# jorgeMFS/HYMET

Measured on AMD Instinct MI355X. Metric: contigs/s + Mbp/s classified, CAMI-medium, 1/2/4/8 MI355X; % HBM roofline, higher is better.
Workload: dtype u64

## Files before the change

### hymet_amd/_lib.py

```python
from __future__ import annotations

import ctypes
import os

HERE = os.path.dirname(os.path.abspath(__file__))
LIB_PATH = os.path.join(HERE, "libhymet_gpu.so")

_c = ctypes
_i64, _u64, _i32, _u32, _vp = _c.c_int64, _c.c_uint64, _c.c_int, _c.c_uint32, _c.c_void_p

_SIGS = {
    "hymet_version": (_i32, []),
    "hymet_init": (_i32, [_i32, _c.POINTER(_vp)]),
    "hymet_destroy": (_i32, [_vp]),
    "hymet_last_error": (_c.c_char_p, []),
    "hymet_set_stream": (_i32, [_vp, _vp]),
    "hymet_sync": (_i32, [_vp]),
    "hymet_prof_enable": (_i32, [_vp, _i32]),
    "hymet_prof_reset": (_i32, [_vp]),
    "hymet_prof_query": (_i32, [_vp, _c.c_char_p, _c.POINTER(_c.c_double), _c.POINTER(_i64), _c.POINTER(_c.c_double)]),
    "hymet_prof_names": (_i32, [_vp, _c.c_char_p, _i64]),
    "hymet_scratch_trim": (_i32, [_vp, _c.POINTER(_i64)]),
    "hymet_scratch_cached": (_i32, [_vp, _c.POINTER(_i64)]),
    "hymet_scratch_stats": (_i32, [_vp, _vp]),
    "hymet_scratch_reserve": (_i32, [_vp, _i64]),
    "hymet_set_oom_hook": (_i32, [_vp, _vp]),
    "hymet_copy_to_host": (_i32, [_vp, _vp, _vp, _i64, _i32]),
    "hymet_copy_to_device": (_i32, [_vp, _vp, _vp, _i64, _i32]),
    "hymet_pack": (_i32, [_vp, _vp, _i64, _i32, _vp, _vp]),
    "hymet_fasta_index": (_i32, [_vp, _i64, _i32, _i64, _c.POINTER(_i64), _vp, _vp, _vp, _vp, _vp]),
    "hymet_fasta_names": (_i32, [_vp, _vp, _vp, _i64, _vp, _vp]),
    "hymet_fasta_compact": (_i32, [_vp, _vp, _i64, _i64, _vp, _vp, _vp, _i64, _vp, _i64, _vp]),
    "hymet_name_hash": (_i32, [_vp, _vp, _vp, _vp, _i64, _vp]),
    "hymet_sort_pairs_u64": (_i32, [_vp, _vp, _vp, _i64, _i32, _i32]),
    "hymet_scan_u32": (_i32, [_vp, _vp, _vp, _i64, _i32, _vp]),
    "hymet_msh_open": (_i32, [_c.c_char_p, _c.POINTER(_vp)]),
    "hymet_msh_info_get": (_i32, [_vp, _vp]),
    "hymet_msh_copy": (_i32, [_vp, _i32, _vp, _vp, _vp, _vp, _vp, _vp]),
    "hymet_msh_upload": (_i32, [_vp, _vp, _i32, _vp, _vp, _i32]),
    "hymet_msh_upload_range": (_i32, [_vp, _vp, _i32, _vp, _vp, _i32, _i64, _i64]),
    "hymet_msh_text_offsets": (_i32, [_vp, _vp, _vp]),
    "hymet_msh_close": (None, [_vp]),
    "hymet_screen_table_slots": (_i64, [_i64]),
    "hymet_screen_table_build": (_i32, [_vp, _vp, _i64, _vp, _i64, _vp, _vp, _i32]),
    "hymet_screen_count": (_i32, [_vp, _vp, _vp, _i64, _i64, _i64, _i32, _u32, _i32, _c.POINTER(_vp), _c.POINTER(_i64),
                                  _c.POINTER(_vp), _c.POINTER(_i64), _c.POINTER(_vp), _u64, _vp, _i64, _vp, _vp]),
    "hymet_screen_stats": (_i32, [_vp, _vp, _i64, _vp, _vp, _vp, _vp]),
    "hymet_screen_winner": (_i32, [_vp, _vp, _i64, _vp, _vp, _i64, _vp, _i64, _vp, _vp, _vp]),
    "hymet_sketch_max_size": (_i64, []),
    "hymet_sketch_batch": (_i32, [_vp, _vp, _vp, _i64, _i32, _u32, _i32, _i64, _vp, _vp, _vp, _i32, _vp, _vp]),
    "hymet_mash_dist": (_i32, [_vp, _vp, _i64, _vp, _i64, _vp, _i64, _vp, _i64, _i64, _i64, _i32, _vp]),
    "hymet_mash_dist_tile": (_i32, [_i32]),
    "hymet_mash_dist_tune": (_i32, [_i32, _i32]),
    "hymet_mash_dist_select": (_i32, [_vp, _vp, _i64, _i64, _vp, _i32, _vp, _vp, _vp, _i64, _c.POINTER(_i64)]),
    "hymet_mash_dist_tri": (_i32, [_vp, _vp, _i64, _vp, _i64, _i64, _i64, _i32, _vp]),
    "hymet_mash_link": (_i32, [_vp, _vp, _i64, _i64, _i64, _vp, _i32, _vp, _vp]),
    "hymet_mash_labels": (_i32, [_vp, _vp, _i64, _vp]),
    "hymet_mm_sketch": (_i32, [_vp, _vp, _vp, _vp, _vp, _i32, _i32, _i32, _i32, _vp, _vp, _i64, _c.POINTER(_i64)]),
    "hymet_mm_index_build": (_i32, [_vp, _vp, _vp, _vp, _vp, _i32, _i32, _i32, _c.POINTER(_vp)]),
    "hymet_mm_index_destroy": (_i32, [_vp]),
    "hymet_mm_index_info": (_i32, [_vp, _c.POINTER(_i32), _c.POINTER(_i32), _c.POINTER(_i32), _c.POINTER(_i64)]),
    "hymet_mm_index_max_occ": (_i32, [_vp, _vp, _c.c_float, _c.POINTER(_i32)]),
    "hymet_mm_index_save": (_i32, [_vp, _vp, _c.c_char_p, _i32, _c.POINTER(_i64)]),
    "hymet_mm_index_load": (_i32, [_vp, _c.c_char_p, _i64, _c.POINTER(_vp), _c.POINTER(_i64)]),
    "hymet_mm_index_export": (_i32, [_vp, _vp, _vp, _vp]),
    "hymet_mm_map": (_i32, [_vp, _vp, _vp, _vp, _vp, _vp, _vp, _vp, _i32, _c.POINTER(_vp)]),
    "hymet_mm_result_size": (_i32, [_vp, _c.POINTER(_i64)]),
    "hymet_mm_result_copy": (_i32, [_vp, _vp, _vp, _vp]),
    "hymet_mm_result_destroy": (_i32, [_vp]),
    "hymet_paf_acc_create": (_i32, [_vp, _c.POINTER(_vp)]),
    "hymet_paf_acc_reset": (_i32, [_vp]),
    "hymet_paf_acc_destroy": (_i32, [_vp]),
    "hymet_paf_acc_info": (_i32, [_vp, _c.POINTER(_i64), _c.POINTER(_vp), _c.POINTER(_vp), _c.POINTER(_vp),
                                  _c.POINTER(_vp), _c.POINTER(_vp)]),
    "hymet_paf_acc_append": (_i32, [_vp, _vp, _vp, _i64, _i64]),
    "hymet_paf_acc_copy": (_i32, [_vp, _vp, _vp, _vp, _vp]),
    "hymet_paf_acc_field": (_i32, [_vp, _vp, _i32, _vp]),
    "hymet_mm_map_acc": (_i32, [_vp, _vp, _vp, _vp, _vp, _vp, _vp, _vp, _i32, _i32, _i32, _i32, _vp]),
    "hymet_emit_paf": (_i32, [_vp, _vp, _vp, _vp, _vp, _vp, _vp, _vp, _vp, _i64, _c.POINTER(_i64), _vp]),
    "hymet_acc_ref_counts": (_i32, [_vp, _vp, _vp]),
    "hymet_acc_classify": (_i32, [_vp, _vp, _i32, _i32] + [_vp] * 15 + [_c.POINTER(_i32)]),
    "hymet_emit_tsv": (_i32, [_vp, _i32, _i32] + [_vp] * 14 + [_i64, _c.POINTER(_i64)]),
    "hymet_mm_chain_dp": (_i32, [_vp, _vp, _vp, _i64, _i32, _i32, _i32, _i32, _i32, _c.c_float, _c.c_float, _vp, _vp]),
    "hymet_mm_mark_compact": (_i32, [_vp, _vp, _vp, _vp, _i64, _vp, _vp, _i32, _vp, _vp, _vp, _c.POINTER(_i64)]),
    "hymet_mm_stamp_scratch": (_i32, [_vp, _c.POINTER(_i64), _c.POINTER(_i64)]),
    "hymet_mm_anchor_sort": (_i32, [_vp, _vp, _vp, _i64, _vp, _i32, _i32, _i32, _u64, _i64, _vp, _vp, _vp, _vp, _vp]),
    "hymet_lca_ref_counts": (_i32, [_vp, _vp, _i64, _vp]),
    "hymet_lca": (_i32, [_vp, _i32, _i32] + [_vp] * 17),
}

_lib = None
_oom_hook = None


def _release_torch_cache(_user):
    try:
        import torch
        torch.cuda.empty_cache()
    except Exception:
        pass


class HymetError(RuntimeError):
    pass


def load():
    global _lib
    if _lib is not None:
        return _lib
    path = os.environ.get("HYMET_LIB", LIB_PATH)
    if not os.path.exists(path):
        raise HymetError(f"{path} not found: build the HIP extension (python -m hymet_amd.build); "
                         "hymet_amd has no CPU fallback")
    lib = ctypes.CDLL(path)
    for name, (res, args) in _SIGS.items():
        fn = getattr(lib, name)
        fn.restype = res
        fn.argtypes = args
    global _oom_hook
    _oom_hook = _c.CFUNCTYPE(None, _vp)(_release_torch_cache)
    lib.hymet_set_oom_hook(_c.cast(_oom_hook, _vp), None)
    _lib = lib
    return lib


def exported_symbols():
    return list(_SIGS)


def check(rc: int, what: str):
    if rc != 0:
        msg = load().hymet_last_error()
        raise HymetError(f"{what} failed ({rc}): {msg.decode() if msg else ''}")


class Gpu:

    def __init__(self, device: int = 0, stream=None):
        import torch

        if not torch.cuda.is_available():
            raise HymetError("no GPU visible: hymet_amd runs on MI355X (gfx950) only")
        self.torch = torch
        self.device = device
        torch.cuda.set_device(device)
        self.dev = torch.device("cuda", device)
        self.lib = load()
        h = _vp()
        check(self.lib.hymet_init(device, _c.byref(h)), "hymet_init")
        self.ctx = h
        self.stream = stream
        self.children = []
        self.bind_stream(stream)

    def fork(self) -> "Gpu":
        child = Gpu(self.device, stream=self.torch.cuda.Stream(device=self.device))
        self.children.append(child)
        return child

    def bind_stream(self, stream=None):
        s = stream if stream is not None else self.torch.cuda.current_stream(self.device)
        check(self.lib.hymet_set_stream(self.ctx, _vp(s.cuda_stream)), "hymet_set_stream")
        self.bound_stream = s

    def call(self, name, *args):
        check(getattr(self.lib, name)(self.ctx, *args), name)

    def sync(self):
        check(self.lib.hymet_sync(self.ctx), "hymet_sync")
        for ch in self.children:
            ch.sync()

    def prof(self, on: bool = True):
        check(self.lib.hymet_prof_enable(self.ctx, int(on)), "hymet_prof_enable")
        for ch in self.children:
            ch.prof(on)

    def prof_reset(self):
        check(self.lib.hymet_prof_reset(self.ctx), "hymet_prof_reset")
        for ch in self.children:
            ch.prof_reset()

    def prof_table(self):
        buf = _c.create_string_buffer(1 << 16)
        check(self.lib.hymet_prof_names(self.ctx, buf, 1 << 16), "hymet_prof_names")
        out = {}
        for name in buf.value.decode().split():
            ms, n, b = _c.c_double(), _i64(), _c.c_double()
            check(self.lib.hymet_prof_query(self.ctx, name.encode(), _c.byref(ms), _c.byref(n), _c.byref(b)), "hymet_prof_query")
            out[name] = (ms.value, n.value, b.value)
        for ch in self.children:
            for name, (ms, n, b) in ch.prof_table().items():
                m0, n0, b0 = out.get(name, (0.0, 0, 0.0))
                out[name] = (m0 + ms, n0 + n, b0 + b)
        return out

    def trim(self) -> int:
        out = _i64()
        check(self.lib.hymet_scratch_trim(self.ctx, _c.byref(out)), "hymet_scratch_trim")
        return out.value

    def reserve(self, nbytes: int):
        check(self.lib.hymet_scratch_reserve(self.ctx, int(nbytes)), "hymet_scratch_reserve")

    def _alloc(self, fn, n, dtype):
        try:
            return fn(int(n), dtype=dtype, device=self.dev)
        except self.torch.OutOfMemoryError:
            if self.trim() == 0:
                raise
            return fn(int(n), dtype=dtype, device=self.dev)

    def empty(self, n, dtype):
        return self._alloc(self.torch.empty, n, dtype)

    def zeros(self, n, dtype):
        return self._alloc(self.torch.zeros, n, dtype)

    def close(self):
        if self.ctx:
            self.lib.hymet_destroy(self.ctx)
            self.ctx = None

    def __del__(self):
        try:
            self.close()
        except Exception:
            pass


def ptr(t) -> _vp:
    return _vp(t.data_ptr())
```

### hymet_amd/csrc/common.hpp

```cpp
#pragma once
#include <hip/hip_runtime.h>
#include <stdint.h>
#include <algorithm>
#include <cstdlib>
#include <map>
#include <string>
#include <utility>
#include <vector>
#include "../../include/hymet_gpu.h"

struct hymet_ctx {
    int device = 0;
    hipStream_t stream = nullptr;
    bool own_stream = false;
    int n_cu = 256;
    bool prof = false;
    std::map<std::string, std::vector<std::pair<hipEvent_t, hipEvent_t>>> ev;
    std::map<std::string, double> bytes;
    std::map<std::string, std::pair<int, double>> dev_bytes;
    int64_t *prof_dev = nullptr;
    void *stage[2] = {nullptr, nullptr};
    hipEvent_t stage_ev[2] = {nullptr, nullptr};
    int64_t *mbox_h = nullptr;
    int64_t *mbox_d = nullptr;
    int32_t *dctr = nullptr;
    int32_t *stamp = nullptr;
    int64_t stamp_cap = 0;
    size_t stamp_cls = 0;
};

namespace hymet {
struct ProfScope {
    hymet_ctx *c;
    const char *name;
    hipEvent_t a = nullptr, b = nullptr;
    ProfScope(hymet_ctx *ctx, const char *n, double alg_bytes = 0.0) : c(ctx), name(n) {
        if (c && c->prof && hipEventCreate(&a) == hipSuccess && hipEventCreate(&b) == hipSuccess) {
            (void)hipEventRecord(a, c->stream);
            c->bytes[name] += alg_bytes;
        }
    }
    ProfScope(hymet_ctx *ctx, const char *n, int slot, double per_unit) : ProfScope(ctx, n, 0.0) {
        if (c && c->prof) c->dev_bytes[name] = {slot, per_unit};
    }
    ~ProfScope() {
        if (c && c->prof && a && b) {
            (void)hipEventRecord(b, c->stream);
            c->ev[name].push_back({a, b});
        }
    }
};
constexpr int kProfSlots = 8;
inline int64_t *prof_dev_slot(hymet_ctx *c, int k) { return c && c->prof && c->prof_dev ? c->prof_dev + k : nullptr; }
}

namespace hymet {
constexpr int kMbox = 64;
inline int64_t *mb_dev(hymet_ctx *c, int i) { return c->mbox_d + i; }
inline int64_t mb_read(const hymet_ctx *c, int i) { return __atomic_load_n(c->mbox_h + i, __ATOMIC_ACQUIRE); }
}

namespace hymet {
inline const char *env_str(const char *name) {
    const char *e = getenv(name);
    return e && *e ? e : nullptr;
}
inline bool env_flag(const char *name, bool dflt = false) {
    const char *e = env_str(name);
    return e ? e[0] != '0' : dflt;
}
inline int64_t env_int(const char *name, int64_t dflt, int64_t lo, int64_t hi) {
    const char *e = env_str(name);
    return e ? std::max(lo, std::min(hi, (int64_t)atoll(e))) : dflt;
}
}

namespace hymet {
void set_error(const std::string &msg);
int fail(int code, const std::string &msg);
int hip_fail(hipError_t e, const char *what);
inline int64_t cdiv(int64_t a, int64_t b) { return (a + b - 1) / b; }
hipError_t scratch_alloc(size_t bytes, hipStream_t stream, void **p, size_t *cls);
void set_oom_hook(void (*hook)(void *), void *user);
void scratch_free(void *p, hipStream_t stream, size_t cls);
hipError_t stamp_scratch(hymet_ctx *ctx, int64_t n, int32_t **out);
void stamp_release(hymet_ctx *ctx);
}

#define HY_CHECK_LAUNCH(what)                                   \
    do {                                                        \
        hipError_t e_ = hipGetLastError();                      \
        if (e_ != hipSuccess) return hymet::hip_fail(e_, what); \
    } while (0)

#define HY_HIP(call)                                            \
    do {                                                        \
        hipError_t e_ = (call);                                 \
        if (e_ != hipSuccess) return hymet::hip_fail(e_, #call); \
    } while (0)

#define HY_ARG(cond, msg)                                                   \
    do {                                                                    \
        if (!(cond)) return hymet::fail(HYMET_E_ARG, std::string(msg));     \
    } while (0)
```

### hymet_amd/csrc/mm_map.hip

```cpp
#include "mm_stages.hpp"

#include <algorithm>
#include <type_traits>
#include <utility>

#include <chrono>
#include <cstdio>
#include <cstdlib>
#include <cstring>

struct hymet_mm_result {
    int n_q = 0;
    std::vector<int64_t> reg_off;
    std::vector<int32_t> rep_len;
    std::vector<hymet_mm_reg> regs;
};

namespace hymet {
namespace mm {

int launch_regions(hymet_ctx *ctx, const uint64_t *ax, const uint32_t *ay, int span, const int32_t *ids, const int64_t *cfirst,
                   const uint64_t *cu, const int64_t *cboff,
                   const int64_t *qc, const int64_t *qb, const uint64_t *mini_pos, const int64_t *mp_off, const int64_t *qlen,
                   const uint32_t *name_hash, const int32_t *rep_len, const int64_t *ref_len, int n_q, const hymet_mm_opt *o,
                   int k, void *z, hymet_mm_reg *regs, int32_t *w, uint64_t *cov, int32_t *tmp, int32_t *n_regs,
                   int64_t NB, int64_t NC, int64_t NM, const uint32_t *cq,
                   const MiniWord *mtab, const int64_t *qbase, const uint32_t *skip_q, uint64_t *sumk, bool sumk_done);

namespace {

__global__ void fill_qid_kernel(const int64_t *off, int n_q, int64_t n, uint32_t *qid, uint32_t *ones, int32_t *zq) {
    const int64_t i = (int64_t)blockIdx.x * blockDim.x + threadIdx.x;
    if (i < n) {
        qid[i] = (uint32_t)upper_idx(off, n_q, i);
        if (ones) ones[i] = 1u;
    }
    if (zq && i < n_q) zq[i] = 0;
}

__global__ void flagged_len_kernel(const uint32_t *flag, const int64_t *qb, int n_q, uint32_t *cnt, int64_t *any) {
    const int q = blockIdx.x * blockDim.x + threadIdx.x;
    if (q > n_q) return;
    if (q == n_q) {
        cnt[q] = 0;
        return;
    }
    const bool f = flag[q] != 0;
    cnt[q] = f ? (uint32_t)(qb[q + 1] - qb[q]) : 0u;
    if (f) *any = 1;
}


__global__ void mzflt_runs_kernel(const uint32_t *sq, const uint64_t *sx, const uint32_t *sidx, const int64_t *qm_off,
                                  int64_t n, int q_occ_max, float q_occ_frac, uint32_t *keep) {
    const int64_t p = (int64_t)blockIdx.x * blockDim.x + threadIdx.x;
    if (p >= n) return;
    if (p > 0 && sq[p] == sq[p - 1] && sx[p] == sx[p - 1]) return;
    int64_t e = p + 1;
    while (e < n && sq[e] == sq[p] && sx[e] == sx[p]) e++;
    const uint32_t q = sq[p];
    const int64_t nq = qm_off[q + 1] - qm_off[q];
    if (nq <= q_occ_max) return;
    const int32_t cnt = (int32_t)(e - p);
    if (cnt > q_occ_max && (float)cnt > (float)nq * q_occ_frac)
        for (int64_t j = p; j < e; j++) keep[sidx[j]] = 0;
}

constexpr int kMzBuckets = 4096;
__global__ __launch_bounds__(256) void mzflt_screen_kernel(const uint64_t *mx, const int64_t *qm_off, int n_q, int q_occ_max,
                                                           uint32_t *keep, uint32_t *cnt, int64_t *any) {
    __shared__ uint32_t h[kMzBuckets];
    __shared__ int hit;
    const int q = blockIdx.x;
    if (q == n_q) {
        if (threadIdx.x == 0) cnt[q] = 0;
        return;
    }
    const int64_t s = qm_off[q], nq = qm_off[q + 1] - s;
    for (int64_t e = threadIdx.x; e < nq; e += 256) keep[s + e] = 1u;
    if (nq <= q_occ_max) {
        if (threadIdx.x == 0) cnt[q] = 0;
        return;
    }
    for (int b = threadIdx.x; b < kMzBuckets; b += 256) h[b] = 0;
    if (threadIdx.x == 0) hit = 0;
    __syncthreads();
    bool over = false;
    for (int64_t e = threadIdx.x; e < nq; e += 256)
        over |= atomicAdd(&h[(uint32_t)(mx[s + e] >> 8) & (kMzBuckets - 1)], 1u) >= (uint32_t)q_occ_max;
    if (over) hit = 1;
    __syncthreads();
    if (threadIdx.x == 0) {
        cnt[q] = hit ? (uint32_t)nq : 0u;
        if (hit) *any = 1;
    }
}

__global__ __launch_bounds__(256) void mzflt_list_kernel(const int64_t *qm_off, const uint32_t *cnt, const int64_t *coff,
                                                         uint32_t *gidx, uint32_t *sq) {
    const int q = blockIdx.x;
    const uint32_t nq = cnt[q];
    if (nq == 0) return;
    const int64_t s = qm_off[q], d = coff[q];
    for (uint32_t e = threadIdx.x; e < nq; e += 256) {
        gidx[d + e] = (uint32_t)(s + e);
        sq[d + e] = (uint32_t)q;
    }
}

__global__ void mzflt_gather_kernel(const uint32_t *perm, const uint32_t *gidx, const uint64_t *mx, uint32_t *gout,
                                    uint64_t *xout, int64_t n) {
    const int64_t i = (int64_t)blockIdx.x * blockDim.x + threadIdx.x;
    if (i >= n) return;
    const uint32_t g = gidx[perm[i]];
    gout[i] = g;
    xout[i] = mx[g];
}

__global__ void compact_mz_kernel(const uint64_t *x, const uint64_t *y, const uint32_t *keep, int64_t *pos, int64_t n,
                                  uint64_t *ox, uint64_t *oy) {
    const int64_t i = (int64_t)blockIdx.x * blockDim.x + threadIdx.x;
    if (i == n - 1) pos[n] = pos[i] + keep[i];
    if (i < n && keep[i]) {
        ox[pos[i]] = x[i];
        oy[pos[i]] = y[i];
    }
}

__global__ void sample_off_kernel(const int64_t *pos, const int64_t *qm_off, int n_q, int64_t total, int64_t *out) {
    const int q = blockIdx.x * blockDim.x + threadIdx.x;
    if (q > n_q) return;
    out[q] = q == n_q ? total : pos[qm_off[q]];
}

__global__ void seed_count_kernel(const uint64_t *mx, int64_t n, const uint32_t *koff, int64_t n_buckets,
                                  uint32_t *seed_n) {
    const int64_t i = (int64_t)blockIdx.x * blockDim.x + threadIdx.x;
    if (i >= n) return;
    const uint64_t h = mx[i] >> 8;
    uint32_t c = 0;
    if ((int64_t)h < n_buckets) c = koff[h + 1] - koff[h];
    seed_n[i] = c;
}

constexpr uint32_t kFlt = 0x80000000u;

__global__ void seed_class_kernel(const uint32_t *seed_n, int64_t M, int max_occ, uint64_t *cls) {
    const int64_t i = (int64_t)blockIdx.x * blockDim.x + threadIdx.x;
    if (i > M) return;
    if (i == M) {
        cls[M] = 0;
        return;
    }
    const uint32_t n = seed_n[i];
    const bool hi = (int)n > max_occ, lo = n > 0 && !hi;
    cls[i] = (uint64_t)(hi ? 1u : 0u) << 32 | (lo ? 1u : 0u);
}

__global__ void seed_list_kernel(const uint32_t *seed_n, const uint64_t *rank, int64_t M, int max_occ, int32_t *low_idx,
                                 int32_t *high_idx) {
    const int64_t i = (int64_t)blockIdx.x * blockDim.x + threadIdx.x;
    if (i >= M) return;
    const uint32_t n = seed_n[i];
    if (!n) return;
    if ((int)n > max_occ) high_idx[rank[i] >> 32] = (int32_t)i;
    else low_idx[(uint32_t)rank[i]] = (int32_t)i;
}

struct StreakParams {
    const uint64_t *my;
    const uint32_t *qid;
    const int64_t *qm_off, *qlen;
    const uint64_t *rank;
    const int32_t *low_idx, *high_idx;
    int64_t n_low;
    int n_q;
    int max_occ, max_max_occ, dist;
    uint32_t *seed_n;
    uint32_t *flt_high;
};

__global__ void streak_kernel(StreakParams P) {
    const int64_t t = (int64_t)blockIdx.x * blockDim.x + threadIdx.x;
    if (t >= P.n_low + P.n_q) return;
    int q;
    int64_t e_idx = -1, p_idx = -1;
    uint64_t re, rp;
    if (t < P.n_low) {
        e_idx = P.low_idx[t];
        q = (int)P.qid[e_idx];
        re = P.rank[e_idx];
        if (t > 0 && P.qid[P.low_idx[t - 1]] == (uint32_t)q) p_idx = P.low_idx[t - 1];
    } else {
        q = (int)(t - P.n_low);
        re = P.rank[P.qm_off[q + 1]];
        const uint64_t r0 = P.rank[P.qm_off[q]];
        if ((uint32_t)re > (uint32_t)r0) p_idx = P.low_idx[(uint32_t)re - 1];
    }
    rp = p_idx >= 0 ? P.rank[p_idx] : P.rank[P.qm_off[q]];
    const int64_t h0 = (int64_t)(rp >> 32), h1 = (int64_t)(re >> 32);
    const int cnt = (int)(h1 - h0);
    if (cnt <= 0) return;
    const bool case_a = P.dist > 0 && P.max_max_occ > P.max_occ;
    bool keep_all = false, keep_none = false;
    uint64_t thr = 0;
    if (case_a) {
        const uint64_t rq0 = P.rank[P.qm_off[q]], rq1 = P.rank[P.qm_off[q + 1]];
        const int64_t n_seed = (int64_t)((uint32_t)rq1 - (uint32_t)rq0) + (int64_t)((rq1 >> 32) - (rq0 >> 32));
        if (n_seed <= 1) return;
        const int32_t ps = p_idx >= 0 ? (int32_t)((uint32_t)P.my[p_idx] >> 1) : 0;
        const int32_t pe = e_idx >= 0 ? (int32_t)((uint32_t)P.my[e_idx] >> 1) : (int32_t)P.qlen[q];
        int32_t mh = (int32_t)((double)(pe - ps) / P.dist + .499);
        if (mh > 128) mh = 128;
        keep_all = mh >= cnt, keep_none = mh <= 0;
        if (!keep_all && !keep_none) {
            uint64_t lo = 0, hi = ~0ull;
            while (lo < hi) {
                const uint64_t mid = lo + (hi - lo) / 2;
                int c = 0;
                for (int64_t r = h0; r < h1; r++) {
                    const int32_t a = P.high_idx[r];
                    c += ((uint64_t)P.seed_n[a] << 32 | (uint32_t)a) <= mid;
                }
                if (c >= mh) hi = mid;
                else lo = mid + 1;
            }
            thr = lo;
        }
    }
    for (int64_t r = h0; r < h1; r++) {
        const int32_t a = P.high_idx[r];
        const uint32_t n = P.seed_n[a];
        bool flt = true;
        if (case_a) {
            const bool chosen = keep_all || (!keep_none && ((uint64_t)n << 32 | (uint32_t)a) <= thr);
            flt = !chosen || (int)n > P.max_max_occ;
        }
        P.flt_high[r] = flt ? 1u : 0u;
    }
}

__global__ void flt_mark_kernel(const uint32_t *flt_high, int64_t n_high, int32_t *v) {
    const int64_t r = (int64_t)blockIdx.x * blockDim.x + threadIdx.x;
    if (r < n_high) v[r] = flt_high[r] ? (int32_t)r : -1;
}

__global__ void rep_len_kernel(const uint32_t *flt_high, const int32_t *prev_max, const int32_t *high_idx, int64_t n_high,
                               const uint64_t *mx, const uint64_t *my, const uint32_t *qid, int32_t *rep_len,
                               uint32_t *seed_n) {
    const int64_t r = (int64_t)blockIdx.x * blockDim.x + threadIdx.x;
    if (r >= n_high || !flt_high[r]) return;
    const int32_t a = high_idx[r];
    const uint32_t q = qid[a];
    const int32_t en = (int32_t)((uint32_t)my[a] >> 1) + 1, st = en - (int32_t)(mx[a] & 0xff);
    int32_t en_prev = 0;
    const int32_t pr = r > 0 ? prev_max[r - 1] : -1;
    if (pr >= 0) {
        const int32_t b = high_idx[pr];
        if (qid[b] == q) en_prev = (int32_t)((uint32_t)my[b] >> 1) + 1;
    }
    atomicAdd(rep_len + q, en - max(st, en_prev));
    seed_n[a] = 0;
}

__global__ void nz_flag_kernel(const uint32_t *v, int64_t n, uint32_t *flag) {
    const int64_t i = (int64_t)blockIdx.x * blockDim.x + threadIdx.x;
    if (i < n) flag[i] = v[i] ? 1u : 0u;
}

struct AnchorParams {
    const uint64_t *mx, *my;
    const uint32_t *seed_n;
    const int64_t *a_pos;
    const uint32_t *qid;
    const int64_t *qlen;
    const uint32_t *koff;
    const uint64_t *ipos;
    int64_t n;
    int rb;
    uint64_t *ax, *k1, *k2;
    uint32_t *ay;
    uint32_t *val;
    const int64_t *mp_pos;
    uint64_t *mini_pos;
};

__global__ void write_anchors_kernel(AnchorParams P) {
    const int64_t i = (int64_t)blockIdx.x * blockDim.x + threadIdx.x;
    if (i >= P.n) return;
    const uint32_t n = P.seed_n[i];
    if (!n) return;
    const uint64_t mx = P.mx[i], my = P.my[i];
    const uint32_t q_pos = (uint32_t)my, q_span = (uint32_t)(mx & 0xff);
    P.mini_pos[P.mp_pos[i]] = (uint64_t)q_span << 32 | (q_pos >> 1);
    const uint32_t q = P.qid[i];
    const int32_t qlen = (int32_t)P.qlen[q];
    const uint32_t *kp = P.koff + (mx >> 8);
    const uint64_t *r = P.ipos + kp[0];
    int64_t a = P.a_pos[i];
    for (uint32_t k = 0; k < n; k++, a++) {
        const uint64_t rk = r[k];
        const uint32_t rpos = (uint32_t)rk >> 1;
        const uint32_t rid = (uint32_t)(rk >> 32);
        uint64_t x, y;
        uint32_t rev;
        if ((rk & 1) == (q_pos & 1)) {
            rev = 0;
            x = (rk & 0xffffffff00000000ULL) | rpos;
            y = (uint64_t)q_span << 32 | (q_pos >> 1);
        } else {
            rev = 1;
            x = 1ULL << 63 | (rk & 0xffffffff00000000ULL) | rpos;
            y = (uint64_t)q_span << 32 | (uint32_t)(qlen - (int32_t)((q_pos >> 1) + 1 - q_span) - 1);
        }
        P.ax[a] = x;
        P.ay[a] = (uint32_t)y;
        P.k1[a] = (uint64_t)q << (1 + P.rb) | (uint64_t)rev << P.rb | rid;
        P.k2[a] = (uint64_t)rpos << 32 | (uint32_t)y;
        P.val[a] = (uint32_t)a;
    }
}

struct AnchorKeyParams {
    const uint64_t *mx, *my;
    const uint32_t *seed_n;
    const int64_t *a_pos;
    const uint32_t *qid;
    const int64_t *qlen;
    const uint32_t *koff;
    const uint64_t *ipos;
    int64_t n;
    int rb, pb;
    int ybits;
    uint64_t *key;
    uint32_t *val;
    const int64_t *mp_pos;
    uint64_t *mini_pos;
};

__global__ __launch_bounds__(256) void write_anchor_keys_kernel(AnchorKeyParams P) {
    __shared__ int64_t s_a[257];
    __shared__ uint64_t s_r[256];
    __shared__ uint32_t s_yf[256], s_yr[256], s_strand[256];
    __shared__ uint64_t s_q[256];
    const int tid = threadIdx.x;
    const int64_t m0 = (int64_t)blockIdx.x * 256;
    const int cnt = (int)min((int64_t)256, P.n - m0);
    if (tid < cnt) {
        const int64_t i = m0 + tid;
        const uint32_t n = P.seed_n[i];
        const uint64_t mx = P.mx[i], my = P.my[i];
        const uint32_t q_pos = (uint32_t)my, q_span = (uint32_t)(mx & 0xff);
        const uint32_t q = P.qid[i];
        if (n) P.mini_pos[P.mp_pos[i]] = (uint64_t)q_span << 32 | (q_pos >> 1);
        s_a[tid] = P.a_pos[i];
        s_r[tid] = P.koff[mx >> 8];
        s_yf[tid] = q_pos >> 1;
        s_yr[tid] = (uint32_t)((int32_t)P.qlen[q] - (int32_t)((q_pos >> 1) + 1 - q_span) - 1);
        s_strand[tid] = q_pos & 1;
        s_q[tid] = (uint64_t)q << (1 + P.rb + P.pb);
    }
    if (tid == 0) s_a[cnt] = P.a_pos[m0 + cnt];
    __syncthreads();
    const int64_t a0 = s_a[0], a1 = s_a[cnt];
    const int sh_rev = P.rb + P.pb;
    for (int64_t a = a0 + tid; a < a1; a += 256) {
        int lo = 0, hi = cnt - 1;
        while (lo < hi) {
            const int mid = (lo + hi + 1) >> 1;
            if (s_a[mid] <= a) lo = mid;
            else hi = mid - 1;
        }
        const uint64_t rk = P.ipos[s_r[lo] + (a - s_a[lo])];
        const uint32_t rpos = (uint32_t)rk >> 1;
        const uint64_t rid = rk >> 32;
        const uint32_t rev = ((uint32_t)rk & 1) != s_strand[lo];
        const uint64_t k = (uint64_t)rev << sh_rev | rid << P.pb | rpos;
        const uint32_t y = rev ? s_yr[lo] : s_yf[lo];
        if (P.ybits) {
            P.key[a] = k << P.ybits | y;
        } else {
            P.key[a] = s_q[lo] | k;
            P.val[a] = y;
        }
    }
}

__global__ void anchor_unpack_kernel(const uint64_t *key, const uint32_t *val, int64_t n, int rb, int pb, uint64_t *ax,
                                     uint32_t *ay) {
    const int64_t i = (int64_t)blockIdx.x * blockDim.x + threadIdx.x;
    if (i >= n) return;
    const uint64_t k = key[i];
    const uint64_t rev = k >> (rb + pb) & 1, rid = k >> pb & ((1ull << rb) - 1), rpos = k & ((1ull << pb) - 1);
    ax[i] = rev << 63 | rid << 32 | rpos;
    const bool prev_eq = i > 0 && key[i - 1] == k;
    const bool next_eq = i + 1 < n && key[i + 1] == k;
    if (!prev_eq && !next_eq) {
        ay[i] = val[i];
    } else if (!prev_eq) {
        int64_t e = i + 1;
        while (e + 1 < n && key[e + 1] == k) e++;
        for (int64_t a = i; a <= e; a++) {
            const uint32_t v = val[a];
            int64_t b = a;
            while (b > i && ay[b - 1] > v) {
                ay[b] = ay[b - 1];
                b--;
            }
            ay[b] = v;
        }
    }
}

__global__ __launch_bounds__(256) void mini_bits_kernel(const uint64_t *my, const uint32_t *seed_n, const uint32_t *qid,
                                                        const int64_t *qbase, int64_t M, MiniWord *tab) {
    const int64_t i = (int64_t)blockIdx.x * blockDim.x + threadIdx.x;
    const int lane = threadIdx.x & 63;
    const bool on = i < M && seed_n[i];
    const int64_t b = on ? qbase[qid[i]] + ((uint32_t)my[i] >> 1) : -64 * (int64_t)(lane + 1);
    const int64_t w = b >> 6;
    uint64_t bits = on ? 1ull << (b & 63) : 0;
#pragma unroll
    for (int d = 1; d < 64; d <<= 1) {
        const int64_t wo = __shfl_down(w, d, 64);
        const uint64_t bo = __shfl_down(bits, d, 64);
        if (lane + d < 64 && wo == w) bits |= bo;
    }
    const int64_t wp = __shfl_up(w, 1, 64);
    if (on && (lane == 0 || wp != w)) atomicOr((unsigned long long *)&tab[w].bits, bits);
}
__global__ void mini_base_kernel(const uint64_t *my, const uint32_t *seed_n, const uint32_t *qid, const int64_t *qm_off,
                                 const int64_t *mp_pos, const int64_t *qbase, int64_t M, MiniWord *tab) {
    const int64_t i = (int64_t)blockIdx.x * blockDim.x + threadIdx.x;
    if (i >= M || !seed_n[i]) return;
    const uint32_t q = qid[i];
    const int64_t b = qbase[q] + ((uint32_t)my[i] >> 1);
    const uint64_t bits = tab[b >> 6].bits;
    tab[b >> 6].base = (uint32_t)(mp_pos[i] - mp_pos[qm_off[q]]) - (uint32_t)__popcll(bits & ((1ull << (b & 63)) - 1));
}

__global__ void rechain_gather_kernel(const uint64_t *bx, const uint32_t *by, const int64_t *qb, const uint32_t *qflag,
                                      const int64_t *new_off, int n_q, int rb, uint64_t *x, uint32_t *y, uint64_t *k1,
                                      uint64_t *k2, uint32_t *val) {
    const int q = blockIdx.x;
    if (q >= n_q || !qflag[q]) return;
    const int64_t b0 = qb[q], b1 = qb[q + 1], o = new_off[q];
    for (int64_t i = b0 + threadIdx.x; i < b1; i += blockDim.x) {
        const int64_t a = o + (i - b0);
        const uint64_t ax = bx[i];
        const uint32_t ay = by[i];
        x[a] = ax;
        y[a] = ay;
        k1[a] = (uint64_t)q << (1 + rb) | (ax >> 63) << rb | (ax << 1 >> 33);
        k2[a] = (uint64_t)(uint32_t)ax << 32 | ay;
        val[a] = (uint32_t)a;
    }
}

__global__ __launch_bounds__(256) void rechain_keys_kernel(const uint64_t *bx, const uint32_t *by, const int64_t *qb,
                                                           const int64_t *new_off, int n_q, int64_t n, int rb, int pb,
                                                           int ybits, uint64_t *key, uint32_t *val) {
    __shared__ int s_q0;
    const int64_t a0 = (int64_t)blockIdx.x * blockDim.x;
    if (threadIdx.x == 0) s_q0 = upper_idx(new_off, n_q, a0);
    __syncthreads();
    const int64_t a = a0 + threadIdx.x;
    if (a >= n) return;
    int q = s_q0;
    while (q + 1 < n_q && new_off[q + 1] <= a) q++;
    const int64_t i = qb[q] + (a - new_off[q]);
    const uint64_t ax = bx[i];
    const uint64_t k = (ax >> 63) << (rb + pb) | (ax << 1 >> 33) << pb | (uint32_t)ax;
    if (ybits) {
        key[a] = k << ybits | by[i];
    } else {
        key[a] = (uint64_t)q << (1 + rb + pb) | k;
        val[a] = by[i];
    }
}

__global__ void reg_count_kernel(const uint32_t *flag, const int32_t *n1, const int32_t *n2, int n_q, uint32_t *cnt) {
    const int q = blockIdx.x * blockDim.x + threadIdx.x;
    if (q < n_q) cnt[q] = (uint32_t)((flag && flag[q]) ? n2[q] : n1[q]);
}

struct RegOut {
    hymet_mm_reg *regs;
    int32_t *q, *part, *rl, *t;
    int32_t q_base, part_id, t_base;
};
__global__ void reg_gather_kernel(const uint32_t *flag, const int32_t *n1, const int32_t *n2, const int64_t *qc1,
                                  const int64_t *qc2, const hymet_mm_reg *r1, const hymet_mm_reg *r2, const int64_t *off,
                                  const int32_t *rep_len, int n_q, RegOut o) {
    const int q = blockIdx.x * blockDim.x + threadIdx.x;
    if (q >= n_q) return;
    const bool use2 = flag && flag[q];
    const hymet_mm_reg *src = use2 ? r2 + qc2[q] : r1 + qc1[q];
    const int nr = use2 ? n2[q] : n1[q];
    const int64_t d = off[q];
    for (int i = 0; i < nr; i++) {
        const hymet_mm_reg r = src[i];
        o.regs[d + i] = r;
        if (o.q) {
            o.q[d + i] = o.q_base + q;
            o.part[d + i] = o.part_id;
            o.rl[d + i] = rep_len[q];
            o.t[d + i] = o.t_base + r.rid;
        }
    }
}
}
}
}

using namespace hymet;
using namespace hymet::mm;

struct CallTrace {
    bool on = env_flag("HYMET_TRACE");
    std::chrono::steady_clock::time_point t = std::chrono::steady_clock::now();
    ~CallTrace() {
        if (on)
            fprintf(stderr, "[hymet_mm_map] %-22s %9.2f ms\n", "TOTAL (with frees)",
                    std::chrono::duration<double, std::milli>(std::chrono::steady_clock::now() - t).count());
    }
};
struct PhaseTrace {
    hymet_ctx *ctx;
    bool on;
    std::chrono::steady_clock::time_point t;
    explicit PhaseTrace(hymet_ctx *c) : ctx(c), on(env_flag("HYMET_TRACE")), t(std::chrono::steady_clock::now()) {}
    void mark(const char *what) {
        if (!on) return;
        (void)hipStreamSynchronize(ctx->stream);
        const auto n = std::chrono::steady_clock::now();
        fprintf(stderr, "[hymet_mm_map] %-22s %9.2f ms\n", what, std::chrono::duration<double, std::milli>(n - t).count());
        t = n;
    }
};

static int sort_anchor_set(hymet_ctx *ctx, DevBuf &x, DevBuf &y, DevBuf &k1, DevBuf &k2, DevBuf &val, int64_t n,
                           int key1_bits, int yhi, AnchorSet &out) {
    DevBuf k2b, valb, k1g, k1b;
    HY_HIP(k2b.alloc(8 * (size_t)n, ctx->stream));
    HY_HIP(valb.alloc(4 * (size_t)n, ctx->stream));
    uint64_t *kk = k2.as<uint64_t>(), *kka = k2b.as<uint64_t>();
    uint32_t *vv = val.as<uint32_t>(), *vva = valb.as<uint32_t>();
    int rc = sort_pairs(ctx, kk, kka, vv, vva, n, 0, 64, "radix_sort_anchor_pos");
    if (rc) return rc;
    HY_HIP(k1g.alloc(8 * (size_t)n, ctx->stream));
    HY_HIP(k1b.alloc(8 * (size_t)n, ctx->stream));
    LAUNCH1(gather_kernel<uint64_t>, n, k1.as<uint64_t>(), vv, k1g.as<uint64_t>(), n);
    uint64_t *k1p = k1g.as<uint64_t>(), *k1a = k1b.as<uint64_t>();
    rc = sort_pairs(ctx, k1p, k1a, vv, vva, n, 0, key1_bits, "radix_sort_anchor_group");
    if (rc) return rc;
    HY_HIP(out.ax.alloc(8 * (size_t)n, ctx->stream));
    HY_HIP(out.ay.alloc(4 * (size_t)n, ctx->stream));
    LAUNCH1(gather_kernel<uint64_t>, n, x.as<uint64_t>(), vv, out.ax.as<uint64_t>(), n);
    LAUNCH1(gather_kernel<uint32_t>, n, y.as<uint32_t>(), vv, out.ay.as<uint32_t>(), n);
    out.n = n;
    out.span = yhi & 0xff;
    return HYMET_OK;
}

static int sort_anchor_words(hymet_ctx *ctx, DevBuf &word, int64_t n, int rb, int pb, int yhi, const int64_t *d_qoff, int n_q,
                             int64_t max_qlen, AnchorSet &out) {
    DevBuf wb;
    HY_HIP(wb.alloc(8 * (size_t)n, ctx->stream));
    HY_HIP(out.ax.alloc(8 * (size_t)n, ctx->stream));
    HY_HIP(out.ay.alloc(4 * (size_t)n, ctx->stream));
    HY_HIP(out.hb.alloc(head_bits_bytes(n), ctx->stream));
    HY_HIP(out.ax32.alloc(4 * (size_t)n, ctx->stream));
    out.n = n;
    out.span = yhi & 0xff;
    const bool log_stats = env_flag("HYMET_ASORT_STATS");
    DevBuf sstat;
    if (log_stats) {
        HY_HIP(sstat.alloc(32, ctx->stream));
        HY_HIP(hipMemsetAsync(sstat.p, 0, 32, ctx->stream));
    }
    const int rc = grouped_anchor_sort(ctx, word.as<uint64_t>(), n, d_qoff, n_q, rb, pb, max_qlen,
                                       wb.as<uint64_t>(), out.ax.as<uint64_t>(), out.ay.as<uint32_t>(),
                                       out.hb.as<uint32_t>(), out.ax32.as<uint32_t>(),
                                       log_stats ? sstat.as<unsigned long long>() : nullptr);
    if (rc == 1) return hymet::fail(HYMET_E_INTERNAL, "sort_anchor_words: anchor words emitted for a layout without one");
    if (rc) return rc;
    if (log_stats) {
        unsigned long long h[4] = {};
        HY_HIP(hipMemcpyAsync(h, sstat.p, 32, hipMemcpyDeviceToHost, ctx->stream));
        HY_HIP(hipStreamSynchronize(ctx->stream));
        fprintf(stderr, "[asort] anchors %lld fast_segs %llu fast_anchors %llu full_segs %llu full_anchors %llu\n",
                (long long)n, h[0], h[1], h[2], h[3]);
    }
    out.has_hb = out.has_x32 = true;
    return HYMET_OK;
}

static int sort_anchor_keys(hymet_ctx *ctx, DevBuf &key, DevBuf &val, int64_t n, int end_bit, int rb, int pb, int yhi,
                            AnchorSet &out) {
    DevBuf kb, vb;
    HY_HIP(kb.alloc(8 * (size_t)n, ctx->stream));
    HY_HIP(vb.alloc(4 * (size_t)n, ctx->stream));
    HY_HIP(out.ax.alloc(8 * (size_t)n, ctx->stream));
    HY_HIP(out.ay.alloc(4 * (size_t)n, ctx->stream));
    out.n = n;
    out.span = yhi & 0xff;
    uint64_t *kk = key.as<uint64_t>(), *kka = kb.as<uint64_t>();
    uint32_t *vv = val.as<uint32_t>(), *vva = vb.as<uint32_t>();
    int rc = sort_pairs<uint64_t, uint32_t>(ctx, kk, kka, vv, vva, n, 0, end_bit, "radix_sort_anchors");
    if (rc) return rc;
    {
        ProfScope _ps(ctx, "mm_anchor_unpack", 24.0 * (double)n);
        LAUNCH1(anchor_unpack_kernel, n, kk, vv, n, rb, pb, out.ax.as<uint64_t>(), out.ay.as<uint32_t>());
    }
    return HYMET_OK;
}

static int dump_anchors(hymet_ctx *ctx, const char *var, const AnchorSet &S, int n_q, bool &dumped) {
    const char *path = env_str(var);
    if (!path || dumped || S.n == 0) return HYMET_OK;
    dumped = true;
    hipStream_t st = ctx->stream;
    const int64_t nd = std::min<int64_t>(S.n, env_int("HYMET_DUMP_MAX", 1 << 24, 0, INT64_MAX));
    std::vector<uint64_t> hx(nd);
    std::vector<uint32_t> hy(nd);
    std::vector<int64_t> qo(n_q + 1);
    HY_HIP(hipMemcpyAsync(hx.data(), S.ax.p, 8 * (size_t)nd, hipMemcpyDeviceToHost, st));
    HY_HIP(hipMemcpyAsync(hy.data(), S.ay.p, 4 * (size_t)nd, hipMemcpyDeviceToHost, st));
    HY_HIP(hipMemcpyAsync(qo.data(), S.d_off.p, 8 * (size_t)(n_q + 1), hipMemcpyDeviceToHost, st));
    HY_HIP(hipStreamSynchronize(st));
    if (FILE *fp = fopen(path, "wb")) {
        uint64_t gid = 0;
        int q = 0;
        std::vector<uint64_t> buf;
        buf.reserve(1 << 21);
        for (int64_t a = 0; a < nd; a++) {
            bool qs = false;
            while (q < n_q && qo[q + 1] <= a) q++, qs = true;
            if (a && (qs || (hx[a] >> 32) != (hx[a - 1] >> 32))) gid++;
            buf.push_back(gid << 32 | (uint32_t)hx[a]);
            buf.push_back((uint64_t)S.span << 32 | hy[a]);
            if (buf.size() >= (1u << 21)) fwrite(buf.data(), 8, buf.size(), fp), buf.clear();
        }
        fwrite(buf.data(), 8, buf.size(), fp);
        fclose(fp);
    }
    return HYMET_OK;
}

struct MapSink {
    hymet_mm_result *res = nullptr;
    hymet_paf_acc *acc = nullptr;
    int32_t q_base = 0, part_id = 0, t_base = 0;
};

static int acc_reserve(hymet_ctx *ctx, hymet_paf_acc *a, int64_t need) {
    if (need <= a->cap) return HYMET_OK;
    const int64_t cap = std::max<int64_t>(need, std::max<int64_t>(a->cap * 3 / 2, 1 << 16));
    hipStream_t st = ctx->stream;
    DevBuf nregs, nq, npart, nrl, nt;
    HY_HIP(nregs.alloc(sizeof(hymet_mm_reg) * (size_t)cap, st));
    HY_HIP(nq.alloc(4 * (size_t)cap, st));
    HY_HIP(npart.alloc(4 * (size_t)cap, st));
    HY_HIP(nrl.alloc(4 * (size_t)cap, st));
    HY_HIP(nt.alloc(4 * (size_t)cap, st));
    if (a->n) {
        HY_HIP(hipMemcpyAsync(nregs.p, a->regs.p, sizeof(hymet_mm_reg) * (size_t)a->n, hipMemcpyDeviceToDevice, st));
        HY_HIP(hipMemcpyAsync(nq.p, a->q.p, 4 * (size_t)a->n, hipMemcpyDeviceToDevice, st));
        HY_HIP(hipMemcpyAsync(npart.p, a->part.p, 4 * (size_t)a->n, hipMemcpyDeviceToDevice, st));
        HY_HIP(hipMemcpyAsync(nrl.p, a->rl.p, 4 * (size_t)a->n, hipMemcpyDeviceToDevice, st));
        HY_HIP(hipMemcpyAsync(nt.p, a->t.p, 4 * (size_t)a->n, hipMemcpyDeviceToDevice, st));
    }
    a->regs.swap(nregs);
    a->q.swap(nq);
    a->part.swap(npart);
    a->rl.swap(nrl);
    a->t.swap(nt);
    a->cap = cap;
    return HYMET_OK;
}

struct MapBatch {
    hymet_ctx *ctx;
    const hymet_mm_index *idx;
    const hymet_mm_opt *opt;
    const int64_t *h_lens;
    int32_t n_q;
    DevBuf mx, my, qm_off;
    int64_t M = 0;
    DevBuf d_qlen, d_hash_buf;
    const uint32_t *d_hash = nullptr;
    DevBuf seed_n, rep_len, qid;
    DevBuf mini_pos, mp_off;
    int64_t NM = 0;
    DevBuf d_qbase, pos_tab;
    std::vector<int64_t> qbase;
    int64_t max_qlen = 1;
    int rb = 0, pb = 0, key1_bits = 0;
    bool key_path = false;
    int ybits = 0;
};

static int sketch_queries(MapBatch &B, const uint32_t *d_2b, const uint32_t *d_mask, const int64_t *h_starts,
                          const uint32_t *h_name_hash, const uint32_t *d_name_hash) {
    hipStream_t st = B.ctx->stream;
    const int n_q = B.n_q;
    int rc = sketch_sequences(B.ctx, d_2b, d_mask, h_starts, B.h_lens, n_q, B.idx->w, B.idx->k, 0, B.mx, B.my, &B.M, &B.qm_off);
    if (rc) return rc;
    HY_HIP(B.d_qlen.alloc(8 * (size_t)n_q, st));
    HY_HIP(hipMemcpyAsync(B.d_qlen.p, B.h_lens, 8 * (size_t)n_q, hipMemcpyHostToDevice, st));
    B.d_hash = d_name_hash;
    if (!B.d_hash) {
        HY_HIP(B.d_hash_buf.alloc(4 * (size_t)n_q, st));
        HY_HIP(hipMemcpyAsync(B.d_hash_buf.p, h_name_hash, 4 * (size_t)n_q, hipMemcpyHostToDevice, st));
        B.d_hash = B.d_hash_buf.as<uint32_t>();
    }
    return HYMET_OK;
}

static int filter_minimizers(MapBatch &B) {
    hymet_ctx *ctx = B.ctx;
    hipStream_t st = ctx->stream;
    const hymet_mm_opt *opt = B.opt;
    const int n_q = B.n_q;
    const int64_t M = B.M;
    DevBuf &mx = B.mx, &my = B.my, &qm_off = B.qm_off;
    DevBuf keep, fcnt, fcoff;
    int64_t MF = 0;
    int rc;
    if (opt->q_occ_frac > 0.0f && M > 0 && opt->mid_occ > 0) {
        HY_HIP(keep.alloc(4 * (size_t)M, st));
        HY_HIP(fcnt.alloc(4 * (size_t)(n_q + 1), st));
        ctx->mbox_h[kMbFlag] = 0;
        hipLaunchKernelGGL(mzflt_screen_kernel, dim3((unsigned)n_q + 1), dim3(256), 0, st, mx.as<uint64_t>(), qm_off.as<int64_t>(),
                           n_q, opt->mid_occ, keep.as<uint32_t>(), fcnt.as<uint32_t>(), mb_dev(ctx, kMbFlag));
        HY_CHECK_LAUNCH("mzflt_screen_kernel");
        HY_HIP(hipStreamSynchronize(st));
        if (mb_read(ctx, kMbFlag) != 0) {
            HY_HIP(fcoff.alloc(8 * (size_t)(n_q + 1), st));
            rc = exclusive_scan_u32_i64(ctx, fcnt.as<uint32_t>(), fcoff.as<int64_t>(), n_q + 1, &MF);
            if (rc) return rc;
        }
    }
    if (MF == 0) return HYMET_OK;
    DevBuf gidx, sx, sx2, sidx, sidx2, sq0, sq, sq2, kpos, nx, ny, gx, gg;
    HY_HIP(gidx.alloc(4 * (size_t)MF, st));
    HY_HIP(sq0.alloc(4 * (size_t)MF, st));
    hipLaunchKernelGGL(mzflt_list_kernel, dim3((unsigned)n_q), dim3(256), 0, st, qm_off.as<int64_t>(), fcnt.as<uint32_t>(),
                       fcoff.as<int64_t>(), gidx.as<uint32_t>(), sq0.as<uint32_t>());
    HY_CHECK_LAUNCH("mzflt_list_kernel");
    HY_HIP(sx.alloc(8 * (size_t)MF, st));
    HY_HIP(sx2.alloc(8 * (size_t)MF, st));
    HY_HIP(sidx.alloc(4 * (size_t)MF, st));
    HY_HIP(sidx2.alloc(4 * (size_t)MF, st));
    LAUNCH1(gather_kernel<uint64_t>, MF, mx.as<uint64_t>(), gidx.as<uint32_t>(), sx.as<uint64_t>(), MF);
    LAUNCH1(iota_u32_kernel, MF, sidx.as<uint32_t>(), MF);
    uint64_t *kx = sx.as<uint64_t>(), *kxa = sx2.as<uint64_t>();
    uint32_t *vi = sidx.as<uint32_t>(), *via = sidx2.as<uint32_t>();
    rc = sort_pairs(ctx, kx, kxa, vi, via, MF, 0, 2 * B.idx->k + 8, "radix_sort_mz");
    if (rc) return rc;
    HY_HIP(sq.alloc(4 * (size_t)MF, st));
    HY_HIP(sq2.alloc(4 * (size_t)MF, st));
    LAUNCH1(gather_kernel<uint32_t>, MF, sq0.as<uint32_t>(), vi, sq.as<uint32_t>(), MF);
    uint32_t *kq = sq.as<uint32_t>(), *kqa = sq2.as<uint32_t>();
    rc = sort_pairs(ctx, kq, kqa, vi, via, MF, 0, bits_for(n_q), "radix_sort_mz");
    if (rc) return rc;
    HY_HIP(gx.alloc(8 * (size_t)MF, st));
    HY_HIP(gg.alloc(4 * (size_t)MF, st));
    LAUNCH1(mzflt_gather_kernel, MF, vi, gidx.as<uint32_t>(), mx.as<uint64_t>(), gg.as<uint32_t>(), gx.as<uint64_t>(), MF);
    LAUNCH1(mzflt_runs_kernel, MF, kq, gx.as<uint64_t>(), gg.as<uint32_t>(), qm_off.as<int64_t>(), MF, opt->mid_occ,
            opt->q_occ_frac, keep.as<uint32_t>());
    int64_t M2 = 0;
    rc = scan_flags(ctx, keep.as<uint32_t>(), M, kpos, &M2);
    if (rc) return rc;
    HY_HIP(nx.alloc(8 * (size_t)(M2 + 1), st));
    HY_HIP(ny.alloc(8 * (size_t)(M2 + 1), st));
    LAUNCH1(compact_mz_kernel, M, mx.as<uint64_t>(), my.as<uint64_t>(), keep.as<uint32_t>(), kpos.as<int64_t>(), M,
            nx.as<uint64_t>(), ny.as<uint64_t>());
    DevBuf nqm;
    HY_HIP(nqm.alloc(8 * (size_t)(n_q + 1), st));
    hipLaunchKernelGGL(sample_off_kernel, dim3((unsigned)cdiv(n_q + 1, 256)), dim3(256), 0, st, kpos.as<int64_t>(),
                       qm_off.as<int64_t>(), n_q, M2, nqm.as<int64_t>());
    HY_CHECK_LAUNCH("sample_off_kernel");
    mx.swap(nx);
    my.swap(ny);
    qm_off.swap(nqm);
    B.M = M2;
    return HYMET_OK;
}

static int select_seeds(MapBatch &B) {
    hymet_ctx *ctx = B.ctx;
    hipStream_t st = ctx->stream;
    const hymet_mm_opt *opt = B.opt;
    const int n_q = B.n_q;
    const int64_t M = B.M;
    DevBuf &mx = B.mx, &my = B.my, &qm_off = B.qm_off, &seed_n = B.seed_n, &rep_len = B.rep_len, &qid = B.qid;
    HY_HIP(seed_n.alloc(4 * (size_t)(M + 1), st));
    HY_HIP(rep_len.alloc(4 * (size_t)n_q, st));
    HY_HIP(qid.alloc(4 * (size_t)(M + 1), st));
    LAUNCH1(fill_qid_kernel, std::max<int64_t>(M, n_q), qm_off.as<int64_t>(), n_q, M, qid.as<uint32_t>(), nullptr,
            rep_len.as<int32_t>());
    {
        ProfScope _ps(ctx, "mm_seed_count", (double)M * (8.0 + 8.0 + 4.0));
        LAUNCH1(seed_count_kernel, M, mx.as<uint64_t>(), M, B.idx->d_koff, B.idx->n_buckets, seed_n.as<uint32_t>());
    }
    if (M == 0) return HYMET_OK;
    ProfScope _ps(ctx, "mm_seed_select", (double)M * (4.0 + 8.0 + 8.0 + 8.0));
    DevBuf cls, rank, spart;
    HY_HIP(cls.alloc(8 * (size_t)(M + 1), st));
    HY_HIP(rank.alloc(8 * (size_t)(M + 1), st));
    LAUNCH1(seed_class_kernel, M + 1, seed_n.as<uint32_t>(), M, opt->mid_occ, cls.as<uint64_t>());
    int rc = scan_u64(ctx, cls.as<uint64_t>(), rank.as<uint64_t>(), M + 1, spart, mb_dev(ctx, kMbScan));
    if (rc) return rc;
    HY_HIP(hipStreamSynchronize(st));
    const uint64_t tot = (uint64_t)mb_read(ctx, kMbScan);
    const int64_t n_low = (uint32_t)tot, n_high = (int64_t)(tot >> 32);
    if (n_high == 0) return HYMET_OK;
    DevBuf low_idx, high_idx, flt_high, vmax, pmax;
    HY_HIP(low_idx.alloc(4 * (size_t)(n_low + 1), st));
    HY_HIP(high_idx.alloc(4 * (size_t)n_high, st));
    HY_HIP(flt_high.alloc(4 * (size_t)n_high, st));
    LAUNCH1(seed_list_kernel, M, seed_n.as<uint32_t>(), rank.as<uint64_t>(), M, opt->mid_occ, low_idx.as<int32_t>(),
            high_idx.as<int32_t>());
    StreakParams S{my.as<uint64_t>(), qid.as<uint32_t>(), qm_off.as<int64_t>(), B.d_qlen.as<int64_t>(),
                   rank.as<uint64_t>(), low_idx.as<int32_t>(), high_idx.as<int32_t>(), n_low, n_q, opt->mid_occ,
                   opt->max_max_occ, opt->occ_dist, seed_n.as<uint32_t>(), flt_high.as<uint32_t>()};
    HY_HIP(hipMemsetAsync(flt_high.p, 0, 4 * (size_t)n_high, st));
    LAUNCH1(streak_kernel, n_low + n_q, S);
    HY_HIP(vmax.alloc(4 * (size_t)n_high, st));
    HY_HIP(pmax.alloc(4 * (size_t)n_high, st));
    LAUNCH1(flt_mark_kernel, n_high, flt_high.as<uint32_t>(), n_high, vmax.as<int32_t>());
    {
        DevBuf mpart;
        rc = inclusive_max_scan_i32(ctx, vmax.as<int32_t>(), pmax.as<int32_t>(), n_high, mpart);
        if (rc) return rc;
    }
    LAUNCH1(rep_len_kernel, n_high, flt_high.as<uint32_t>(), pmax.as<int32_t>(), high_idx.as<int32_t>(), n_high,
            mx.as<uint64_t>(), my.as<uint64_t>(), qid.as<uint32_t>(), rep_len.as<int32_t>(), seed_n.as<uint32_t>());
    return HYMET_OK;
}

static int build_mini_table(MapBatch &B, const DevBuf &mp_pos) {
    hymet_ctx *ctx = B.ctx;
    hipStream_t st = ctx->stream;
    const int n_q = B.n_q;
    B.qbase.assign(n_q + 1, 0);
    for (int q = 0; q < n_q; q++) {
        B.qbase[q + 1] = B.qbase[q] + ((B.h_lens[q] + 63) & ~(int64_t)63);
        B.max_qlen = std::max<int64_t>(B.max_qlen, B.h_lens[q]);
    }
    HY_HIP(B.d_qbase.alloc(8 * (size_t)(n_q + 1), st));
    HY_HIP(hipMemcpyAsync(B.d_qbase.p, B.qbase.data(), 8 * (size_t)(n_q + 1), hipMemcpyHostToDevice, st));
    const size_t n_words = (size_t)(B.qbase[n_q] >> 6) + 1;
    HY_HIP(B.pos_tab.alloc(sizeof(MiniWord) * n_words, st));
    HY_HIP(hipMemsetAsync(B.pos_tab.p, 0, sizeof(MiniWord) * n_words, st));
    LAUNCH1(mini_bits_kernel, B.M, B.my.as<uint64_t>(), B.seed_n.as<uint32_t>(), B.qid.as<uint32_t>(), B.d_qbase.as<int64_t>(),
            B.M, B.pos_tab.as<MiniWord>());
    LAUNCH1(mini_base_kernel, B.M, B.my.as<uint64_t>(), B.seed_n.as<uint32_t>(), B.qid.as<uint32_t>(), B.qm_off.as<int64_t>(),
            mp_pos.as<int64_t>(), B.d_qbase.as<int64_t>(), B.M, B.pos_tab.as<MiniWord>());
    return HYMET_OK;
}

static int first_pass_anchors(MapBatch &B, AnchorSet &S1) {
    hymet_ctx *ctx = B.ctx;
    hipStream_t st = ctx->stream;
    const hymet_mm_index *idx = B.idx;
    const int n_q = B.n_q;
    const int64_t M = B.M;
    DevBuf &mx = B.mx, &my = B.my, &qm_off = B.qm_off, &seed_n = B.seed_n, &qid = B.qid, &d_qlen = B.d_qlen;
    DevBuf a_pos, mflag, mp_pos;
    int64_t A = 0;
    int rc = scan_flags(ctx, seed_n.as<uint32_t>(), M, a_pos, &A);
    if (rc) return rc;
    HY_ARG(A <= anchor_cap(), "hymet_mm_map: the batch has more anchors than 32-bit chain links hold (map fewer bases per batch)");
    HY_HIP(mflag.alloc(4 * (size_t)(M + 1), st));
    LAUNCH1(nz_flag_kernel, M, seed_n.as<uint32_t>(), M, mflag.as<uint32_t>());
    rc = scan_flags(ctx, mflag.as<uint32_t>(), M, mp_pos, &B.NM);
    if (rc) return rc;
    HY_HIP(hipMemcpyAsync(a_pos.as<int64_t>() + M, &A, 8, hipMemcpyHostToDevice, st));
    HY_HIP(hipMemcpyAsync(mp_pos.as<int64_t>() + M, &B.NM, 8, hipMemcpyHostToDevice, st));
    HY_HIP(B.mini_pos.alloc(8 * (size_t)(B.NM + 1), st));
    HY_HIP(B.mp_off.alloc(8 * (size_t)(n_q + 1), st));
    hipLaunchKernelGGL(sample_off_kernel, dim3((unsigned)cdiv(n_q + 1, 256)), dim3(256), 0, st, mp_pos.as<int64_t>(),
                       qm_off.as<int64_t>(), n_q, B.NM, B.mp_off.as<int64_t>());
    HY_CHECK_LAUNCH("sample_off_kernel");
    rc = build_mini_table(B, mp_pos);
    if (rc) return rc;
    HY_HIP(S1.d_off.alloc(8 * (size_t)(n_q + 1), st));
    hipLaunchKernelGGL(sample_off_kernel, dim3((unsigned)cdiv(n_q + 1, 256)), dim3(256), 0, st, a_pos.as<int64_t>(),
                       qm_off.as<int64_t>(), n_q, A, S1.d_off.as<int64_t>());
    HY_CHECK_LAUNCH("sample_off_kernel");
    B.rb = bits_for(idx->n_seq);
    B.key1_bits = bits_for(n_q) + 1 + B.rb;
    HY_ARG(B.key1_bits <= 64, "hymet_mm_map: too many queries x targets for the sort key");
    int64_t max_len = 1;
    for (int64_t l : idx->h_len) max_len = std::max(max_len, l);
    B.pb = bits_for(max_len - 1);
    B.key_path = B.key1_bits + B.pb <= 64 && !env_flag("HYMET_ANCHOR_LEGACY");
    B.ybits = B.key_path && env_flag("HYMET_ANCHOR_GSORT", true) ? anchor_word_ybits(B.rb, B.pb, B.max_qlen) : 0;
    if (B.key_path) {
        const bool words = B.ybits > 0 && A > 0;
        DevBuf key, val;
        HY_HIP(key.alloc(8 * (size_t)(A + 1), st));
        if (!words) HY_HIP(val.alloc(4 * (size_t)(A + 1), st));
        AnchorKeyParams P{mx.as<uint64_t>(), my.as<uint64_t>(), seed_n.as<uint32_t>(), a_pos.as<int64_t>(),
                          qid.as<uint32_t>(), d_qlen.as<int64_t>(), idx->d_koff, idx->d_pos, M, B.rb, B.pb,
                          words ? B.ybits : 0, key.as<uint64_t>(), val.as<uint32_t>(), mp_pos.as<int64_t>(),
                          B.mini_pos.as<uint64_t>()};
        {
            ProfScope _ps(ctx, "mm_anchors", (double)A * (8.0 + 12.0));
            if (M > 0) {
                hipLaunchKernelGGL(write_anchor_keys_kernel, dim3((unsigned)cdiv(M, 256)), dim3(256), 0, st, P);
                HY_CHECK_LAUNCH("write_anchor_keys_kernel");
            }
        }
        if (words) return sort_anchor_words(ctx, key, A, B.rb, B.pb, idx->k, S1.d_off.as<int64_t>(), n_q, B.max_qlen, S1);
        return sort_anchor_keys(ctx, key, val, A, B.key1_bits + B.pb, B.rb, B.pb, idx->k, S1);
    }
    DevBuf x, y, k1, k2, val;
    HY_HIP(x.alloc(8 * (size_t)(A + 1), st));
    HY_HIP(y.alloc(4 * (size_t)(A + 1), st));
    HY_HIP(k1.alloc(8 * (size_t)(A + 1), st));
    HY_HIP(k2.alloc(8 * (size_t)(A + 1), st));
    HY_HIP(val.alloc(4 * (size_t)(A + 1), st));
    AnchorParams P{mx.as<uint64_t>(), my.as<uint64_t>(), seed_n.as<uint32_t>(), a_pos.as<int64_t>(), qid.as<uint32_t>(),
                   d_qlen.as<int64_t>(), idx->d_koff, idx->d_pos, M, B.rb, x.as<uint64_t>(), k1.as<uint64_t>(),
                   k2.as<uint64_t>(), y.as<uint32_t>(), val.as<uint32_t>(), mp_pos.as<int64_t>(), B.mini_pos.as<uint64_t>()};
    ProfScope _ps(ctx, "mm_anchors", (double)A * (8.0 + 36.0));
    LAUNCH1(write_anchors_kernel, M, P);
    return sort_anchor_set(ctx, x, y, k1, k2, val, A, B.key1_bits, idx->k, S1);
}

static int long_join_anchors(MapBatch &B, const AnchorSet &S1, const ChainSet &C1, const LeanJoin &lj, const DevBuf &flag,
                             AnchorSet &S2, bool &any) {
    hymet_ctx *ctx = B.ctx;
    hipStream_t st = ctx->stream;
    const int n_q = B.n_q;
    const DevBuf &qbuf = lj.mark_only ? lj.qb2 : C1.d_qb;
    DevBuf fcnt;
    HY_HIP(fcnt.alloc(4 * (size_t)(n_q + 1), st));
    ctx->mbox_h[kMbFlag] = 0;
    LAUNCH1(flagged_len_kernel, n_q + 1, flag.as<uint32_t>(), qbuf.as<int64_t>(), n_q, fcnt.as<uint32_t>(), mb_dev(ctx, kMbFlag));
    int64_t A2 = 0;
    int rc = scan_flags(ctx, fcnt.as<uint32_t>(), n_q + 1, S2.d_off, &A2);
    if (rc) return rc;
    any = mb_read(ctx, kMbFlag) != 0;
    if (!any) return HYMET_OK;
    HY_ARG(A2 <= anchor_cap(), "hymet_mm_map: the long join has more anchors than 32-bit chain links hold");
    if (lj.mark_only) {
        rc = marked_anchor_set(ctx, S1, lj, flag.as<uint32_t>(), n_q, A2, S2);
    } else if (B.key_path) {
        const bool words = B.ybits > 0 && A2 > 0;
        DevBuf key, val;
        HY_HIP(key.alloc(8 * (size_t)(A2 + 1), st));
        if (!words) HY_HIP(val.alloc(4 * (size_t)(A2 + 1), st));
        LAUNCH1(rechain_keys_kernel, A2, C1.bx.as<uint64_t>(), C1.by.as<uint32_t>(), C1.d_qb.as<int64_t>(),
                S2.d_off.as<int64_t>(), n_q, A2, B.rb, B.pb, words ? B.ybits : 0, key.as<uint64_t>(), val.as<uint32_t>());
        rc = words ? sort_anchor_words(ctx, key, A2, B.rb, B.pb, B.idx->k, S2.d_off.as<int64_t>(), n_q, B.max_qlen, S2)
                   : sort_anchor_keys(ctx, key, val, A2, B.key1_bits + B.pb, B.rb, B.pb, B.idx->k, S2);
    } else {
        DevBuf x, y, k1, k2, val;
        HY_HIP(x.alloc(8 * (size_t)(A2 + 1), st));
        HY_HIP(y.alloc(4 * (size_t)(A2 + 1), st));
        HY_HIP(k1.alloc(8 * (size_t)(A2 + 1), st));
        HY_HIP(k2.alloc(8 * (size_t)(A2 + 1), st));
        HY_HIP(val.alloc(4 * (size_t)(A2 + 1), st));
        hipLaunchKernelGGL(rechain_gather_kernel, dim3((unsigned)n_q), dim3(256), 0, st, C1.bx.as<uint64_t>(),
                           C1.by.as<uint32_t>(), C1.d_qb.as<int64_t>(), flag.as<uint32_t>(), S2.d_off.as<int64_t>(), n_q,
                           B.rb, x.as<uint64_t>(), y.as<uint32_t>(), k1.as<uint64_t>(), k2.as<uint64_t>(), val.as<uint32_t>());
        HY_CHECK_LAUNCH("rechain_gather_kernel");
        rc = sort_anchor_set(ctx, x, y, k1, k2, val, A2, B.key1_bits, S1.span, S2);
    }
    if (rc) return rc;
    static bool dumped = false;
    return dump_anchors(ctx, "HYMET_DUMP_ANCHORS2", S2, n_q, dumped);
}

static int run_regions(MapBatch &B, ChainSet &C, DevBuf &rg, DevBuf &nr, const uint32_t *skip_q, DevBuf &sumk, bool &sumk_done) {
    hipStream_t st = B.ctx->stream;
    const int64_t NC = C.n_chain;
    DevBuf z, wv, cov, tmp;
    HY_HIP(z.alloc(16 * (size_t)(NC + 1), st));
    HY_HIP(rg.alloc(sizeof(hymet_mm_reg) * (size_t)(NC + 1), st));
    HY_HIP(wv.alloc(4 * (size_t)(NC + 1), st));
    HY_HIP(cov.alloc(8 * (size_t)(NC + 1), st));
    HY_HIP(tmp.alloc(4 * (size_t)(NC + 1), st));
    HY_HIP(nr.alloc(4 * (size_t)B.n_q, st));
    return launch_regions(B.ctx, C.ax, C.ay, C.span, C.ids.as<int32_t>(), C.cfirst.as<int64_t>(), C.cu.as<uint64_t>(),
                          C.cboff.as<int64_t>(), C.d_qc.as<int64_t>(), C.d_qb.as<int64_t>(), B.mini_pos.as<uint64_t>(),
                          B.mp_off.as<int64_t>(), B.d_qlen.as<int64_t>(), B.d_hash, B.rep_len.as<int32_t>(), B.idx->d_len,
                          B.n_q, B.opt, B.idx->k, z.p, rg.as<hymet_mm_reg>(), wv.as<int32_t>(), cov.as<uint64_t>(),
                          tmp.as<int32_t>(), nr.as<int32_t>(), C.n_anchor, NC, B.NM, C.cq.as<uint32_t>(),
                          B.pos_tab.as<MiniWord>(), B.d_qbase.as<int64_t>(), skip_q, sumk.as<uint64_t>(),
                          std::exchange(sumk_done, true));
}

struct RegSet {
    const int32_t *n;
    const int64_t *qc;
    const hymet_mm_reg *r;
};

static int emit_records(MapBatch &B, const uint32_t *fl, const RegSet &s1, const RegSet &s2, MapSink &sink) {
    hymet_ctx *ctx = B.ctx;
    hipStream_t st = ctx->stream;
    const int n_q = B.n_q;
    hymet_mm_result *res = sink.res;
    DevBuf cnt, off;
    HY_HIP(cnt.alloc(4 * (size_t)(n_q + 1), st));
    LAUNCH1(reg_count_kernel, n_q, fl, s1.n, s2.n, n_q, cnt.as<uint32_t>());
    int64_t N = 0;
    int rc = scan_flags(ctx, cnt.as<uint32_t>(), n_q, off, &N);
    if (rc) return rc;
    HY_HIP(hipMemcpyAsync(off.as<int64_t>() + n_q, &N, 8, hipMemcpyHostToDevice, st));
    RegOut o{};
    DevBuf tmp_regs;
    if (sink.acc) {
        hymet_paf_acc *a = sink.acc;
        rc = acc_reserve(ctx, a, a->n + N);
        if (rc) return rc;
        o = RegOut{a->regs.as<hymet_mm_reg>() + a->n, a->q.as<int32_t>() + a->n, a->part.as<int32_t>() + a->n,
                   a->rl.as<int32_t>() + a->n, a->t.as<int32_t>() + a->n, sink.q_base, sink.part_id, sink.t_base};
    } else {
        HY_HIP(tmp_regs.alloc(sizeof(hymet_mm_reg) * (size_t)(N + 1), st));
        o.regs = tmp_regs.as<hymet_mm_reg>();
    }
    {
        ProfScope _ps(ctx, "mm_paf_records", (double)N * (2.0 * sizeof(hymet_mm_reg) + 16.0));
        LAUNCH1(reg_gather_kernel, n_q, fl, s1.n, s2.n, s1.qc, s2.qc, s1.r, s2.r, off.as<int64_t>(), B.rep_len.as<int32_t>(),
                n_q, o);
    }
    if (sink.acc) {
        sink.acc->n += N;
    } else {
        res->regs.resize(N);
        if (N) HY_HIP(hipMemcpyAsync(res->regs.data(), tmp_regs.p, sizeof(hymet_mm_reg) * (size_t)N, hipMemcpyDeviceToHost, st));
        HY_HIP(hipMemcpyAsync(res->reg_off.data(), off.p, 8 * (size_t)(n_q + 1), hipMemcpyDeviceToHost, st));
        HY_HIP(hipMemcpyAsync(res->rep_len.data(), B.rep_len.p, 4 * (size_t)n_q, hipMemcpyDeviceToHost, st));
    }
    HY_HIP(hipStreamSynchronize(st));
    return HYMET_OK;
}

static int mm_map_impl(hymet_ctx *ctx, const hymet_mm_index *idx, const hymet_mm_opt *opt, const uint32_t *d_2b,
                       const uint32_t *d_mask, const int64_t *h_starts, const int64_t *h_lens, const uint32_t *h_name_hash,
                       const uint32_t *d_name_hash, int32_t n_q, MapSink &sink) {
    CallTrace call_trace;
    HY_ARG(ctx && idx && opt && d_2b && d_mask, "hymet_mm_map: null argument");
    HY_ARG(n_q >= 0, "hymet_mm_map: n_q < 0");
    HY_ARG(h_name_hash || d_name_hash, "hymet_mm_map: no query name hashes");
    HY_ARG(opt->mid_occ > 0, "hymet_mm_map: opt->mid_occ must be resolved (hymet_mm_index_max_occ + clamps)");
    HY_HIP(hipSetDevice(ctx->device));
    if (sink.res) {
        sink.res->n_q = n_q;
        sink.res->reg_off.assign(n_q + 1, 0);
        sink.res->rep_len.assign(n_q, 0);
    }
    if (n_q == 0) return HYMET_OK;
    const float pen_gap = (float)(opt->chain_gap_scale * 0.01 * idx->k);
    const float pen_skip = (float)(opt->chain_skip_scale * 0.01 * idx->k);
    PhaseTrace tr(ctx);
    MapBatch B{ctx, idx, opt, h_lens, n_q};
    int rc = sketch_queries(B, d_2b, d_mask, h_starts, h_name_hash, d_name_hash);
    if (rc) return rc;
    tr.mark("sketch");
    rc = filter_minimizers(B);
    if (rc) return rc;
    tr.mark("mz_flt");
    rc = select_seeds(B);
    if (rc) return rc;
    tr.mark("seeds");
    AnchorSet S1;
    rc = first_pass_anchors(B, S1);
    if (rc) return rc;
    tr.mark("anchors+sort");
    static bool dumped1 = false;
    rc = dump_anchors(ctx, "HYMET_DUMP_ANCHORS", S1, n_q, dumped1);
    if (rc) return rc;
    ChainSet C1;
    const bool long_join = opt->bw_long > opt->bw;
    const bool resort = env_flag("HYMET_RECHAIN_SORT");
    LeanJoin lj{B.d_qlen.as<int64_t>(), opt->rmq_rescue_size, opt->rmq_rescue_ratio, B.key_path && !resort};
    rc = chain_set(ctx, opt, pen_gap, pen_skip, opt->bw, S1, n_q, C1, long_join ? &lj : nullptr, long_join && !lj.mark_only);
    if (rc) return rc;
    tr.mark("chain_set 1");
    ChainSet C2;
    AnchorSet S2;
    DevBuf flag;
    bool joined = false;
    if (long_join && C1.n_chain > 0) {
        flag.swap(lj.flag);
        rc = long_join_anchors(B, S1, C1, lj, flag, S2, joined);
        if (rc) return rc;
        if (joined) {
            rc = chain_set(ctx, opt, pen_gap, pen_skip, opt->bw_long, S2, n_q, C2);
            if (rc) return rc;
        }
    }
    tr.mark("long join");
    DevBuf sumk, rg1, nr1, rg2, nr2;
    HY_HIP(sumk.alloc(8 * (size_t)(n_q + 1), ctx->stream));
    bool sumk_done = false;
    const uint32_t *fl = joined ? flag.as<uint32_t>() : nullptr;
    rc = run_regions(B, C1, rg1, nr1, fl, sumk, sumk_done);
    if (rc) return rc;
    if (joined) {
        rc = run_regions(B, C2, rg2, nr2, nullptr, sumk, sumk_done);
        if (rc) return rc;
    }
    const RegSet r1{nr1.as<int32_t>(), C1.d_qc.as<int64_t>(), rg1.as<hymet_mm_reg>()};
    const RegSet r2{nr2.as<int32_t>(), C2.d_qc.as<int64_t>(), rg2.as<hymet_mm_reg>()};
    rc = emit_records(B, fl, r1, joined ? r2 : r1, sink);
    if (rc) return rc;
    tr.mark("regions");
    return HYMET_OK;
}

extern "C" {

int hymet_mm_map(hymet_ctx *ctx, const hymet_mm_index *idx, const hymet_mm_opt *opt, const uint32_t *d_2b,
                 const uint32_t *d_mask, const int64_t *h_starts, const int64_t *h_lens, const uint32_t *h_name_hash,
                 int32_t n_q, hymet_mm_result **out) {
    HY_ARG(out != nullptr, "hymet_mm_map: null argument");
    MapSink sink;
    sink.res = new hymet_mm_result();
    *out = sink.res;
    return mm_map_impl(ctx, idx, opt, d_2b, d_mask, h_starts, h_lens, h_name_hash, nullptr, n_q, sink);
}

int hymet_paf_acc_create(hymet_ctx *ctx, hymet_paf_acc **out) {
    HY_ARG(ctx && out, "hymet_paf_acc_create: null argument");
    hymet_paf_acc *a = new hymet_paf_acc();
    a->device = ctx->device;
    *out = a;
    return HYMET_OK;
}

int hymet_paf_acc_reset(hymet_paf_acc *acc) {
    HY_ARG(acc, "hymet_paf_acc_reset: null argument");
    acc->n = 0;
    return HYMET_OK;
}

int hymet_paf_acc_destroy(hymet_paf_acc *acc) {
    if (acc) {
        (void)hipSetDevice(acc->device);
        delete acc;
    }
    return HYMET_OK;
}

int hymet_paf_acc_info(const hymet_paf_acc *acc, int64_t *n_lines, void **d_regs, void **d_q, void **d_part, void **d_rl,
                       void **d_t) {
    HY_ARG(acc && n_lines, "hymet_paf_acc_info: null argument");
    *n_lines = acc->n;
    if (d_regs) *d_regs = acc->regs.p;
    if (d_q) *d_q = acc->q.p;
    if (d_part) *d_part = acc->part.p;
    if (d_rl) *d_rl = acc->rl.p;
    if (d_t) *d_t = acc->t.p;
    return HYMET_OK;
}

int hymet_paf_acc_append(hymet_ctx *ctx, hymet_paf_acc *dst, const hymet_paf_acc *src, int64_t begin, int64_t end) {
    HY_ARG(ctx && dst && src && dst != src, "hymet_paf_acc_append: null or aliased argument");
    HY_ARG(begin >= 0 && end >= begin && end <= src->n, "hymet_paf_acc_append: line range outside the source");
    const int64_t m = end - begin;
    if (m == 0) return HYMET_OK;
    HY_HIP(hipSetDevice(ctx->device));
    int rc = acc_reserve(ctx, dst, dst->n + m);
    if (rc) return rc;
    hipStream_t st = ctx->stream;
    const int64_t d = dst->n;
    HY_HIP(hipMemcpyAsync(dst->regs.as<hymet_mm_reg>() + d, src->regs.as<hymet_mm_reg>() + begin, sizeof(hymet_mm_reg) * (size_t)m,
                          hipMemcpyDeviceToDevice, st));
    HY_HIP(hipMemcpyAsync(dst->q.as<int32_t>() + d, src->q.as<int32_t>() + begin, 4 * (size_t)m, hipMemcpyDeviceToDevice, st));
    HY_HIP(hipMemcpyAsync(dst->part.as<int32_t>() + d, src->part.as<int32_t>() + begin, 4 * (size_t)m, hipMemcpyDeviceToDevice,
                          st));
    HY_HIP(hipMemcpyAsync(dst->rl.as<int32_t>() + d, src->rl.as<int32_t>() + begin, 4 * (size_t)m, hipMemcpyDeviceToDevice, st));
    HY_HIP(hipMemcpyAsync(dst->t.as<int32_t>() + d, src->t.as<int32_t>() + begin, 4 * (size_t)m, hipMemcpyDeviceToDevice, st));
    dst->n += m;
    return HYMET_OK;
}

int hymet_paf_acc_copy(hymet_ctx *ctx, const hymet_paf_acc *acc, int32_t *h_q, int32_t *h_part, int32_t *h_t) {
    HY_ARG(ctx && acc, "hymet_paf_acc_copy: null argument");
    if (acc->n <= 0) return HYMET_OK;
    HY_HIP(hipSetDevice(ctx->device));
    hipStream_t st = ctx->stream;
    if (h_q) HY_HIP(hipMemcpyAsync(h_q, acc->q.p, 4 * (size_t)acc->n, hipMemcpyDeviceToHost, st));
    if (h_part) HY_HIP(hipMemcpyAsync(h_part, acc->part.p, 4 * (size_t)acc->n, hipMemcpyDeviceToHost, st));
    if (h_t) HY_HIP(hipMemcpyAsync(h_t, acc->t.p, 4 * (size_t)acc->n, hipMemcpyDeviceToHost, st));
    HY_HIP(hipStreamSynchronize(st));
    return HYMET_OK;
}

int hymet_paf_acc_field(hymet_ctx *ctx, const hymet_paf_acc *acc, int field, int32_t *h_out) {
    HY_ARG(ctx && acc && h_out && field >= 0 && field < (int)(sizeof(hymet_mm_reg) / 4), "hymet_paf_acc_field: bad argument");
    if (acc->n <= 0) return HYMET_OK;
    HY_HIP(hipSetDevice(ctx->device));
    const char *src = static_cast<const char *>(acc->regs.p) + 4 * (size_t)field;
    HY_HIP(hipMemcpy2DAsync(h_out, 4, src, sizeof(hymet_mm_reg), 4, (size_t)acc->n, hipMemcpyDeviceToHost, ctx->stream));
    HY_HIP(hipStreamSynchronize(ctx->stream));
    return HYMET_OK;
}

int hymet_mm_map_acc(hymet_ctx *ctx, const hymet_mm_index *idx, const hymet_mm_opt *opt, const uint32_t *d_2b,
                     const uint32_t *d_mask, const int64_t *h_starts, const int64_t *h_lens, const uint32_t *d_name_hash,
                     int32_t n_q, int32_t q_base, int32_t part_id, int32_t t_base, hymet_paf_acc *acc) {
    HY_ARG(acc && d_name_hash, "hymet_mm_map_acc: null argument");
    MapSink sink;
    sink.acc = acc;
    sink.q_base = q_base;
    sink.part_id = part_id;
    sink.t_base = t_base;
    return mm_map_impl(ctx, idx, opt, d_2b, d_mask, h_starts, h_lens, nullptr, d_name_hash, n_q, sink);
}

int hymet_mm_result_size(const hymet_mm_result *res, int64_t *n_regs) {
    HY_ARG(res && n_regs, "hymet_mm_result_size: null argument");
    *n_regs = (int64_t)res->regs.size();
    return HYMET_OK;
}

int hymet_mm_result_copy(const hymet_mm_result *res, int64_t *h_off, int32_t *h_rep_len, hymet_mm_reg *h_regs) {
    HY_ARG(res, "hymet_mm_result_copy: null result");
    if (h_off) memcpy(h_off, res->reg_off.data(), 8 * (size_t)(res->n_q + 1));
    if (h_rep_len && res->n_q) memcpy(h_rep_len, res->rep_len.data(), 4 * (size_t)res->n_q);
    if (h_regs && !res->regs.empty()) memcpy(h_regs, res->regs.data(), sizeof(hymet_mm_reg) * res->regs.size());
    return HYMET_OK;
}

int hymet_mm_result_destroy(hymet_mm_result *res) {
    delete res;
    return HYMET_OK;
}

}
```

### hymet_amd/csrc/mm_sketch.hip

```cpp
#include "mm_common.hpp"

#include "sort.hpp"

#include <cstdio>
#include <cstdlib>
#include <cstring>

namespace hymet {
namespace mm {
namespace {

template <int W, bool WRITE>
__global__ __launch_bounds__(256) void mm_sketch_kernel(SketchParams P) {
    const int64_t g = (int64_t)blockIdx.x * blockDim.x + threadIdx.x;
    if (g >= P.n_chunks) return;
    int lo = 0, hi = P.n_seq - 1;
    while (lo < hi) {
        const int mid = (lo + hi + 1) >> 1;
        if (P.chunk_off[mid] <= g) lo = mid;
        else hi = mid - 1;
    }
    const int s = lo;
    const int64_t L = P.seq_len[s];
    const int64_t cst = (g - P.chunk_off[s]) * kChunk;
    const int64_t cen = min(cst + kChunk, L);
    const int64_t wst = max((int64_t)0, cst - P.warm);
    const int64_t base = P.seq_start[s];
    const int k = P.k;
    const uint64_t shift1 = 2 * (k - 1), mask = (1ULL << 2 * k) - 1;
    const uint64_t ridhi = P.rid_mode ? ((uint64_t)s << 32) : 0;
    uint64_t km0 = 0, km1 = 0;
    int l = 0, kmer_span = 0;
    uint64_t bx[W], by[W];
#pragma unroll
    for (int j = 0; j < W; j++) bx[j] = by[j] = kMax64;
    uint64_t minx = kMax64, miny = kMax64;
    int64_t step = 0, min_step = -W;
    uint32_t cnt = 0;
    const int64_t out0 = WRITE ? (P.slot_cap ? g * P.slot_cap : P.out_off[g]) : 0;
    const uint32_t lim = P.slot_cap ? (uint32_t)P.slot_cap : 0xffffffffu;
    uint32_t cw = 0, mw = 0;
    auto push = [&](uint64_t x, uint64_t y) {
        if (WRITE && cnt < lim) {
            P.out_x[out0 + cnt] = x;
            P.out_y[out0 + cnt] = y;
        }
        cnt++;
    };
    for (int64_t i = wst; i < cen; ++i) {
        const int64_t pi = base + i;
        if (i == wst || (pi & 15) == 0) cw = P.w2b[pi >> 4];
        if (i == wst || (pi & 31) == 0) mw = P.wm[pi >> 5];
        const bool emit = i >= cst;
        const uint32_t c = (cw >> (2 * (pi & 15))) & 3u;
        const bool bad = (mw >> (pi & 31)) & 1u;
        uint64_t ix = kMax64, iy = kMax64;
        if (!bad) {
            kmer_span = l + 1 < k ? l + 1 : k;
            km0 = (km0 << 2 | c) & mask;
            km1 = (km1 >> 2) | (uint64_t)(3u ^ c) << shift1;
            if (km0 == km1) continue;
            const int z = km0 < km1 ? 0 : 1;
            ++l;
            if (l >= k && kmer_span < 256) {
                ix = hash64m(z ? km1 : km0, mask) << 8 | (uint64_t)kmer_span;
                iy = ridhi | (uint64_t)(uint32_t)i << 1 | (uint64_t)z;
            }
        } else {
            l = 0;
            kmer_span = 0;
        }
#pragma unroll
        for (int j = 0; j < W - 1; j++) {
            bx[j] = bx[j + 1];
            by[j] = by[j + 1];
        }
        bx[W - 1] = ix;
        by[W - 1] = iy;
        if (l == W + k - 1 && minx != kMax64 && emit) {
#pragma unroll
            for (int j = 0; j < W - 1; j++)
                if (minx == bx[j] && by[j] != miny) push(bx[j], by[j]);
        }
        if (ix <= minx) {
            if (l >= W + k && minx != kMax64 && emit) push(minx, miny);
            minx = ix;
            miny = iy;
            min_step = step;
        } else if (min_step == step - W) {
            if (l >= W + k - 1 && minx != kMax64 && emit) push(minx, miny);
            minx = kMax64;
#pragma unroll
            for (int j = 0; j < W; j++)
                if (minx >= bx[j]) {
                    minx = bx[j];
                    miny = by[j];
                    min_step = step - (W - 1 - j);
                }
            if (l >= W + k - 1 && minx != kMax64 && emit) {
#pragma unroll
                for (int j = 0; j < W; j++)
                    if (minx == bx[j] && miny != by[j]) push(bx[j], by[j]);
            }
        }
        ++step;
    }
    if (cen == L && minx != kMax64) push(minx, miny);
    if (!WRITE || P.slot_cap) P.counts[g] = cnt;
    if (WRITE && P.slot_cap && cnt > lim) atomicOr(P.overflow, 1u);
}

__global__ __launch_bounds__(64) void sketch_compact_kernel(const uint64_t *sx, const uint64_t *sy, const uint32_t *cnt,
                                                            const int64_t *off, int slot_cap, uint64_t *ox, uint64_t *oy) {
    const int64_t g = blockIdx.x;
    const int64_t s0 = g * slot_cap, o = off[g];
    for (uint32_t j = threadIdx.x; j < cnt[g]; j += 64) {
        ox[o + j] = sx[s0 + j];
        oy[o + j] = sy[s0 + j];
    }
}

__global__ void bucket_hist_kernel(const uint64_t *__restrict__ x, int64_t n, uint32_t *__restrict__ cnt,
                                   uint32_t *__restrict__ hash_out) {
    const int64_t i = (int64_t)blockIdx.x * blockDim.x + threadIdx.x;
    if (i >= n) return;
    const uint32_t h = (uint32_t)(x[i] >> 8);
    hash_out[i] = h;
    atomicAdd(&cnt[h], 1u);
}

__global__ __launch_bounds__(256) void occ_hist_kernel(const uint32_t *__restrict__ koff, int64_t n_buckets, uint32_t *hist,
                                                       int cap) {
    __shared__ uint32_t sh[256];
    sh[threadIdx.x] = 0;
    __syncthreads();
    uint32_t ones = 0;
    for (int64_t h = (int64_t)blockIdx.x * blockDim.x + threadIdx.x; h < n_buckets;
         h += (int64_t)gridDim.x * blockDim.x) {
        const uint32_t c = koff[h + 1] - koff[h];
        if (c == 1) ones++;
        else if (c > 1 && c < 256) atomicAdd(&sh[c], 1u);
        else if (c >= 256) atomicAdd(&hist[c < (uint32_t)cap ? c : (uint32_t)cap], 1u);
    }
    for (int o = 32; o > 0; o >>= 1) ones += __shfl_xor(ones, o, 64);
    if ((threadIdx.x & 63) == 0) atomicAdd(&sh[1], ones);
    __syncthreads();
    if (sh[threadIdx.x]) atomicAdd(&hist[threadIdx.x], sh[threadIdx.x]);
}

}

int launch_sketch(hymet_ctx *ctx, int w, bool write, const SketchParams &P) {
    if (P.n_chunks <= 0) return HYMET_OK;
    ProfScope _ps(ctx, write ? "mm_sketch_write" : "mm_sketch_count", (double)P.n_chunks * (kChunk * 0.375 + 4.0));
    const dim3 grid((unsigned)cdiv(P.n_chunks, 256)), block(256);
    switch (w) {
#define HY_W(WW)                                                                                   \
    case WW:                                                                                       \
        if (write) hipLaunchKernelGGL((mm_sketch_kernel<WW, true>), grid, block, 0, ctx->stream, P); \
        else hipLaunchKernelGGL((mm_sketch_kernel<WW, false>), grid, block, 0, ctx->stream, P);    \
        break;
        HY_W(2) HY_W(3) HY_W(4) HY_W(5) HY_W(6) HY_W(7) HY_W(8) HY_W(9) HY_W(10) HY_W(11) HY_W(12)
        HY_W(13) HY_W(14) HY_W(15) HY_W(16) HY_W(17) HY_W(18) HY_W(19) HY_W(20) HY_W(24) HY_W(25) HY_W(28) HY_W(32)
#undef HY_W
    default:
        return fail(HYMET_E_ARG, "minimizer window w must be one of 2..20, 24, 25, 28, 32");
    }
    HY_CHECK_LAUNCH("mm_sketch_kernel");
    return HYMET_OK;
}

int sketch_sequences(hymet_ctx *ctx, const uint32_t *d_2b, const uint32_t *d_mask, const int64_t *h_starts,
                     const int64_t *h_lens, int n_seq, int w, int k, int rid_mode, DevBuf &d_x, DevBuf &d_y,
                     int64_t *n_out, DevBuf *d_seq_off) {
    *n_out = 0;
    if (k < 1 || k > 28) return fail(HYMET_E_ARG, "k must be in 1..28 (minimap2)");
    std::vector<int64_t> coff(n_seq + 1, 0);
    for (int i = 0; i < n_seq; i++) coff[i + 1] = coff[i] + (h_lens[i] + kChunk - 1) / kChunk;
    const int64_t n_chunks = coff[n_seq];
    DevBuf d_starts, d_lens, d_coff, d_cnt, d_off;
    HY_HIP(d_starts.alloc(8 * (size_t)n_seq, ctx->stream));
    HY_HIP(d_lens.alloc(8 * (size_t)n_seq, ctx->stream));
    HY_HIP(d_coff.alloc(8 * (size_t)(n_seq + 1), ctx->stream));
    HY_HIP(hipMemcpyAsync(d_starts.p, h_starts, 8 * (size_t)n_seq, hipMemcpyHostToDevice, ctx->stream));
    HY_HIP(hipMemcpyAsync(d_lens.p, h_lens, 8 * (size_t)n_seq, hipMemcpyHostToDevice, ctx->stream));
    HY_HIP(hipMemcpyAsync(d_coff.p, coff.data(), 8 * (size_t)(n_seq + 1), hipMemcpyHostToDevice, ctx->stream));
    HY_HIP(d_cnt.alloc(4 * (size_t)(n_chunks + 1), ctx->stream));
    HY_HIP(d_off.alloc(8 * (size_t)(n_chunks + 1), ctx->stream));
    SketchParams P{};
    P.w2b = d_2b;
    P.wm = d_mask;
    P.seq_start = d_starts.as<int64_t>();
    P.seq_len = d_lens.as<int64_t>();
    P.chunk_off = d_coff.as<int64_t>();
    P.n_chunks = n_chunks;
    P.n_seq = n_seq;
    P.k = k;
    P.warm = w + k + 16;
    P.rid_mode = rid_mode;
    P.counts = d_cnt.as<uint32_t>();
    int64_t total = 0;
    int rc = HYMET_OK;
    constexpr int kSlotCap = kChunk + 64;
    bool done = false;
    if (n_chunks > 0 && (double)n_chunks * kSlotCap * 16.0 <= 2.0e9 && !env_flag("HYMET_SKETCH_TWO_PASS")) {
        DevBuf sx, sy;
        HY_HIP(sx.alloc(8 * (size_t)n_chunks * kSlotCap, ctx->stream));
        HY_HIP(sy.alloc(8 * (size_t)n_chunks * kSlotCap, ctx->stream));
        HY_HIP(hipMemsetAsync(d_cnt.as<uint32_t>() + n_chunks, 0, 4, ctx->stream));
        SketchParams Q = P;
        Q.slot_cap = kSlotCap;
        Q.overflow = d_cnt.as<uint32_t>() + n_chunks;
        Q.out_x = sx.as<uint64_t>();
        Q.out_y = sy.as<uint64_t>();
        rc = launch_sketch(ctx, w, true, Q);
        if (rc) return rc;
        uint32_t ovf = 0;
        HY_HIP(hipMemcpyAsync(&ovf, Q.overflow, 4, hipMemcpyDeviceToHost, ctx->stream));
        rc = exclusive_scan_u32_i64(ctx, d_cnt.as<uint32_t>(), d_off.as<int64_t>(), n_chunks, &total);
        if (rc) return rc;
        if (!ovf) {
            HY_HIP(d_x.alloc(8 * (size_t)total, ctx->stream));
            HY_HIP(d_y.alloc(8 * (size_t)total, ctx->stream));
            hipLaunchKernelGGL(sketch_compact_kernel, dim3((unsigned)n_chunks), dim3(64), 0, ctx->stream, sx.as<uint64_t>(),
                               sy.as<uint64_t>(), d_cnt.as<uint32_t>(), d_off.as<int64_t>(), kSlotCap, d_x.as<uint64_t>(),
                               d_y.as<uint64_t>());
            HY_CHECK_LAUNCH("sketch_compact_kernel");
            done = true;
        }
    }
    if (!done) {
        rc = launch_sketch(ctx, w, false, P);
        if (rc) return rc;
        rc = exclusive_scan_u32_i64(ctx, d_cnt.as<uint32_t>(), d_off.as<int64_t>(), n_chunks, &total);
        if (rc) return rc;
        HY_HIP(d_x.alloc(8 * (size_t)total, ctx->stream));
        HY_HIP(d_y.alloc(8 * (size_t)total, ctx->stream));
        P.out_off = d_off.as<int64_t>();
        P.out_x = d_x.as<uint64_t>();
        P.out_y = d_y.as<uint64_t>();
        rc = launch_sketch(ctx, w, true, P);
        if (rc) return rc;
    }
    if (d_seq_off) {
        std::vector<int64_t> so(n_seq + 1);
        std::vector<int64_t> choff(n_chunks + 1);
        if (n_chunks) HY_HIP(hipMemcpyAsync(choff.data(), d_off.p, 8 * (size_t)n_chunks, hipMemcpyDeviceToHost, ctx->stream));
        HY_HIP(hipStreamSynchronize(ctx->stream));
        choff[n_chunks] = total;
        for (int i = 0; i <= n_seq; i++) so[i] = choff[coff[i]];
        HY_HIP(d_seq_off->alloc(8 * (size_t)(n_seq + 1), ctx->stream));
        HY_HIP(hipMemcpyAsync(d_seq_off->p, so.data(), 8 * (size_t)(n_seq + 1), hipMemcpyHostToDevice, ctx->stream));
        HY_HIP(hipStreamSynchronize(ctx->stream));
    }
    *n_out = total;
    return HYMET_OK;
}

}
}

using namespace hymet;
using namespace hymet::mm;

extern "C" {

int hymet_mm_sketch(hymet_ctx *ctx, const uint32_t *d_2b, const uint32_t *d_mask, const int64_t *h_starts,
                    const int64_t *h_lens, int32_t n_seq, int w, int k, int rid_mode, uint64_t *h_x, uint64_t *h_y,
                    int64_t cap, int64_t *n_out) {
    HY_ARG(ctx && d_2b && d_mask && n_out, "hymet_mm_sketch: null argument");
    HY_HIP(hipSetDevice(ctx->device));
    DevBuf dx, dy;
    int64_t n = 0;
    int rc = sketch_sequences(ctx, d_2b, d_mask, h_starts, h_lens, n_seq, w, k, rid_mode, dx, dy, &n, nullptr);
    if (rc) return rc;
    *n_out = n;
    if (n > cap) return fail(HYMET_E_CAPACITY, "hymet_mm_sketch: output capacity too small");
    if (n) {
        HY_HIP(hipMemcpyAsync(h_x, dx.p, 8 * (size_t)n, hipMemcpyDeviceToHost, ctx->stream));
        HY_HIP(hipMemcpyAsync(h_y, dy.p, 8 * (size_t)n, hipMemcpyDeviceToHost, ctx->stream));
    }
    HY_HIP(hipStreamSynchronize(ctx->stream));
    return HYMET_OK;
}

int hymet_mm_index_build(hymet_ctx *ctx, const uint32_t *d_2b, const uint32_t *d_mask, const int64_t *h_starts,
                         const int64_t *h_lens, int32_t n_seq, int w, int k, hymet_mm_index **out) {
    HY_ARG(ctx && d_2b && d_mask && out, "hymet_mm_index_build: null argument");
    HY_ARG(k >= 1 && k <= 15, "hymet_mm_index_build: direct-address index supports k <= 15 (minimap2 default 15)");
    HY_ARG(n_seq >= 0, "hymet_mm_index_build: n_seq < 0");
    HY_HIP(hipSetDevice(ctx->device));
    hipStream_t st = ctx->stream;
    DevBuf dx, dy;
    int64_t n = 0;
    int rc = sketch_sequences(ctx, d_2b, d_mask, h_starts, h_lens, n_seq, w, k, 1, dx, dy, &n, nullptr);
    if (rc) return rc;
    HY_ARG(n < (1ll << 32), "hymet_mm_index_build: more than 2^32 minimizers in one index part");
    const int64_t nb = 1ll << (2 * k);
    hymet_mm_index *idx = new hymet_mm_index();
    idx->w = w, idx->k = k, idx->n_seq = n_seq, idx->n_pos = n, idx->n_buckets = nb, idx->device = ctx->device;
    idx->h_len.assign(h_lens, h_lens + n_seq);
    auto cleanup = [&](int code) {
        hymet_mm_index_destroy(idx);
        return code;
    };
    if (hipMalloc(&idx->d_koff, 4 * (size_t)(nb + 1)) != hipSuccess || hipMalloc(&idx->d_pos, 8 * (size_t)(n + 1)) != hipSuccess ||
        hipMalloc(&idx->d_hash, 4 * (size_t)(n + 1)) != hipSuccess || hipMalloc(&idx->d_len, 8 * (size_t)(n_seq + 1)) != hipSuccess)
        return cleanup(fail(HYMET_E_HIP, "hymet_mm_index_build: out of device memory"));
    if (n_seq) {
        if (hipMemcpyAsync(idx->d_len, h_lens, 8 * (size_t)n_seq, hipMemcpyHostToDevice, st) != hipSuccess)
            return cleanup(fail(HYMET_E_HIP, "copy lengths"));
    }
    DevBuf cnt, hsh, hsh2, pos2;
    if (cnt.alloc(4 * (size_t)(nb + 1), st) || hsh.alloc(4 * (size_t)(n + 1), st) || hsh2.alloc(4 * (size_t)(n + 1), st) ||
        pos2.alloc(8 * (size_t)(n + 1), st))
        return cleanup(fail(HYMET_E_HIP, "hymet_mm_index_build: out of device memory (scratch)"));
    if (hipMemsetAsync(cnt.p, 0, 4 * (size_t)(nb + 1), st)) return cleanup(fail(HYMET_E_HIP, "memset"));
    if (n) {
        hipLaunchKernelGGL(bucket_hist_kernel, dim3((unsigned)cdiv(n, 256)), dim3(256), 0, st, dx.as<uint64_t>(), n,
                           cnt.as<uint32_t>(), hsh.as<uint32_t>());
        if (hipGetLastError() != hipSuccess) return cleanup(fail(HYMET_E_HIP, "bucket_hist_kernel"));
    }
    {
        DevBuf part;
        if (scan_u32(ctx, cnt.as<uint32_t>(), idx->d_koff, nb + 1, part)) return cleanup(fail(HYMET_E_HIP, "scan"));
    }
    if (n) {
        uint64_t *ky = dy.as<uint64_t>(), *kya = pos2.as<uint64_t>();
        uint32_t *vh = hsh.as<uint32_t>(), *vha = hsh2.as<uint32_t>();
        const int ybits = 32 + bits_for(n_seq);
        if (radix_sort_pairs(ctx, ky, kya, vh, vha, n, 0, std::min(64, ybits))) return cleanup(fail(HYMET_E_HIP, "sort"));
        uint32_t *kh = vh, *kha = vha;
        uint64_t *vy = ky, *vya = kya;
        if (radix_sort_pairs(ctx, kh, kha, vy, vya, n, 0, 2 * k)) return cleanup(fail(HYMET_E_HIP, "sort"));
        if (hipMemcpyAsync(idx->d_hash, kh, 4 * (size_t)n, hipMemcpyDeviceToDevice, st) ||
            hipMemcpyAsync(idx->d_pos, vy, 8 * (size_t)n, hipMemcpyDeviceToDevice, st))
            return cleanup(fail(HYMET_E_HIP, "copy"));
    }
    if (hipStreamSynchronize(st) != hipSuccess) return cleanup(fail(HYMET_E_HIP, "hymet_mm_index_build: sync"));
    *out = idx;
    return HYMET_OK;
}

int hymet_mm_index_destroy(hymet_mm_index *idx) {
    if (!idx) return HYMET_OK;
    (void)hipSetDevice(idx->device);
    if (idx->d_koff) (void)hipFree(idx->d_koff);
    if (idx->d_pos) (void)hipFree(idx->d_pos);
    if (idx->d_hash) (void)hipFree(idx->d_hash);
    if (idx->d_len) (void)hipFree(idx->d_len);
    delete idx;
    return HYMET_OK;
}

int hymet_mm_index_info(const hymet_mm_index *idx, int32_t *w, int32_t *k, int32_t *n_seq, int64_t *n_pos) {
    HY_ARG(idx, "hymet_mm_index_info: null index");
    if (w) *w = idx->w;
    if (k) *k = idx->k;
    if (n_seq) *n_seq = idx->n_seq;
    if (n_pos) *n_pos = idx->n_pos;
    return HYMET_OK;
}

int hymet_mm_index_max_occ(hymet_ctx *ctx, const hymet_mm_index *idx, float frac, int32_t *out) {
    HY_ARG(ctx && idx && out, "hymet_mm_index_max_occ: null argument");
    if (frac <= 0.f) {
        *out = INT32_MAX;
        return HYMET_OK;
    }
    HY_HIP(hipSetDevice(ctx->device));
    const int cap = 1 << 20;
    DevBuf hist;
    HY_HIP(hist.alloc(4 * (size_t)(cap + 1), ctx->stream));
    HY_HIP(hipMemsetAsync(hist.p, 0, 4 * (size_t)(cap + 1), ctx->stream));
    hipLaunchKernelGGL(occ_hist_kernel, dim3(ctx->n_cu * 8), dim3(256), 0, ctx->stream, idx->d_koff, idx->n_buckets,
                       hist.as<uint32_t>(), cap);
    HY_CHECK_LAUNCH("occ_hist_kernel");
    std::vector<uint32_t> h(cap + 1);
    HY_HIP(hipMemcpyAsync(h.data(), hist.p, 4 * (size_t)(cap + 1), hipMemcpyDeviceToHost, ctx->stream));
    HY_HIP(hipStreamSynchronize(ctx->stream));
    uint64_t n_keys = 0;
    for (int c = 1; c <= cap; c++) n_keys += h[c];
    if (n_keys == 0) {
        *out = INT32_MAX;
        return HYMET_OK;
    }
    const uint64_t kk = (uint64_t)(uint32_t)((1. - frac) * (double)n_keys);
    uint64_t acc = 0;
    int val = cap;
    for (int c = 1; c <= cap; c++) {
        acc += h[c];
        if (acc > kk) {
            val = c;
            break;
        }
    }
    HY_ARG(val < cap, "hymet_mm_index_max_occ: occurrence above histogram range");
    *out = val + 1;
    return HYMET_OK;
}

static const char kIxMagic[8] = {'H', 'Y', 'M', 'E', 'T', 'I', 'X', '1'};

int hymet_mm_index_save(hymet_ctx *ctx, const hymet_mm_index *idx, const char *path, int append, int64_t *end_offset) {
    HY_ARG(ctx && idx && path, "hymet_mm_index_save: null argument");
    HY_HIP(hipSetDevice(ctx->device));
    FILE *fp = fopen(path, append ? "ab" : "wb");
    if (!fp) return fail(HYMET_E_ARG, std::string("hymet_mm_index_save: cannot open ") + path);
    const int32_t hdr[4] = {idx->w, idx->k, idx->n_seq, 0};
    const int64_t n = idx->n_pos;
    bool ok = fwrite(kIxMagic, 1, 8, fp) == 8 && fwrite(hdr, 4, 4, fp) == 4 && fwrite(&n, 8, 1, fp) == 1 &&
              (idx->n_seq == 0 || fwrite(idx->h_len.data(), 8, (size_t)idx->n_seq, fp) == (size_t)idx->n_seq);
    const int64_t chunk = 1 << 24;
    std::vector<uint64_t> buf;
    for (int pass = 0; ok && pass < 2; pass++) {
        const size_t es = pass == 0 ? 4 : 8;
        buf.resize((size_t)std::min<int64_t>(n, chunk) + 1);
        for (int64_t a = 0; ok && a < n; a += chunk) {
            const int64_t m = std::min<int64_t>(chunk, n - a);
            const void *src = pass == 0 ? (const void *)(idx->d_hash + a) : (const void *)(idx->d_pos + a);
            if (hipMemcpy(buf.data(), src, es * (size_t)m, hipMemcpyDeviceToHost) != hipSuccess) {
                fclose(fp);
                return fail(HYMET_E_HIP, "hymet_mm_index_save: copy");
            }
            ok = fwrite(buf.data(), es, (size_t)m, fp) == (size_t)m;
        }
    }
    if (end_offset) *end_offset = (int64_t)ftell(fp);
    if (fclose(fp) != 0 || !ok) return fail(HYMET_E_ARG, std::string("hymet_mm_index_save: write failed: ") + path);
    return HYMET_OK;
}

__global__ void koff_gap_kernel(const uint32_t *__restrict__ hash, int64_t n, uint32_t *__restrict__ koff) {
    const int64_t i = (int64_t)blockIdx.x * blockDim.x + threadIdx.x;
    if (i >= n) return;
    const int64_t prev = i ? (int64_t)hash[i - 1] : -1;
    for (int64_t b = prev + 1; b <= (int64_t)hash[i]; b++) koff[b] = (uint32_t)i;
}

__global__ void koff_tail_kernel(int64_t from, int64_t to, uint32_t v, uint32_t *__restrict__ koff) {
    for (int64_t b = from + (int64_t)blockIdx.x * blockDim.x + threadIdx.x; b <= to; b += (int64_t)gridDim.x * blockDim.x)
        koff[b] = v;
}

int hymet_mm_index_load(hymet_ctx *ctx, const char *path, int64_t offset, hymet_mm_index **out, int64_t *end_offset) {
    HY_ARG(ctx && path && out, "hymet_mm_index_load: null argument");
    HY_HIP(hipSetDevice(ctx->device));
    hipStream_t st = ctx->stream;
    FILE *fp = fopen(path, "rb");
    if (!fp) return fail(HYMET_E_ARG, std::string("hymet_mm_index_load: cannot open ") + path);
    char mg[8];
    int32_t hdr[4];
    int64_t n = 0;
    if (fseeko(fp, offset, SEEK_SET) != 0 || fread(mg, 1, 8, fp) != 8 || memcmp(mg, kIxMagic, 8) != 0 ||
        fread(hdr, 4, 4, fp) != 4 || fread(&n, 8, 1, fp) != 1 || hdr[1] < 1 || hdr[1] > 15 || hdr[2] < 0 || n < 0 ||
        n >= (1ll << 32)) {
        fclose(fp);
        return fail(HYMET_E_ARG, std::string("hymet_mm_index_load: not a hymet index part: ") + path);
    }
    hymet_mm_index *idx = new hymet_mm_index();
    idx->w = hdr[0], idx->k = hdr[1], idx->n_seq = hdr[2], idx->n_pos = n, idx->n_buckets = 1ll << (2 * hdr[1]);
    idx->device = ctx->device;
    idx->h_len.resize(idx->n_seq);
    auto bad = [&](int code, const char *what) {
        fclose(fp);
        hymet_mm_index_destroy(idx);
        return fail(code, std::string("hymet_mm_index_load: ") + what);
    };
    if (idx->n_seq && fread(idx->h_len.data(), 8, (size_t)idx->n_seq, fp) != (size_t)idx->n_seq) return bad(HYMET_E_ARG, "truncated");
    const int64_t nb = idx->n_buckets;
    if (hipMalloc(&idx->d_koff, 4 * (size_t)(nb + 1)) != hipSuccess || hipMalloc(&idx->d_pos, 8 * (size_t)(n + 1)) != hipSuccess ||
        hipMalloc(&idx->d_hash, 4 * (size_t)(n + 1)) != hipSuccess || hipMalloc(&idx->d_len, 8 * (size_t)(idx->n_seq + 1)) != hipSuccess)
        return bad(HYMET_E_HIP, "out of device memory");
    if (idx->n_seq && hipMemcpy(idx->d_len, idx->h_len.data(), 8 * (size_t)idx->n_seq, hipMemcpyHostToDevice) != hipSuccess)
        return bad(HYMET_E_HIP, "copy lengths");
    const int64_t chunk = 1 << 24;
    std::vector<uint64_t> buf((size_t)std::min<int64_t>(std::max<int64_t>(n, 1), chunk));
    for (int pass = 0; pass < 2; pass++) {
        const size_t es = pass == 0 ? 4 : 8;
        for (int64_t a = 0; a < n; a += chunk) {
            const int64_t m = std::min<int64_t>(chunk, n - a);
            if (fread(buf.data(), es, (size_t)m, fp) != (size_t)m) return bad(HYMET_E_ARG, "truncated");
            void *dst = pass == 0 ? (void *)(idx->d_hash + a) : (void *)(idx->d_pos + a);
            if (hipMemcpy(dst, buf.data(), es * (size_t)m, hipMemcpyHostToDevice) != hipSuccess) return bad(HYMET_E_HIP, "copy");
        }
    }
    if (end_offset) *end_offset = (int64_t)ftello(fp);
    fclose(fp);
    if (n > 0) {
        uint32_t last = 0;
        if (hipMemcpy(&last, idx->d_hash + n - 1, 4, hipMemcpyDeviceToHost) != hipSuccess) return bad(HYMET_E_HIP, "copy");
        hipLaunchKernelGGL(koff_gap_kernel, dim3((unsigned)cdiv(n, 256)), dim3(256), 0, st, idx->d_hash, n, idx->d_koff);
        hipLaunchKernelGGL(koff_tail_kernel, dim3(ctx->n_cu * 8), dim3(256), 0, st, (int64_t)last + 1, nb, (uint32_t)n,
                           idx->d_koff);
    } else {
        hipLaunchKernelGGL(koff_tail_kernel, dim3(ctx->n_cu * 8), dim3(256), 0, st, (int64_t)0, nb, 0u, idx->d_koff);
    }
    if (hipGetLastError() != hipSuccess || hipStreamSynchronize(st) != hipSuccess) {
        hymet_mm_index_destroy(idx);
        return fail(HYMET_E_HIP, "hymet_mm_index_load: offsets kernel");
    }
    *out = idx;
    return HYMET_OK;
}

int hymet_mm_index_export(hymet_ctx *ctx, const hymet_mm_index *idx, uint32_t *h_hash, uint64_t *h_pos) {
    HY_ARG(ctx && idx && h_hash && h_pos, "hymet_mm_index_export: null argument");
    HY_HIP(hipSetDevice(ctx->device));
    if (idx->n_pos) {
        HY_HIP(hipMemcpyAsync(h_hash, idx->d_hash, 4 * (size_t)idx->n_pos, hipMemcpyDeviceToHost, ctx->stream));
        HY_HIP(hipMemcpyAsync(h_pos, idx->d_pos, 8 * (size_t)idx->n_pos, hipMemcpyDeviceToHost, ctx->stream));
    }
    HY_HIP(hipStreamSynchronize(ctx->stream));
    return HYMET_OK;
}

}
```

### hymet_amd/csrc/mm_stages.hpp

```cpp
#pragma once
#include "mm_common.hpp"
#include "sort.hpp"

namespace hymet {
namespace mm {

#define LAUNCH1(kern, n, ...)                                                                           \
    do {                                                                                                \
        if ((n) > 0) {                                                                                  \
            hipLaunchKernelGGL(kern, dim3((unsigned)cdiv((n), 256)), dim3(256), 0, ctx->stream, __VA_ARGS__); \
            HY_CHECK_LAUNCH(#kern);                                                                     \
        }                                                                                               \
    } while (0)

namespace {

__device__ __forceinline__ int upper_idx(const int64_t *off, int n, int64_t v) {
    int lo = 0, hi = n - 1;
    while (lo < hi) {
        const int mid = (lo + hi + 1) >> 1;
        if (off[mid] <= v) lo = mid;
        else hi = mid - 1;
    }
    return lo;
}

__global__ void iota_u32_kernel(uint32_t *a, int64_t n) {
    const int64_t i = (int64_t)blockIdx.x * blockDim.x + threadIdx.x;
    if (i < n) a[i] = (uint32_t)i;
}

template <typename T>
__global__ void gather_kernel(const T *__restrict__ src, const uint32_t *__restrict__ idx, T *__restrict__ dst, int64_t n) {
    const int64_t i = (int64_t)blockIdx.x * blockDim.x + threadIdx.x;
    if (i < n) dst[i] = src[idx[i]];
}

}

template <typename K, typename V, int RB = 0>
static int sort_pairs(hymet_ctx *ctx, K *&keys, K *&keys_alt, V *&vals, V *&vals_alt, int64_t n, int begin_bit, int end_bit,
                      const char *tag = "radix_sort") {
    if (n <= 1) return HYMET_OK;
    ProfScope _ps(ctx, tag, 2.0 * (double)n * (sizeof(K) + sizeof(V)) * (double)((end_bit - begin_bit + 7) / 8));
    return radix_sort_pairs(ctx, keys, keys_alt, vals, vals_alt, n, begin_bit, end_bit);
}

inline int scan_flags(hymet_ctx *ctx, const uint32_t *flag, int64_t n, DevBuf &pos, int64_t *total) {
    HY_HIP(pos.alloc(8 * (size_t)(n + 1), ctx->stream));
    return exclusive_scan_u32_i64(ctx, flag, pos.as<int64_t>(), n, total);
}

inline int64_t anchor_cap() { return env_int("HYMET_ANCHOR_CAP", INT32_MAX - 1, 1, INT32_MAX - 1); }

struct AnchorSet {
    DevBuf ax;
    DevBuf ay;
    int span = 0;
    int64_t n = 0;
    DevBuf d_off;
    DevBuf hb;
    bool has_hb = false;
    DevBuf ax32;
    bool has_x32 = false;
};

struct ChainSet {
    DevBuf cu, cboff;
    DevBuf ids, cfirst;
    const uint64_t *ax = nullptr;
    const uint32_t *ay = nullptr;
    int span = 0;
    DevBuf bx, by, bchain;
    DevBuf cq;
    int64_t n_anchor = 0, n_chain = 0;
    DevBuf d_qc, d_qb;
};

struct LeanJoin {
    const int64_t *qlen;
    int rescue_size;
    float rescue_ratio;
    bool mark_only;
    DevBuf flag;
    DevBuf mark;
    DevBuf qb2;
    int64_t n2 = 0;
};

int chain_set(hymet_ctx *ctx, const hymet_mm_opt *opt, float pen_gap, float pen_skip, int bw, AnchorSet &A, int n_q,
              ChainSet &C, LeanJoin *lj = nullptr, bool copy = false);
int marked_anchor_set(hymet_ctx *ctx, const AnchorSet &S1, const LeanJoin &lj, const uint32_t *flag, int n_q, int64_t A2,
                      AnchorSet &S2);

}
}
```

### hymet_amd/pipeline.py

```python
from __future__ import annotations

import ctypes
import hashlib
import os
import time
from dataclasses import dataclass, field
from typing import Dict, List, Optional, Sequence

import numpy as np

from . import classify as cls
from . import mapper as mp
from . import screen as scr
from . import select as sel
from ._lib import check, ptr
from .ingest import FastaIndex, QueryShard, shard_bytes
from .msh import SketchDB, read_msh
from .seqio import SeqSet

_c = ctypes
TSV_HEADER = b"Query\tLineage\tTaxonomic Level\tConfidence\r\n"


@dataclass
class Config:
    mash_thresh: str = "0.9"
    cand_max: int = 5000
    dedupe: bool = False
    split_idx: str = "2g"
    index_mini_batch: float = 50e6
    w: int = 10
    k: int = 15
    map_batch_bases: int = 40_000_000
    map_streams: int = 2
    n_input_files: int = 1
    limit: bool = True
    screen_winner: bool = False
    reload_inputs: bool = True


@dataclass
class IndexSet:
    names: List[str]
    lens: np.ndarray
    parts: List[mp.IndexPart]
    part_first: List[int]
    opt: mp.MapOpt
    dev: Dict[str, object] = field(default_factory=dict)


class HostText:

    def __init__(self, buf, n: int):
        self._buf, self.n, self._bytes = buf, int(n), None

    def view(self) -> memoryview:
        if self._bytes is not None:
            return memoryview(self._bytes)
        return memoryview(self._buf)[:self.n]

    def bytes(self) -> bytes:
        if self._bytes is None:
            self._bytes = bytes(memoryview(self._buf)[:self.n])
            self._buf = None
        return self._bytes

    detach = bytes


@dataclass
class RunResult:
    selected: List[str]
    screen_rows: List[List[str]]
    thresholds: List[str]
    tsv: bytes
    n_queries: int
    n_classified: int
    n_paf_lines: int
    paf_text: Optional[object] = None
    screen: Optional[list] = None

    @property
    def paf_bytes(self) -> Optional[bytes]:
        t = self.paf_text
        return t.bytes() if isinstance(t, HostText) else t

    @property
    def paf(self) -> Optional[List[str]]:
        if self.paf_bytes is None:
            return None
        return self.paf_bytes.decode().split("\n")[:-1] if self.paf_bytes else []


class PafAcc:

    def __init__(self, gpu):
        self.gpu = gpu
        h = _c.c_void_p()
        check(gpu.lib.hymet_paf_acc_create(gpu.ctx, _c.byref(h)), "hymet_paf_acc_create")
        self.h = h

    def reset(self):
        check(self.gpu.lib.hymet_paf_acc_reset(self.h), "hymet_paf_acc_reset")

    @property
    def n(self) -> int:
        n = _c.c_int64()
        check(self.gpu.lib.hymet_paf_acc_info(self.h, _c.byref(n), None, None, None, None, None), "hymet_paf_acc_info")
        return n.value

    def columns(self):
        n = self.n
        q, part, t = (np.zeros(max(n, 1), np.int32) for _ in range(3))
        check(self.gpu.lib.hymet_paf_acc_copy(self.gpu.ctx, self.h, q.ctypes.data_as(_c.c_void_p),
                                              part.ctypes.data_as(_c.c_void_p), t.ctypes.data_as(_c.c_void_p)),
              "hymet_paf_acc_copy")
        return q[:n], part[:n], t[:n]

    def close(self):
        if getattr(self, "h", None):
            self.gpu.lib.hymet_paf_acc_destroy(self.h)
            self.h = None

    def __del__(self):
        try:
            self.close()
        except Exception:
            pass


def make_index_set(gpu, names, lens, parts, first) -> IndexSet:
    torch = gpu.torch
    opt = mp.MapOpt.asm10()
    opt.resolve_mid_occ(parts[0])
    ix = IndexSet(list(names), np.asarray(lens, np.int64), list(parts), list(first), opt)
    tb = [n.encode() for n in ix.names]
    toff = np.zeros(len(tb) + 1, np.int64)
    np.cumsum([len(b) for b in tb], out=toff[1:])
    ix.dev = {"tname": torch.frombuffer(bytearray(b"".join(tb) or b"\0"), dtype=torch.uint8).to(gpu.dev),
              "tname_off": torch.from_numpy(toff).to(gpu.dev),
              "tlen": torch.from_numpy(ix.lens.copy()).to(gpu.dev)}
    return ix


def map_shard(gpu, ix: IndexSet, sh: QueryShard, acc: PafAcc) -> int:
    acc.reset()
    starts = np.ascontiguousarray(sh.starts, np.int64)
    lens = np.ascontiguousarray(sh.lengths, np.int64)
    hbase = sh.name_hash.data_ptr()
    for pi, part in enumerate(ix.parts):
        for b0, b1 in sh.batches:
            n = b1 - b0
            if n <= 0:
                continue
            gpu.call("hymet_mm_map_acc", part.h, _c.byref(ix.opt), ptr(sh.mm.w2b), ptr(sh.mm.wmask),
                     _c.c_void_p(starts.ctypes.data + 8 * b0), _c.c_void_p(lens.ctypes.data + 8 * b0),
                     _c.c_void_p(hbase + 4 * b0), n, b0, pi, ix.part_first[pi], acc.h)
    return acc.n


def map_shard_streams(gpus, accs, ix: IndexSet, sh: QueryShard, acc: PafAcc) -> int:
    import threading
    tasks = [(pi, b0, b1) for pi in range(len(ix.parts)) for b0, b1 in sh.batches if b1 > b0]
    segs = [None] * len(tasks)
    errs = []
    starts = np.ascontiguousarray(sh.starts, np.int64)
    lens = np.ascontiguousarray(sh.lengths, np.int64)
    hbase = sh.name_hash.data_ptr()

    def work(w):
        g, a = gpus[w], accs[w]
        try:
            a.reset()
            for ti in range(w, len(tasks), len(gpus)):
                pi, b0, b1 = tasks[ti]
                before = a.n
                g.call("hymet_mm_map_acc", ix.parts[pi].h, _c.byref(ix.opt), ptr(sh.mm.w2b), ptr(sh.mm.wmask),
                       _c.c_void_p(starts.ctypes.data + 8 * b0), _c.c_void_p(lens.ctypes.data + 8 * b0),
                       _c.c_void_p(hbase + 4 * b0), b1 - b0, b0, pi, ix.part_first[pi], a.h)
                segs[ti] = (w, before, a.n)
        except Exception as e:
            errs.append(e)

    th = [threading.Thread(target=work, args=(w,)) for w in range(len(gpus))]
    for t in th:
        t.start()
    for t in th:
        t.join()
    if errs:
        raise errs[0]
    acc.reset()
    g0 = acc.gpu
    for w, b, e in segs:
        g0.call("hymet_paf_acc_append", acc.h, accs[w].h, b, e)
    return acc.n


def _dev_buf(gpu, bufs, key, nbytes):
    b = bufs.get(key)
    if b is None or b.numel() < nbytes:
        bufs.pop(key, None)
        b = gpu.empty(max(int(nbytes), 16), gpu.torch.uint8)
        bufs[key] = b
    return b


_bytes_new = _c.pythonapi.PyBytes_FromStringAndSize
_bytes_new.restype = _c.py_object
_bytes_new.argtypes = [_c.c_void_p, _c.c_ssize_t]


def _to_host(gpu, bufs, key, dev, n, prefix: bytes = b"") -> bytes:
    if n == 0:
        return bytes(prefix)
    m = len(prefix)
    b = _bytes_new(None, int(n) + m)
    addr = _c.cast(_c.c_char_p(b), _c.c_void_p).value
    if m:
        _c.memmove(addr, prefix, m)
    check(gpu.lib.hymet_copy_to_host(gpu.ctx, addr + m, ptr(dev), int(n), 16), "hymet_copy_to_host")
    return b


def emit_paf_bytes(gpu, ix: IndexSet, sh: QueryShard, acc: PafAcc, bufs) -> bytes:
    n = acc.n
    if n == 0:
        return b""
    nb = _c.c_int64()
    cap = 200 * n
    while True:
        out = _dev_buf(gpu, bufs, "paf", cap)
        rc = gpu.lib.hymet_emit_paf(gpu.ctx, acc.h, ptr(sh.qname), ptr(sh.qname_off), ptr(sh.qlen), ptr(ix.dev["tname"]),
                                    ptr(ix.dev["tname_off"]), ptr(ix.dev["tlen"]), ptr(out), cap, _c.byref(nb), None)
        if rc == -3:
            cap = nb.value
            continue
        check(rc, "hymet_emit_paf")
        break
    return _to_host(gpu, bufs, "paf_h", out, nb.value)


def run_beside(loader, main):
    if loader is None:
        return main()
    import threading
    err = []

    def body():
        try:
            loader()
        except BaseException as e:
            err.append(e)
    th = threading.Thread(target=body, name="hymet-inputs")
    th.start()
    try:
        out = main()
    finally:
        th.join()
    if err:
        raise err[0]
    return out


class Pipeline:
    def __init__(self, gpu, dbs: Sequence[SketchDB], ref_lookup, taxonomy, hierarchy, cfg: Config = None, comm=None,
                 variant: int = cls.CAMI):
        """dbs: SketchDB objects (tables built once) or .msh paths (read by the native
        reader and rebuilt into HBM tables on every run when cfg.reload_inputs, as `mash
        screen` reads its DB per call)."""
        self.gpu, self.cfg, self.comm = gpu, cfg or Config(), comm
        self.db_paths = [str(d) for d in dbs] if dbs and all(isinstance(d, (str, os.PathLike)) for d in dbs) else None
        self.dbs = [] if self.db_paths else list(dbs)
        self.tables = [scr.ScreenTable(gpu, db) for db in self.dbs]
        self.ref_lookup = ref_lookup
        self.taxonomy, self.hierarchy, self.variant = taxonomy, hierarchy, variant
        self.timings: Dict[str, float] = {}
        self._pin: Dict[int, object] = {}
        self._load_classifier()
        if self.db_paths:
            self._load_dbs()
        self.index_cache: Dict[str, IndexSet] = {}
        self.opt: Optional[mp.MapOpt] = None
        self.acc = PafAcc(gpu)
        self.map_gpus = [gpu.fork() for _ in range(self.cfg.map_streams)] if self.cfg.map_streams > 1 else []
        self.map_accs = [PafAcc(g) for g in self.map_gpus]
        self._bufs: Dict[str, object] = {}
        self._paf_pin = [None, None]
        self._paf_holders = [None, None]
        self._ran = False

    def _pinned_hashes(self, i, n):
        torch = self.gpu.torch
        b = self._pin.get(i)
        if b is None or b.numel() < n:
            b = torch.empty(int(n), dtype=torch.int64, pin_memory=True)
            self._pin[i] = b
        return b

    def _load_dbs(self):
        self._read_dbs()
        self._build_tables()

    def _read_dbs(self, side=None):
        self.tables, self.dbs = [], []
        t0 = time.perf_counter()
        dbs = []
        shard = (self.rank, self.world) if side is not None and self.world > 1 else None
        for i, p in enumerate(self.db_paths):
            pin = lambda n, i=i: self._pinned_hashes(i, n).numpy().view(np.uint64)[:n]
            if side is None:
                dbs.append(read_msh(p, alloc=pin))
            else:
                with self.gpu.torch.cuda.stream(side.stream):
                    dbs.append(read_msh(p, alloc=pin, upload=(side, lambda n: side.empty(n, side.torch.int64)),
                                        shard=shard, defer_meta=True))
        self.dbs = dbs
        self.timings["msh_read_s"] = time.perf_counter() - t0
        for k in ("open", "meta", "hashes"):
            self.timings[f"msh_{k}_s"] = sum(getattr(db, "load_s", {}).get(k, 0.0) for db in dbs)

    def _build_tables(self, side=None):
        t1 = time.perf_counter()
        if side is None:
            self._finish_meta()
            self.tables = [scr.ScreenTable(self.gpu, db, pinned=self._pin[i]) for i, db in enumerate(self.dbs)]
            self.gpu.sync()
        else:
            with self.gpu.torch.cuda.stream(side.stream):
                self.tables = [scr.ScreenTable(side, db, pinned=self._pin[i]) for i, db in enumerate(self.dbs)]
            self.timings["screen_table_enqueue_s"] = time.perf_counter() - t1
            self._finish_meta()
            side.stream.synchronize()
        self.timings["screen_table_s"] = time.perf_counter() - t1

    def _finish_meta(self):
        for db in self.dbs:
            if getattr(db, "finish_meta", None) is not None:
                db.finish_meta()

    def _read_inputs(self, side=None):
        import threading
        err = []

        def classifier():
            try:
                self._load_classifier(side)
            except BaseException as e:
                err.append(e)
        th = threading.Thread(target=classifier, name="hymet-taxonomy")
        th.start()
        try:
            if self.db_paths:
                self._read_dbs(side)
                if side is not None and self._sliced():
                    if not self._db_gather_main():
                        self._join_slices(side)
                elif side is not None:
                    self._build_tables(side)
        finally:
            self._finish_meta()
            th.join()
        if err:
            raise err[0]

    def _sliced(self):
        return any(getattr(db, "dev_slice", None) is not None for db in self.dbs)

    @staticmethod
    def _db_gather_main() -> bool:
        return os.environ.get("HYMET_DB_GATHER", "loader") == "main"

    def _join_slices(self, side):
        t0 = time.perf_counter()
        with self.comm.owned():
            with self.gpu.torch.cuda.stream(side.stream):
                for i, db in enumerate(self.dbs):
                    if db.dev_slice is not None and db.dev_hashes is not None:
                        self.comm.allgather_slices_(db.dev_hashes, db.dev_slice[2], key=i)
            self.timings["msh_allgather_s"] = time.perf_counter() - t0
            self._build_tables(side)

    def _load_classifier(self, side=None):
        t0 = time.perf_counter()
        try:
            self.classifier = cls.Classifier(self.gpu, self.taxonomy, self.hierarchy, self.variant)
            self.classifier_error = None
        except Exception as e:
            self.classifier, self.classifier_error = None, e
        if self.classifier is not None and side is not None:
            torch = self.gpu.torch
            with torch.cuda.stream(side.stream):
                self.classifier.device_tables(None)
            side.stream.synchronize()
        self.timings["classifier_load_s"] = time.perf_counter() - t0

    def load_inputs(self):
        if self.db_paths:
            self._load_dbs()
        self._load_classifier()

    @property
    def world(self) -> int:
        return self.comm.world if self.comm is not None else 1

    @property
    def rank(self) -> int:
        return self.comm.rank if self.comm is not None else 0

    def ingest(self, queries, defer_base: bool = False) -> QueryShard:
        if isinstance(queries, QueryShard):
            return queries
        d_all = None
        if isinstance(queries, (bytes, bytearray, memoryview)):
            data = bytes(queries)
            if self.world > 1:
                b0, b1 = shard_bytes(data, self.rank, self.world)
                d_rng, fx = self._upload_while(data, b0, b1, lambda: FastaIndex(data, byte_range=(b0, b1)))
                sh = QueryShard.from_fasta(self.gpu, fx, 0, fx.n, self.cfg.map_batch_bases, q_base=0,
                                           d_all=d_rng, d_base=b0)
                sh.fasta, sh.fasta_r0 = fx, 0
                sh.byte_sharded = True
                sh.q_base = None
                if not defer_base:
                    self.shard_base(sh)
                return sh
            if len(data):
                d_all, queries = self._upload_while(data, 0, len(data), lambda: FastaIndex(data))
            else:
                queries = FastaIndex(data)
        if isinstance(queries, FastaIndex):
            r0, r1 = queries.shard(self.rank, self.world)
            sh = QueryShard.from_fasta(self.gpu, queries, r0, r1, self.cfg.map_batch_bases,
                                       d_all=d_all if (r0, r1) == (0, queries.n) else None)
            sh.fasta, sh.fasta_r0 = queries, r0
            return sh
        if isinstance(queries, SeqSet):
            if self.world > 1:
                raise ValueError("multi-rank runs take the FASTA bytes (every rank shards the same input)")
            return QueryShard.from_seqset(self.gpu, queries, 0, self.cfg.map_batch_bases)
        raise TypeError(f"unsupported query input {type(queries)!r}")

    prepare = ingest

    def shard_base(self, sh: QueryShard) -> int:
        if sh.q_base is None:
            counts = self.comm.allgather_np(np.array([sh.n], np.int64), tag="shard_records")
            sh.q_base = int(sum(int(c[0]) for c in counts[:self.rank]))
        return sh.q_base

    def _upload_while(self, data: bytes, b0: int, b1: int, scan):
        import threading
        torch = self.gpu.torch
        d = self.gpu.empty(max(b1 - b0, 1), torch.uint8)
        up_err = []

        def upload():
            try:
                if b1 > b0:
                    src = ctypes.cast(ctypes.c_char_p(data), ctypes.c_void_p).value + b0
                    check(self.gpu.lib.hymet_copy_to_device(self.gpu.ctx, ptr(d), ctypes.c_void_p(src), b1 - b0, 16),
                          "hymet_copy_to_device")
            except BaseException as e:
                up_err.append(e)
        up = threading.Thread(target=upload, name="hymet-upload")
        up.start()
        try:
            out = scan()
        finally:
            up.join()
        if up_err:
            raise up_err[0]
        return d, out

    def screen_select(self, pool):
        t0 = time.perf_counter()
        res = scr.screen(self.gpu, pool, self.dbs, self.tables, self.comm, winner=self.cfg.screen_winner)
        self.last_screen = res
        ph = getattr(self, "phases", None)
        if ph is not None:
            ph["screen_only_s"] = ph.get("screen_only_s", 0.0) + time.perf_counter() - t0
        rows, thr, selections = [], [], []
        for r in res:
            s = sel.sort_gr(sel.sort_unique_k5(r.lines(v_max=0.9)))
            t, top, names = sel.select_threshold(s, self.cfg.mash_thresh, self.cfg.n_input_files)
            rows.append(s)
            thr.append(t)
            selections.append(names)
        selected = sel.union_sorted(*selections)
        if not self.cfg.limit:
            return selected, rows, thr
        scores = sel.best_scores(rows)
        limited = sel.limit(selected, scores, self.cfg.cand_max, self.cfg.dedupe)
        return limited, rows, thr

    def index_for(self, selected: List[str]) -> IndexSet:
        key = hashlib.sha1(("".join(n + "\n" for n in selected)).encode()).hexdigest()
        if key in self.index_cache:
            return self.index_cache[key]
        refs: SeqSet = self.ref_lookup(selected)
        parts_idx = mp.split_parts(refs.lengths, float(mp.parse_num(self.cfg.split_idx)), self.cfg.index_mini_batch)
        parts, first = [], []
        for p in parts_idx:
            sub = refs.subset(p) if len(parts_idx) > 1 else refs
            parts.append(mp.IndexPart(self.gpu, sub, self.cfg.w, self.cfg.k))
            first.append(int(p[0]))
        ix = make_index_set(self.gpu, list(refs.names), refs.lengths, parts, first)
        self.index_cache = {key: ix}
        return ix

    def map_all(self, ix: IndexSet, sh: QueryShard) -> int:
        self.opt = ix.opt
        if self.map_gpus:
            self.gpu.sync()
            return map_shard_streams(self.map_gpus, self.map_accs, ix, sh, self.acc)
        return map_shard(self.gpu, ix, sh, self.acc)

    def classify_rows(self, ix: IndexSet, sh: QueryShard):
        gpu, torch = self.gpu, self.gpu.torch
        tabs = self.classifier.device_tables(ix.names)
        counts = gpu.zeros(max(len(ix.names), 1), torch.int32)
        gpu.call("hymet_acc_ref_counts", self.acc.h, ptr(counts))
        if self.world > 1:
            self.comm.allreduce_sum_(counts)
        n_q = max(sh.n, 1)
        rq, rp, rd, rt = (gpu.zeros(n_q, torch.int32) for _ in range(4))
        rn = gpu.zeros(n_q * 8, torch.int32)
        rc = gpu.zeros(n_q, torch.float64)
        nr = _c.c_int32()
        legacy = self.variant == cls.LEGACY
        gpu.call("hymet_acc_classify", self.acc.h, self.variant, sh.n, ptr(sh.qlen), ptr(counts), ptr(tabs["t_tax"]),
                 ptr(tabs["tax_names"]), ptr(tabs["in_hier"]), ptr(sh.qname) if legacy else None,
                 ptr(sh.qname_off) if legacy else None, ptr(ix.dev["tname"]) if legacy else None,
                 ptr(ix.dev["tname_off"]) if legacy else None, ptr(rq), ptr(rp), ptr(rd), ptr(rn), ptr(rc), ptr(rt),
                 _c.byref(nr))
        R = nr.value
        return {"q": rq[:R], "part": rp[:R], "depth": rd[:R], "names": rn[:R * 8], "conf": rc[:R], "tax": rt[:R]}, R

    def emit_tsv(self, rows, R, qname, qname_off) -> bytes:
        gpu = self.gpu
        tabs = self.classifier.device_tables(None)
        legacy = self.variant == cls.LEGACY
        nb = _c.c_int64()
        cap = max(256 * R, 1 << 16)
        while True:
            out = self._dev_buf("tsv", cap)
            rc = gpu.lib.hymet_emit_tsv(gpu.ctx, self.variant, R, ptr(rows["q"]), ptr(rows["depth"]), ptr(rows["names"]),
                                        ptr(rows["conf"]), ptr(rows["tax"]), ptr(qname), ptr(qname_off), ptr(tabs["label"]),
                                        ptr(tabs["label_off"]), ptr(tabs["taxlin"]) if legacy else None,
                                        ptr(tabs["taxlin_off"]) if legacy else None,
                                        ptr(tabs["taxlvl"]) if legacy else None,
                                        ptr(tabs["taxlvl_off"]) if legacy else None, ptr(out), cap, _c.byref(nb))
            if rc == -3:
                cap = nb.value
                continue
            check(rc, "hymet_emit_tsv")
            break
        return self._to_host("tsv_h", out, nb.value, prefix=TSV_HEADER)

    def emit_paf(self, ix: IndexSet, sh: QueryShard) -> HostText:
        gpu, torch = self.gpu, self.gpu.torch
        if getattr(self, "_paf_copy", None) is not None:
            self._paf_copy.synchronize()
            self._paf_copy = None
        n = self.acc.n
        if n == 0:
            return HostText(b"", 0)
        nb = _c.c_int64()
        cap = 200 * n
        while True:
            out = self._dev_buf("paf", cap)
            rc = gpu.lib.hymet_emit_paf(gpu.ctx, self.acc.h, ptr(sh.qname), ptr(sh.qname_off), ptr(sh.qlen),
                                        ptr(ix.dev["tname"]), ptr(ix.dev["tname_off"]), ptr(ix.dev["tlen"]), ptr(out), cap,
                                        _c.byref(nb), None)
            if rc == -3:
                cap = nb.value
                continue
            check(rc, "hymet_emit_paf")
            break
        m = nb.value
        slot = self._paf_slot = (getattr(self, "_paf_slot", 1) + 1) % 2
        holder = self._paf_holders[slot]() if self._paf_holders[slot] is not None else None
        if holder is not None:
            holder.detach()
        buf = self._paf_pin[slot]
        if buf is None or buf.numel() < m:
            for s_ in (slot, 1 - slot):
                b_ = self._paf_pin[s_]
                if b_ is None or b_.numel() < m:
                    h_ = self._paf_holders[s_]() if self._paf_holders[s_] is not None else None
                    if h_ is not None:
                        h_.detach()
                    self._paf_pin[s_] = None
                    self._paf_pin[s_] = torch.empty(int(m * 1.25) + 4096, dtype=torch.uint8, pin_memory=True)
            buf = self._paf_pin[slot]
        if self.map_gpus:
            side = self.map_gpus[0].stream
            ev = torch.cuda.Event()
            ev.record(gpu.bound_stream)
            side.wait_event(ev)
            with torch.cuda.stream(side):
                buf[:m].copy_(out[:m], non_blocking=True)
            self._paf_copy = side
        else:
            gpu.sync()
            buf[:m].copy_(out[:m])
        t = HostText(buf.numpy(), m)
        import weakref
        self._paf_holders[slot] = weakref.ref(t)
        return t

    def _dev_buf(self, key, nbytes):
        return _dev_buf(self.gpu, self._bufs, key, nbytes)

    def _to_host(self, key, dev, n, prefix: bytes = b"") -> bytes:
        return _to_host(self.gpu, self._bufs, key, dev, n, prefix)

    def run(self, queries, with_paf=False) -> RunResult:
        side = self.map_gpus[0] if self.map_gpus else None
        reader = self.cfg.reload_inputs and self._ran
        self._ran = True
        ph = self.phases = {}
        tp = [time.perf_counter()]

        def lap(name):
            t = time.perf_counter()
            ph[name] = ph.get(name, 0.0) + t - tp[0]
            tp[0] = t

        def read():
            t0 = time.perf_counter()
            try:
                self._read_inputs(side)
            finally:
                self.timings["reader_s"] = time.perf_counter() - t0

        def ingest():
            sh_ = self.ingest(queries, defer_base=True)
            lap("ingest_s")
            return sh_
        sh = run_beside(read if reader else None, ingest)
        lap("input_wait_s")
        if getattr(sh, "byte_sharded", False):
            self.shard_base(sh)
        if reader and self.db_paths and side is None:
            self._build_tables()
        elif reader and side is not None and not self.tables and self._sliced():
            self._join_slices(side)
            lap("db_join_s")
        selected, rows, thr = self.screen_select(sh.mash)
        if not selected:
            raise RuntimeError("candidate list empty after applying limit")
        lap("screen_select_s")
        ix = self.index_for(selected)
        n_lines = self.map_all(ix, sh)
        lap("map_s")
        paf_text = self.emit_paf(ix, sh) if with_paf else None
        lap("emit_paf_s")
        tsv, n_rows, n_cls = b"", 0, 0
        if self.classifier is not None:
            rws, R = self.classify_rows(ix, sh)
            lap("classify_s")
            if self.world > 1:
                rws, R = self.comm.gather_rows(rws, sh.q_base, self.gpu)
                qname, qname_off = self._global_names(sh)
            else:
                qname, qname_off = sh.qname, sh.qname_off
            lap("gather_rows_s")
            if self.rank == 0:
                tsv = self.emit_tsv(rws, R, qname, qname_off)
                n_rows = R
                n_cls = int((rws["depth"] != 0).sum().item()) if R else 0
            lap("emit_tsv_s")
        total_rows = self.comm.broadcast_obj(n_rows) if self.world > 1 else n_rows
        if total_rows < 1:
            tsv = self._fallback(ix, sh)
            n_rows = n_cls = 0
        if getattr(self, "_paf_copy", None) is not None:
            self._paf_copy.synchronize()
            self._paf_copy = None
        lap("finish_s")
        return RunResult(selected, rows, thr, tsv, n_rows, n_cls, n_lines, paf_text, self.last_screen)

    def _global_names(self, sh: QueryShard):
        fx = sh.fasta
        if getattr(sh, "byte_sharded", False):
            return self.comm.gather_name_pools(sh.qname, sh.qname_off, sh.n)
        if self._bufs.get("names_of") is not fx:
            torch = self.gpu.torch
            pool, off = fx.name_pool()
            self._bufs["names"] = (torch.from_numpy(pool.copy() if len(pool) else np.zeros(1, np.uint8)).to(self.gpu.dev),
                                   torch.from_numpy(off).to(self.gpu.dev))
            self._bufs["names_of"] = fx
        return self._bufs["names"]

    def _fallback(self, ix: IndexSet, sh: QueryShard) -> bytes:
        from . import fallback
        q, part, t = self.acc.columns()
        if sh.names_host is not None:
            names = sh.names_host
        else:
            names = sh.fasta.names()[sh.fasta_r0:sh.fasta_r0 + sh.n]
        pairs = [(names[int(a)], ix.names[int(b)]) for a, b in zip(q, t)]
        if self.world > 1:
            got = self.comm.gather_obj([(int(p_), sh.q_base + int(a), j, pa[0], pa[1])
                                        for j, (p_, a, pa) in enumerate(zip(part, q, pairs))])
            if self.rank != 0:
                return b""
            pairs = [(x[3], x[4]) for x in sorted(y for g in got for y in g)]
        tsv = fallback.fallback_tsv(pairs, self.taxonomy)
        if tsv.count(b"\n") < 2:
            raise RuntimeError("classification still empty after fallback")
        return tsv
```

### include/hymet_gpu.h

```cpp
#ifndef HYMET_GPU_H
#define HYMET_GPU_H

#include <stdint.h>

#ifdef __cplusplus
extern "C" {
#endif

#define HYMET_OK 0
#define HYMET_E_HIP (-1)
#define HYMET_E_ARG (-2)
#define HYMET_E_CAPACITY (-3)
#define HYMET_E_INTERNAL (-4)

typedef struct hymet_ctx hymet_ctx;

int hymet_init(int device, hymet_ctx **out);
int hymet_destroy(hymet_ctx *ctx);
const char *hymet_last_error(void);
int hymet_set_stream(hymet_ctx *ctx, void *hip_stream);
int hymet_sync(hymet_ctx *ctx);
int hymet_version(void);
int hymet_prof_enable(hymet_ctx *ctx, int on);
int hymet_prof_reset(hymet_ctx *ctx);
int hymet_prof_query(hymet_ctx *ctx, const char *name, double *total_ms, int64_t *count, double *alg_bytes);
int hymet_prof_names(hymet_ctx *ctx, char *buf, int64_t cap);
int hymet_scratch_trim(hymet_ctx *ctx, int64_t *freed_bytes);
int hymet_scratch_cached(hymet_ctx *ctx, int64_t *bytes);
int hymet_scratch_reserve(hymet_ctx *ctx, int64_t bytes);
int hymet_set_oom_hook(void (*hook)(void *user), void *user);
int hymet_scratch_stats(hymet_ctx *ctx, int64_t *counts);
int hymet_copy_to_host(hymet_ctx *ctx, void *dst, const void *src, int64_t n, int threads);
int hymet_copy_to_device(hymet_ctx *ctx, void *dst, const void *src, int64_t n, int threads);

int hymet_pack(hymet_ctx *ctx, const uint8_t *d_ascii, int64_t n, int alphabet,
               uint32_t *d_2b, uint32_t *d_mask);

int hymet_fasta_index(const char *h_buf, int64_t n, int threads, int64_t cap, int64_t *n_rec, int64_t *h_name_off,
                      int32_t *h_name_len, int64_t *h_seq_off, int64_t *h_seq_end, int64_t *h_nbases);
int hymet_fasta_names(const char *h_buf, const int64_t *h_name_off, const int32_t *h_name_len, int64_t n, char *h_pool,
                      int64_t *h_pool_off);
int hymet_fasta_compact(hymet_ctx *ctx, const uint8_t *d_raw, int64_t raw_len, int64_t raw_base, const int64_t *h_seq_off,
                        const int64_t *h_seq_end, const int64_t *h_nbases, int64_t n_rec, uint8_t *d_pool,
                        int64_t pool_len, int64_t *d_pool_start);
int hymet_name_hash(hymet_ctx *ctx, const uint8_t *d_raw, const int64_t *d_name_off, const int32_t *d_name_len, int64_t n,
                    uint32_t *d_hash);

int64_t hymet_screen_table_slots(int64_t n_hashes);
int hymet_screen_table_build(hymet_ctx *ctx, const uint64_t *d_hashes, int64_t n_hashes,
                             uint64_t *d_table, int64_t n_slots, int64_t *d_scratch, int32_t *d_canon_of,
                             int key_bits);
int hymet_sort_pairs_u64(hymet_ctx *ctx, uint64_t *d_keys, uint32_t *d_vals, int64_t n, int begin_bit, int end_bit);

int hymet_scan_u32(hymet_ctx *ctx, const uint32_t *d_in, int64_t *d_out, int64_t n, int mode, int64_t *total);

typedef struct hymet_msh hymet_msh;
typedef struct {
    int32_t k, window_size, sketch_size;
    uint32_t seed;
    int32_t noncanonical, preserve_case, use64;
    int64_t n_refs, n_hashes, names_bytes, comments_bytes, alphabet_len;
} hymet_msh_info;
int hymet_msh_open(const char *path, hymet_msh **out);
int hymet_msh_info_get(const hymet_msh *m, hymet_msh_info *info);
int hymet_msh_copy(const hymet_msh *m, int threads, uint64_t *hashes, int64_t *offsets, int64_t *lengths,
                   char *names, char *comments, char *alphabet);
int hymet_msh_text_offsets(const hymet_msh *m, int64_t *name_start, int64_t *comment_start);
int hymet_msh_upload(hymet_ctx *ctx, const hymet_msh *m, int threads, uint64_t *pinned, uint64_t *d_hashes,
                     int n_chunks);
int hymet_msh_upload_range(hymet_ctx *ctx, const hymet_msh *m, int threads, uint64_t *pinned, uint64_t *d_hashes,
                           int n_chunks, int64_t lo_h, int64_t hi_h);
void hymet_msh_close(hymet_msh *m);
int hymet_screen_count(hymet_ctx *ctx, const uint32_t *d_2b, const uint32_t *d_mask,
                       int64_t n_bases, int64_t pos_begin, int64_t pos_end, int k, uint32_t seed,
                       int ndb, const uint64_t *const *h_d_tables, const int64_t *h_n_slots,
                       const uint64_t *const *h_d_hashes, const int64_t *h_n_hashes,
                       uint32_t *const *h_d_counts, uint64_t cand_thr, uint64_t *d_cand,
                       int64_t cand_cap, unsigned long long *d_cand_n,
                       unsigned long long *d_nkmers);
int hymet_screen_stats(hymet_ctx *ctx, const int64_t *d_ref_off, int64_t n_refs,
                       const int32_t *d_canon_of, const uint32_t *d_counts, uint32_t *d_shared,
                       uint32_t *d_median);
int hymet_screen_winner(hymet_ctx *ctx, const int64_t *d_ref_off, int64_t n_refs,
                        const int32_t *d_canon_of, const uint32_t *d_counts, int64_t n_hashes,
                        const int32_t *d_comp, int64_t n_comp, uint32_t *d_win, uint32_t *d_shared,
                        uint32_t *d_median);

int64_t hymet_sketch_max_size(void);
int hymet_sketch_batch(hymet_ctx *ctx, const uint32_t *d_2b, const uint32_t *d_mask, int64_t n_bases,
                       int k, uint32_t seed, int32_t s, int64_t n_chunks, const int32_t *h_chunk_sketch,
                       const int64_t *h_chunk_begin, const int64_t *h_chunk_end, int32_t n_sketches,
                       uint64_t *d_out, int32_t *d_out_n);

int hymet_mash_dist(hymet_ctx *ctx, const uint64_t *d_ref_hashes, int64_t n_ref_hashes, const int64_t *d_ref_off,
                    int64_t n_ref, const uint64_t *d_qry_hashes, int64_t n_qry_hashes, const int64_t *d_qry_off,
                    int64_t n_qry, int64_t q_begin, int64_t q_end, int32_t s, uint32_t *d_out);
int hymet_mash_dist_tile(int32_t s);
int hymet_mash_dist_tune(int path, int tq);
int hymet_mash_dist_select(hymet_ctx *ctx, const uint32_t *d_block, int64_t n_rows, int64_t n_ref,
                           const uint16_t *d_min_common, int32_t s, int64_t *d_row_off, int32_t *d_ref_idx,
                           uint32_t *d_val, int64_t cap, int64_t *total);
int hymet_mash_dist_tri(hymet_ctx *ctx, const uint64_t *d_hashes, int64_t n_hashes, const int64_t *d_off, int64_t n,
                        int64_t q_begin, int64_t q_end, int32_t s, uint32_t *d_out);
int hymet_mash_link(hymet_ctx *ctx, const uint32_t *d_block, int64_t n_rows, int64_t n, int64_t q_begin,
                    const uint16_t *d_min_common, int32_t s, int32_t *d_parent, uint64_t *d_n_links);
int hymet_mash_labels(hymet_ctx *ctx, int32_t *d_parent, int64_t n, int32_t *d_label);

typedef struct hymet_mm_index hymet_mm_index;
int hymet_mm_sketch(hymet_ctx *ctx, const uint32_t *d_2b, const uint32_t *d_mask, const int64_t *h_starts,
                    const int64_t *h_lens, int32_t n_seq, int w, int k, int rid_mode, uint64_t *h_x,
                    uint64_t *h_y, int64_t cap, int64_t *n_out);
int hymet_mm_index_build(hymet_ctx *ctx, const uint32_t *d_2b, const uint32_t *d_mask, const int64_t *h_starts,
                         const int64_t *h_lens, int32_t n_seq, int w, int k, hymet_mm_index **out);
int hymet_mm_index_destroy(hymet_mm_index *idx);
int hymet_mm_index_info(const hymet_mm_index *idx, int32_t *w, int32_t *k, int32_t *n_seq, int64_t *n_pos);
int hymet_mm_index_max_occ(hymet_ctx *ctx, const hymet_mm_index *idx, float frac, int32_t *out);
int hymet_mm_index_save(hymet_ctx *ctx, const hymet_mm_index *idx, const char *path, int append, int64_t *end_offset);
int hymet_mm_index_load(hymet_ctx *ctx, const char *path, int64_t offset, hymet_mm_index **out, int64_t *end_offset);
int hymet_mm_index_export(hymet_ctx *ctx, const hymet_mm_index *idx, uint32_t *h_hash, uint64_t *h_pos);

typedef struct {
    int32_t mid_occ;
    float q_occ_frac;
    int32_t max_max_occ, occ_dist;
    int32_t min_cnt, min_chain_score;
    int32_t bw, bw_long, max_gap, max_chain_skip;
    int32_t rmq_inner_dist, rmq_size_cap, rmq_rescue_size;
    float rmq_rescue_ratio;
    float chain_gap_scale, chain_skip_scale;
    float mask_level, pri_ratio;
    int32_t mask_len, best_n, a, b, seed;
} hymet_mm_opt;

typedef struct {
    int32_t qs, qe, rs, re, rid, rev;
    int32_t mlen, blen, mapq, cnt, score, subsc, parent, id, n_sub, strand_retained;
    float div;
    int32_t as;
    uint32_t hash;
    int32_t pad;
} hymet_mm_reg;

typedef struct hymet_mm_result hymet_mm_result;
int hymet_mm_map(hymet_ctx *ctx, const hymet_mm_index *idx, const hymet_mm_opt *opt,
                 const uint32_t *d_2b, const uint32_t *d_mask, const int64_t *h_starts,
                 const int64_t *h_lens, const uint32_t *h_name_hash, int32_t n_q,
                 hymet_mm_result **out);
int hymet_mm_result_size(const hymet_mm_result *res, int64_t *n_regs);
int hymet_mm_result_copy(const hymet_mm_result *res, int64_t *h_off, int32_t *h_rep_len,
                         hymet_mm_reg *h_regs);
int hymet_mm_result_destroy(hymet_mm_result *res);
typedef struct hymet_paf_acc hymet_paf_acc;
int hymet_paf_acc_create(hymet_ctx *ctx, hymet_paf_acc **out);
int hymet_paf_acc_reset(hymet_paf_acc *acc);
int hymet_paf_acc_destroy(hymet_paf_acc *acc);
int hymet_paf_acc_info(const hymet_paf_acc *acc, int64_t *n_lines, void **d_regs, void **d_q, void **d_part, void **d_rl,
                       void **d_t);
int hymet_paf_acc_append(hymet_ctx *ctx, hymet_paf_acc *dst, const hymet_paf_acc *src, int64_t begin, int64_t end);
int hymet_paf_acc_copy(hymet_ctx *ctx, const hymet_paf_acc *acc, int32_t *h_q, int32_t *h_part, int32_t *h_t);
int hymet_paf_acc_field(hymet_ctx *ctx, const hymet_paf_acc *acc, int field, int32_t *h_out);
int hymet_mm_map_acc(hymet_ctx *ctx, const hymet_mm_index *idx, const hymet_mm_opt *opt, const uint32_t *d_2b,
                     const uint32_t *d_mask, const int64_t *h_starts, const int64_t *h_lens, const uint32_t *d_name_hash,
                     int32_t n_q, int32_t q_base, int32_t part_id, int32_t t_base, hymet_paf_acc *acc);
int hymet_emit_paf(hymet_ctx *ctx, const hymet_paf_acc *acc, const uint8_t *d_qname, const int64_t *d_qname_off,
                   const int64_t *d_qlen, const uint8_t *d_tname, const int64_t *d_tname_off, const int64_t *d_tlen,
                   char *d_out, int64_t cap, int64_t *n_bytes, int64_t *d_line_off);
int hymet_mm_chain_dp(hymet_ctx *ctx, const uint64_t *h_x, const uint64_t *h_y, int64_t n, int max_dist,
                      int max_dist_inner, int bw, int max_chn_skip, int cap_rmq_size, float pen_gap,
                      float pen_skip, int32_t *h_f, int64_t *h_p);
int hymet_mm_mark_compact(hymet_ctx *ctx, const uint64_t *h_x, const uint64_t *h_y, const int32_t *h_mark, int64_t n,
                          const int64_t *h_qoff, const uint32_t *h_qflag, int32_t n_q, uint64_t *h_ox, uint64_t *h_oy,
                          uint32_t *h_ohb, int64_t *n_kept);
int hymet_mm_stamp_scratch(hymet_ctx *ctx, int64_t *capacity, int64_t *nonzero);
int hymet_mm_anchor_sort(hymet_ctx *ctx, const uint64_t *h_key, const uint32_t *h_val, int64_t n,
                         const int64_t *h_qoff, int32_t n_q, int32_t rb, int32_t pb, uint64_t yhi, int64_t max_qlen,
                         uint64_t *h_ax, uint64_t *h_ay, uint32_t *h_ax32, uint32_t *h_hb, int64_t *h_stats);

int hymet_lca_ref_counts(hymet_ctx *ctx, const int32_t *d_line_t, int64_t n_lines, int32_t *d_counts);
int hymet_acc_ref_counts(hymet_ctx *ctx, const hymet_paf_acc *acc, int32_t *d_counts);
int hymet_acc_classify(hymet_ctx *ctx, const hymet_paf_acc *acc, int mode, int32_t n_q, const int64_t *d_qlen,
                       const int32_t *d_ref_counts, const int32_t *d_t_tax, const int32_t *d_tax_names,
                       const uint8_t *d_tax_in_hier, const uint8_t *d_qname_pool, const int64_t *d_qname_off,
                       const uint8_t *d_tname_pool, const int64_t *d_tname_off, int32_t *d_row_q, int32_t *d_row_part,
                       int32_t *d_row_depth, int32_t *d_row_names, double *d_row_conf, int32_t *d_row_tax,
                       int32_t *n_rows);
int hymet_emit_tsv(hymet_ctx *ctx, int mode, int32_t n_rows, const int32_t *d_row_q, const int32_t *d_row_depth,
                   const int32_t *d_row_names, const double *d_row_conf, const int32_t *d_row_tax, const uint8_t *d_qname,
                   const int64_t *d_qname_off, const uint8_t *d_label, const int64_t *d_label_off, const uint8_t *d_taxlin,
                   const int64_t *d_taxlin_off, const uint8_t *d_taxlvl, const int64_t *d_taxlvl_off, char *d_out,
                   int64_t cap, int64_t *n_bytes);
int hymet_lca(hymet_ctx *ctx, int mode, int32_t n_q, const int64_t *d_q_off, const int32_t *d_line_t,
              const int64_t *d_line_blen, const int64_t *d_line_qlen, const uint8_t *d_line_exact,
              const int32_t *d_ref_counts, const int32_t *d_t_tax, const int32_t *d_tax_names,
              const uint8_t *d_tax_in_hier, int32_t *d_scr_tid, double *d_scr_w, int32_t *d_scr_nm,
              double *d_scr_nw, int32_t *d_out_depth, int32_t *d_out_names, double *d_out_conf,
              int32_t *d_out_tax);

#ifdef __cplusplus
}
#endif
#endif
```

Before: 136,400.

## Sketch query batch once and reuse it across all index partitions

```diff
diff --git a/hymet_amd/_lib.py b/hymet_amd/_lib.py
--- a/hymet_amd/_lib.py
+++ b/hymet_amd/_lib.py
@@ -77,6 +77,11 @@
     "hymet_paf_acc_copy": (_i32, [_vp, _vp, _vp, _vp, _vp]),
     "hymet_paf_acc_field": (_i32, [_vp, _vp, _i32, _vp]),
     "hymet_mm_map_acc": (_i32, [_vp, _vp, _vp, _vp, _vp, _vp, _vp, _vp, _i32, _i32, _i32, _i32, _vp]),
+    "hymet_mm_qsketch_create": (_i32, [_vp, _vp, _i32, _i32, _vp, _vp, _vp, _vp, _i32, _c.POINTER(_vp)]),
+    "hymet_mm_qsketch_destroy": (_i32, [_vp]),
+    "hymet_mm_map_acc_qs": (_i32, [_vp, _vp, _vp, _vp, _vp, _i32, _i32, _i32, _vp]),
+    "hymet_mm_qsketch_copy": (_i32, [_vp, _c.POINTER(_i64), _vp, _vp, _vp]),
+    "hymet_mm_qsketch_live": (_i32, [_vp, _c.POINTER(_i64)]),
     "hymet_emit_paf": (_i32, [_vp, _vp, _vp, _vp, _vp, _vp, _vp, _vp, _vp, _i64, _c.POINTER(_i64), _vp]),
     "hymet_acc_ref_counts": (_i32, [_vp, _vp, _vp]),
     "hymet_acc_classify": (_i32, [_vp, _vp, _i32, _i32] + [_vp] * 15 + [_c.POINTER(_i32)]),
diff --git a/hymet_amd/csrc/common.hpp b/hymet_amd/csrc/common.hpp
--- a/hymet_amd/csrc/common.hpp
+++ b/hymet_amd/csrc/common.hpp
@@ -27,6 +27,7 @@
     int32_t *stamp = nullptr;
     int64_t stamp_cap = 0;
     size_t stamp_cls = 0;
+    int64_t qs_live = 0;
 };
 
 namespace hymet {
diff --git a/hymet_amd/csrc/mm_map.hip b/hymet_amd/csrc/mm_map.hip
--- a/hymet_amd/csrc/mm_map.hip
+++ b/hymet_amd/csrc/mm_map.hip
@@ -684,56 +684,61 @@
     hymet_ctx *ctx;
     const hymet_mm_index *idx;
     const hymet_mm_opt *opt;
-    const int64_t *h_lens;
-    int32_t n_q;
-    DevBuf mx, my, qm_off;
-    int64_t M = 0;
-    DevBuf d_qlen, d_hash_buf;
+    const hymet_mm_qsketch &qs;
+    const int32_t n_q;
+    const uint64_t *const mx, *const my;
+    const int64_t *const qm_off;
+    const int64_t M;
+    const uint32_t *const qid;
+    const int64_t *const d_qlen;
+    const int64_t *const d_qbase;
+    const int64_t max_qlen;
+    DevBuf d_hash_buf;
     const uint32_t *d_hash = nullptr;
-    DevBuf seed_n, rep_len, qid;
+    DevBuf seed_n, rep_len;
     DevBuf mini_pos, mp_off;
     int64_t NM = 0;
-    DevBuf d_qbase, pos_tab;
-    std::vector<int64_t> qbase;
-    int64_t max_qlen = 1;
+    DevBuf pos_tab;
+    MapBatch(hymet_ctx *c, const hymet_mm_index *i, const hymet_mm_opt *o, const hymet_mm_qsketch &s)
+        : ctx(c), idx(i), opt(o), qs(s), n_q(s.n_q), mx(s.mx.as<uint64_t>()), my(s.my.as<uint64_t>()),
+          qm_off(s.qm_off.as<int64_t>()), M(s.M), qid(s.qid.as<uint32_t>()), d_qlen(s.d_qlen.as<int64_t>()),
+          d_qbase(s.d_qbase.as<int64_t>()), max_qlen(s.max_qlen) {}
     int rb = 0, pb = 0, key1_bits = 0;
     bool key_path = false;
     int ybits = 0;
 };
 
-static int sketch_queries(MapBatch &B, const uint32_t *d_2b, const uint32_t *d_mask, const int64_t *h_starts,
-                          const uint32_t *h_name_hash, const uint32_t *d_name_hash) {
-    hipStream_t st = B.ctx->stream;
-    const int n_q = B.n_q;
-    int rc = sketch_sequences(B.ctx, d_2b, d_mask, h_starts, B.h_lens, n_q, B.idx->w, B.idx->k, 0, B.mx, B.my, &B.M, &B.qm_off);
-    if (rc) return rc;
-    HY_HIP(B.d_qlen.alloc(8 * (size_t)n_q, st));
-    HY_HIP(hipMemcpyAsync(B.d_qlen.p, B.h_lens, 8 * (size_t)n_q, hipMemcpyHostToDevice, st));
-    B.d_hash = d_name_hash;
-    if (!B.d_hash) {
-        HY_HIP(B.d_hash_buf.alloc(4 * (size_t)n_q, st));
-        HY_HIP(hipMemcpyAsync(B.d_hash_buf.p, h_name_hash, 4 * (size_t)n_q, hipMemcpyHostToDevice, st));
-        B.d_hash = B.d_hash_buf.as<uint32_t>();
-    }
-    return HYMET_OK;
-}
-
-static int filter_minimizers(MapBatch &B) {
-    hymet_ctx *ctx = B.ctx;
+static int sketch_queries(hymet_mm_qsketch &Q, const uint32_t *d_2b, const uint32_t *d_mask, const int64_t *h_starts,
+                          const int64_t *h_lens) {
+    hipStream_t st = Q.ctx->stream;
+    const int n_q = Q.n_q;
+    Q.qbase.assign(n_q + 1, 0);
+    for (int q = 0; q < n_q; q++) {
+        Q.qbase[q + 1] = Q.qbase[q] + ((h_lens[q] + 63) & ~(int64_t)63);
+        Q.max_qlen = std::max<int64_t>(Q.max_qlen, h_lens[q]);
+    }
+    HY_HIP(Q.d_qlen.alloc(8 * (size_t)n_q, st));
+    HY_HIP(hipMemcpyAsync(Q.d_qlen.p, h_lens, 8 * (size_t)n_q, hipMemcpyHostToDevice, st));
+    HY_HIP(Q.d_qbase.alloc(8 * (size_t)(n_q + 1), st));
+    HY_HIP(hipMemcpyAsync(Q.d_qbase.p, Q.qbase.data(), 8 * (size_t)(n_q + 1), hipMemcpyHostToDevice, st));
+    return sketch_sequences(Q.ctx, d_2b, d_mask, h_starts, h_lens, n_q, Q.w, Q.k, 0, Q.mx, Q.my, &Q.M, &Q.qm_off);
+}
+
+static int filter_minimizers(hymet_mm_qsketch &Q) {
+    hymet_ctx *ctx = Q.ctx;
     hipStream_t st = ctx->stream;
-    const hymet_mm_opt *opt = B.opt;
-    const int n_q = B.n_q;
-    const int64_t M = B.M;
-    DevBuf &mx = B.mx, &my = B.my, &qm_off = B.qm_off;
+    const int n_q = Q.n_q;
+    const int64_t M = Q.M;
+    DevBuf &mx = Q.mx, &my = Q.my, &qm_off = Q.qm_off;
     DevBuf keep, fcnt, fcoff;
     int64_t MF = 0;
     int rc;
-    if (opt->q_occ_frac > 0.0f && M > 0 && opt->mid_occ > 0) {
+    if (Q.q_occ_frac > 0.0f && M > 0 && Q.mid_occ > 0) {
         HY_HIP(keep.alloc(4 * (size_t)M, st));
         HY_HIP(fcnt.alloc(4 * (size_t)(n_q + 1), st));
         ctx->mbox_h[kMbFlag] = 0;
         hipLaunchKernelGGL(mzflt_screen_kernel, dim3((unsigned)n_q + 1), dim3(256), 0, st, mx.as<uint64_t>(), qm_off.as<int64_t>(),
-                           n_q, opt->mid_occ, keep.as<uint32_t>(), fcnt.as<uint32_t>(), mb_dev(ctx, kMbFlag));
+                           n_q, Q.mid_occ, keep.as<uint32_t>(), fcnt.as<uint32_t>(), mb_dev(ctx, kMbFlag));
         HY_CHECK_LAUNCH("mzflt_screen_kernel");
         HY_HIP(hipStreamSynchronize(st));
         if (mb_read(ctx, kMbFlag) != 0) {
@@ -757,7 +762,7 @@
     LAUNCH1(iota_u32_kernel, MF, sidx.as<uint32_t>(), MF);
     uint64_t *kx = sx.as<uint64_t>(), *kxa = sx2.as<uint64_t>();
     uint32_t *vi = sidx.as<uint32_t>(), *via = sidx2.as<uint32_t>();
-    rc = sort_pairs(ctx, kx, kxa, vi, via, MF, 0, 2 * B.idx->k + 8, "radix_sort_mz");
+    rc = sort_pairs(ctx, kx, kxa, vi, via, MF, 0, 2 * Q.k + 8, "radix_sort_mz");
     if (rc) return rc;
     HY_HIP(sq.alloc(4 * (size_t)MF, st));
     HY_HIP(sq2.alloc(4 * (size_t)MF, st));
@@ -768,8 +773,8 @@
     HY_HIP(gx.alloc(8 * (size_t)MF, st));
     HY_HIP(gg.alloc(4 * (size_t)MF, st));
     LAUNCH1(mzflt_gather_kernel, MF, vi, gidx.as<uint32_t>(), mx.as<uint64_t>(), gg.as<uint32_t>(), gx.as<uint64_t>(), MF);
-    LAUNCH1(mzflt_runs_kernel, MF, kq, gx.as<uint64_t>(), gg.as<uint32_t>(), qm_off.as<int64_t>(), MF, opt->mid_occ,
-            opt->q_occ_frac, keep.as<uint32_t>());
+    LAUNCH1(mzflt_runs_kernel, MF, kq, gx.as<uint64_t>(), gg.as<uint32_t>(), qm_off.as<int64_t>(), MF, Q.mid_occ,
+            Q.q_occ_frac, keep.as<uint32_t>());
     int64_t M2 = 0;
     rc = scan_flags(ctx, keep.as<uint32_t>(), M, kpos, &M2);
     if (rc) return rc;
@@ -785,7 +790,7 @@
     mx.swap(nx);
     my.swap(ny);
     qm_off.swap(nqm);
-    B.M = M2;
+    Q.M = M2;
     return HYMET_OK;
 }
 
@@ -795,15 +800,13 @@
     const hymet_mm_opt *opt = B.opt;
     const int n_q = B.n_q;
     const int64_t M = B.M;
-    DevBuf &mx = B.mx, &my = B.my, &qm_off = B.qm_off, &seed_n = B.seed_n, &rep_len = B.rep_len, &qid = B.qid;
+    DevBuf &seed_n = B.seed_n, &rep_len = B.rep_len;
     HY_HIP(seed_n.alloc(4 * (size_t)(M + 1), st));
     HY_HIP(rep_len.alloc(4 * (size_t)n_q, st));
-    HY_HIP(qid.alloc(4 * (size_t)(M + 1), st));
-    LAUNCH1(fill_qid_kernel, std::max<int64_t>(M, n_q), qm_off.as<int64_t>(), n_q, M, qid.as<uint32_t>(), nullptr,
-            rep_len.as<int32_t>());
+    HY_HIP(hipMemsetAsync(rep_len.p, 0, 4 * (size_t)n_q, st));
     {
         ProfScope _ps(ctx, "mm_seed_count", (double)M * (8.0 + 8.0 + 4.0));
-        LAUNCH1(seed_count_kernel, M, mx.as<uint64_t>(), M, B.idx->d_koff, B.idx->n_buckets, seed_n.as<uint32_t>());
+        LAUNCH1(seed_count_kernel, M, B.mx, M, B.idx->d_koff, B.idx->n_buckets, seed_n.as<uint32_t>());
     }
     if (M == 0) return HYMET_OK;
     ProfScope _ps(ctx, "mm_seed_select", (double)M * (4.0 + 8.0 + 8.0 + 8.0));
@@ -823,7 +826,7 @@
     HY_HIP(flt_high.alloc(4 * (size_t)n_high, st));
     LAUNCH1(seed_list_kernel, M, seed_n.as<uint32_t>(), rank.as<uint64_t>(), M, opt->mid_occ, low_idx.as<int32_t>(),
             high_idx.as<int32_t>());
-    StreakParams S{my.as<uint64_t>(), qid.as<uint32_t>(), qm_off.as<int64_t>(), B.d_qlen.as<int64_t>(),
+    StreakParams S{B.my, B.qid, B.qm_off, B.d_qlen,
                    rank.as<uint64_t>(), low_idx.as<int32_t>(), high_idx.as<int32_t>(), n_low, n_q, opt->mid_occ,
                    opt->max_max_occ, opt->occ_dist, seed_n.as<uint32_t>(), flt_high.as<uint32_t>()};
     HY_HIP(hipMemsetAsync(flt_high.p, 0, 4 * (size_t)n_high, st));
@@ -837,28 +840,19 @@
         if (rc) return rc;
     }
     LAUNCH1(rep_len_kernel, n_high, flt_high.as<uint32_t>(), pmax.as<int32_t>(), high_idx.as<int32_t>(), n_high,
-            mx.as<uint64_t>(), my.as<uint64_t>(), qid.as<uint32_t>(), rep_len.as<int32_t>(), seed_n.as<uint32_t>());
+            B.mx, B.my, B.qid, rep_len.as<int32_t>(), seed_n.as<uint32_t>());
     return HYMET_OK;
 }
 
 static int build_mini_table(MapBatch &B, const DevBuf &mp_pos) {
     hymet_ctx *ctx = B.ctx;
     hipStream_t st = ctx->stream;
-    const int n_q = B.n_q;
-    B.qbase.assign(n_q + 1, 0);
-    for (int q = 0; q < n_q; q++) {
-        B.qbase[q + 1] = B.qbase[q] + ((B.h_lens[q] + 63) & ~(int64_t)63);
-        B.max_qlen = std::max<int64_t>(B.max_qlen, B.h_lens[q]);
-    }
-    HY_HIP(B.d_qbase.alloc(8 * (size_t)(n_q + 1), st));
-    HY_HIP(hipMemcpyAsync(B.d_qbase.p, B.qbase.data(), 8 * (size_t)(n_q + 1), hipMemcpyHostToDevice, st));
-    const size_t n_words = (size_t)(B.qbase[n_q] >> 6) + 1;
+    const size_t n_words = (size_t)(B.qs.qbase[B.n_q] >> 6) + 1;
     HY_HIP(B.pos_tab.alloc(sizeof(MiniWord) * n_words, st));
     HY_HIP(hipMemsetAsync(B.pos_tab.p, 0, sizeof(MiniWord) * n_words, st));
-    LAUNCH1(mini_bits_kernel, B.M, B.my.as<uint64_t>(), B.seed_n.as<uint32_t>(), B.qid.as<uint32_t>(), B.d_qbase.as<int64_t>(),
-            B.M, B.pos_tab.as<MiniWord>());
-    LAUNCH1(mini_base_kernel, B.M, B.my.as<uint64_t>(), B.seed_n.as<uint32_t>(), B.qid.as<uint32_t>(), B.qm_off.as<int64_t>(),
-            mp_pos.as<int64_t>(), B.d_qbase.as<int64_t>(), B.M, B.pos_tab.as<MiniWord>());
+    LAUNCH1(mini_bits_kernel, B.M, B.my, B.seed_n.as<uint32_t>(), B.qid, B.d_qbase, B.M, B.pos_tab.as<MiniWord>());
+    LAUNCH1(mini_base_kernel, B.M, B.my, B.seed_n.as<uint32_t>(), B.qid, B.qm_off, mp_pos.as<int64_t>(), B.d_qbase, B.M,
+            B.pos_tab.as<MiniWord>());
     return HYMET_OK;
 }
 
@@ -868,7 +862,7 @@
     const hymet_mm_index *idx = B.idx;
     const int n_q = B.n_q;
     const int64_t M = B.M;
-    DevBuf &mx = B.mx, &my = B.my, &qm_off = B.qm_off, &seed_n = B.seed_n, &qid = B.qid, &d_qlen = B.d_qlen;
+    DevBuf &seed_n = B.seed_n;
     DevBuf a_pos, mflag, mp_pos;
     int64_t A = 0;
     int rc = scan_flags(ctx, seed_n.as<uint32_t>(), M, a_pos, &A);
@@ -883,13 +877,13 @@
     HY_HIP(B.mini_pos.alloc(8 * (size_t)(B.NM + 1), st));
     HY_HIP(B.mp_off.alloc(8 * (size_t)(n_q + 1), st));
     hipLaunchKernelGGL(sample_off_kernel, dim3((unsigned)cdiv(n_q + 1, 256)), dim3(256), 0, st, mp_pos.as<int64_t>(),
-                       qm_off.as<int64_t>(), n_q, B.NM, B.mp_off.as<int64_t>());
+                       B.qm_off, n_q, B.NM, B.mp_off.as<int64_t>());
     HY_CHECK_LAUNCH("sample_off_kernel");
     rc = build_mini_table(B, mp_pos);
     if (rc) return rc;
     HY_HIP(S1.d_off.alloc(8 * (size_t)(n_q + 1), st));
     hipLaunchKernelGGL(sample_off_kernel, dim3((unsigned)cdiv(n_q + 1, 256)), dim3(256), 0, st, a_pos.as<int64_t>(),
-                       qm_off.as<int64_t>(), n_q, A, S1.d_off.as<int64_t>());
+                       B.qm_off, n_q, A, S1.d_off.as<int64_t>());
     HY_CHECK_LAUNCH("sample_off_kernel");
     B.rb = bits_for(idx->n_seq);
     B.key1_bits = bits_for(n_q) + 1 + B.rb;
@@ -904,8 +898,8 @@
         DevBuf key, val;
         HY_HIP(key.alloc(8 * (size_t)(A + 1), st));
         if (!words) HY_HIP(val.alloc(4 * (size_t)(A + 1), st));
-        AnchorKeyParams P{mx.as<uint64_t>(), my.as<uint64_t>(), seed_n.as<uint32_t>(), a_pos.as<int64_t>(),
-                          qid.as<uint32_t>(), d_qlen.as<int64_t>(), idx->d_koff, idx->d_pos, M, B.rb, B.pb,
+        AnchorKeyParams P{B.mx, B.my, seed_n.as<uint32_t>(), a_pos.as<int64_t>(),
+                          B.qid, B.d_qlen, idx->d_koff, idx->d_pos, M, B.rb, B.pb,
                           words ? B.ybits : 0, key.as<uint64_t>(), val.as<uint32_t>(), mp_pos.as<int64_t>(),
                           B.mini_pos.as<uint64_t>()};
         {
@@ -924,8 +918,8 @@
     HY_HIP(k1.alloc(8 * (size_t)(A + 1), st));
     HY_HIP(k2.alloc(8 * (size_t)(A + 1), st));
     HY_HIP(val.alloc(4 * (size_t)(A + 1), st));
-    AnchorParams P{mx.as<uint64_t>(), my.as<uint64_t>(), seed_n.as<uint32_t>(), a_pos.as<int64_t>(), qid.as<uint32_t>(),
-                   d_qlen.as<int64_t>(), idx->d_koff, idx->d_pos, M, B.rb, x.as<uint64_t>(), k1.as<uint64_t>(),
+    AnchorParams P{B.mx, B.my, seed_n.as<uint32_t>(), a_pos.as<int64_t>(), B.qid,
+                   B.d_qlen, idx->d_koff, idx->d_pos, M, B.rb, x.as<uint64_t>(), k1.as<uint64_t>(),
                    k2.as<uint64_t>(), y.as<uint32_t>(), val.as<uint32_t>(), mp_pos.as<int64_t>(), B.mini_pos.as<uint64_t>()};
     ProfScope _ps(ctx, "mm_anchors", (double)A * (8.0 + 36.0));
     LAUNCH1(write_anchors_kernel, M, P);
@@ -989,10 +983,10 @@
     HY_HIP(nr.alloc(4 * (size_t)B.n_q, st));
     return launch_regions(B.ctx, C.ax, C.ay, C.span, C.ids.as<int32_t>(), C.cfirst.as<int64_t>(), C.cu.as<uint64_t>(),
                           C.cboff.as<int64_t>(), C.d_qc.as<int64_t>(), C.d_qb.as<int64_t>(), B.mini_pos.as<uint64_t>(),
-                          B.mp_off.as<int64_t>(), B.d_qlen.as<int64_t>(), B.d_hash, B.rep_len.as<int32_t>(), B.idx->d_len,
+                          B.mp_off.as<int64_t>(), B.d_qlen, B.d_hash, B.rep_len.as<int32_t>(), B.idx->d_len,
                           B.n_q, B.opt, B.idx->k, z.p, rg.as<hymet_mm_reg>(), wv.as<int32_t>(), cov.as<uint64_t>(),
                           tmp.as<int32_t>(), nr.as<int32_t>(), C.n_anchor, NC, B.NM, C.cq.as<uint32_t>(),
-                          B.pos_tab.as<MiniWord>(), B.d_qbase.as<int64_t>(), skip_q, sumk.as<uint64_t>(),
+                          B.pos_tab.as<MiniWord>(), B.d_qbase, skip_q, sumk.as<uint64_t>(),
                           std::exchange(sumk_done, true));
 }
 
@@ -1043,15 +1037,41 @@
     return HYMET_OK;
 }
 
-static int mm_map_impl(hymet_ctx *ctx, const hymet_mm_index *idx, const hymet_mm_opt *opt, const uint32_t *d_2b,
-                       const uint32_t *d_mask, const int64_t *h_starts, const int64_t *h_lens, const uint32_t *h_name_hash,
-                       const uint32_t *d_name_hash, int32_t n_q, MapSink &sink) {
-    CallTrace call_trace;
-    HY_ARG(ctx && idx && opt && d_2b && d_mask, "hymet_mm_map: null argument");
+static int qsketch_build(hymet_ctx *ctx, const hymet_mm_opt *opt, int w, int k, const uint32_t *d_2b, const uint32_t *d_mask,
+                         const int64_t *h_starts, const int64_t *h_lens, int32_t n_q, hymet_mm_qsketch &Q) {
+    HY_ARG(ctx && opt && d_2b && d_mask, "hymet_mm_map: null argument");
     HY_ARG(n_q >= 0, "hymet_mm_map: n_q < 0");
-    HY_ARG(h_name_hash || d_name_hash, "hymet_mm_map: no query name hashes");
+    HY_ARG(n_q == 0 || (h_starts && h_lens), "hymet_mm_map: null argument");
     HY_ARG(opt->mid_occ > 0, "hymet_mm_map: opt->mid_occ must be resolved (hymet_mm_index_max_occ + clamps)");
     HY_HIP(hipSetDevice(ctx->device));
+    Q.ctx = ctx;
+    Q.w = w, Q.k = k;
+    Q.mid_occ = opt->mid_occ, Q.q_occ_frac = opt->q_occ_frac;
+    Q.n_q = n_q;
+    if (n_q == 0) return HYMET_OK;
+    PhaseTrace tr(ctx);
+    int rc = sketch_queries(Q, d_2b, d_mask, h_starts, h_lens);
+    if (rc) return rc;
+    tr.mark("sketch");
+    rc = filter_minimizers(Q);
+    if (rc) return rc;
+    HY_HIP(Q.qid.alloc(4 * (size_t)(Q.M + 1), ctx->stream));
+    LAUNCH1(fill_qid_kernel, Q.M, Q.qm_off.as<int64_t>(), n_q, Q.M, Q.qid.as<uint32_t>(), nullptr, nullptr);
+    tr.mark("mz_flt");
+    return HYMET_OK;
+}
+
+static int mm_map_qs(hymet_ctx *ctx, const hymet_mm_index *idx, const hymet_mm_opt *opt, const hymet_mm_qsketch *qs,
+                     const uint32_t *h_name_hash, const uint32_t *d_name_hash, MapSink &sink) {
+    HY_ARG(ctx && idx && opt, "hymet_mm_map: null argument");
+    HY_ARG(qs != nullptr, "hymet_mm_map: null query sketch");
+    HY_ARG(qs->ctx == ctx, "hymet_mm_map: the query sketch belongs to another context");
+    HY_ARG(qs->w == idx->w && qs->k == idx->k, "hymet_mm_map: the query sketch's w / k are not the index's");
+    HY_ARG(qs->mid_occ == opt->mid_occ && qs->q_occ_frac == opt->q_occ_frac,
+           "hymet_mm_map: the query sketch was filtered with another mid_occ / q_occ_frac");
+    HY_ARG(h_name_hash || d_name_hash, "hymet_mm_map: no query name hashes");
+    HY_HIP(hipSetDevice(ctx->device));
+    const int32_t n_q = qs->n_q;
     if (sink.res) {
         sink.res->n_q = n_q;
         sink.res->reg_off.assign(n_q + 1, 0);
@@ -1061,14 +1081,14 @@
     const float pen_gap = (float)(opt->chain_gap_scale * 0.01 * idx->k);
     const float pen_skip = (float)(opt->chain_skip_scale * 0.01 * idx->k);
     PhaseTrace tr(ctx);
-    MapBatch B{ctx, idx, opt, h_lens, n_q};
-    int rc = sketch_queries(B, d_2b, d_mask, h_starts, h_name_hash, d_name_hash);
-    if (rc) return rc;
-    tr.mark("sketch");
-    rc = filter_minimizers(B);
-    if (rc) return rc;
-    tr.mark("mz_flt");
-    rc = select_seeds(B);
+    MapBatch B(ctx, idx, opt, *qs);
+    B.d_hash = d_name_hash;
+    if (!B.d_hash) {
+        HY_HIP(B.d_hash_buf.alloc(4 * (size_t)n_q, ctx->stream));
+        HY_HIP(hipMemcpyAsync(B.d_hash_buf.p, h_name_hash, 4 * (size_t)n_q, hipMemcpyHostToDevice, ctx->stream));
+        B.d_hash = B.d_hash_buf.as<uint32_t>();
+    }
+    int rc = select_seeds(B);
     if (rc) return rc;
     tr.mark("seeds");
     AnchorSet S1;
@@ -1081,7 +1101,7 @@
     ChainSet C1;
     const bool long_join = opt->bw_long > opt->bw;
     const bool resort = env_flag("HYMET_RECHAIN_SORT");
-    LeanJoin lj{B.d_qlen.as<int64_t>(), opt->rmq_rescue_size, opt->rmq_rescue_ratio, B.key_path && !resort};
+    LeanJoin lj{B.d_qlen, opt->rmq_rescue_size, opt->rmq_rescue_ratio, B.key_path && !resort};
     rc = chain_set(ctx, opt, pen_gap, pen_skip, opt->bw, S1, n_q, C1, long_join ? &lj : nullptr, long_join && !lj.mark_only);
     if (rc) return rc;
     tr.mark("chain_set 1");
@@ -1122,11 +1142,69 @@
 int hymet_mm_map(hymet_ctx *ctx, const hymet_mm_index *idx, const hymet_mm_opt *opt, const uint32_t *d_2b,
                  const uint32_t *d_mask, const int64_t *h_starts, const int64_t *h_lens, const uint32_t *h_name_hash,
                  int32_t n_q, hymet_mm_result **out) {
-    HY_ARG(out != nullptr, "hymet_mm_map: null argument");
+    HY_ARG(out != nullptr && idx != nullptr, "hymet_mm_map: null argument");
+    CallTrace call_trace;
     MapSink sink;
     sink.res = new hymet_mm_result();
     *out = sink.res;
-    return mm_map_impl(ctx, idx, opt, d_2b, d_mask, h_starts, h_lens, h_name_hash, nullptr, n_q, sink);
+    hymet_mm_qsketch qs;
+    const int rc = qsketch_build(ctx, opt, idx->w, idx->k, d_2b, d_mask, h_starts, h_lens, n_q, qs);
+    return rc ? rc : mm_map_qs(ctx, idx, opt, &qs, h_name_hash, nullptr, sink);
+}
+
+int hymet_mm_qsketch_create(hymet_ctx *ctx, const hymet_mm_opt *opt, int w, int k, const uint32_t *d_2b, const uint32_t *d_mask,
+                            const int64_t *h_starts, const int64_t *h_lens, int32_t n_q, hymet_mm_qsketch **out) {
+    HY_ARG(out != nullptr, "hymet_mm_qsketch_create: null argument");
+    *out = nullptr;
+    hymet_mm_qsketch *qs = new hymet_mm_qsketch();
+    const int rc = qsketch_build(ctx, opt, w, k, d_2b, d_mask, h_starts, h_lens, n_q, *qs);
+    if (rc) {
+        delete qs;
+        return rc;
+    }
+    qs->counted = true;
+    ctx->qs_live++;
+    *out = qs;
+    return HYMET_OK;
+}
+
+int hymet_mm_qsketch_destroy(hymet_mm_qsketch *qs) {
+    if (!qs) return HYMET_OK;
+    (void)hipSetDevice(qs->ctx->device);
+    if (qs->counted) qs->ctx->qs_live--;
+    delete qs;
+    return HYMET_OK;
+}
+
+int hymet_mm_qsketch_live(const hymet_ctx *ctx, int64_t *n) {
+    HY_ARG(ctx && n, "hymet_mm_qsketch_live: null argument");
+    *n = ctx->qs_live;
+    return HYMET_OK;
+}
+
+int hymet_mm_qsketch_copy(const hymet_mm_qsketch *qs, int64_t *n_mz, uint64_t *h_mx, uint64_t *h_my, int64_t *h_qm_off) {
+    HY_ARG(qs && n_mz, "hymet_mm_qsketch_copy: null argument");
+    *n_mz = qs->M;
+    if (qs->n_q == 0 || !(h_mx || h_my || h_qm_off)) return HYMET_OK;
+    HY_HIP(hipSetDevice(qs->ctx->device));
+    hipStream_t st = qs->ctx->stream;
+    if (h_mx && qs->M) HY_HIP(hipMemcpyAsync(h_mx, qs->mx.p, 8 * (size_t)qs->M, hipMemcpyDeviceToHost, st));
+    if (h_my && qs->M) HY_HIP(hipMemcpyAsync(h_my, qs->my.p, 8 * (size_t)qs->M, hipMemcpyDeviceToHost, st));
+    if (h_qm_off) HY_HIP(hipMemcpyAsync(h_qm_off, qs->qm_off.p, 8 * (size_t)(qs->n_q + 1), hipMemcpyDeviceToHost, st));
+    HY_HIP(hipStreamSynchronize(st));
+    return HYMET_OK;
+}
+
+int hymet_mm_map_acc_qs(hymet_ctx *ctx, const hymet_mm_index *idx, const hymet_mm_opt *opt, const hymet_mm_qsketch *qs,
+                        const uint32_t *d_name_hash, int32_t q_base, int32_t part_id, int32_t t_base, hymet_paf_acc *acc) {
+    HY_ARG(acc && d_name_hash, "hymet_mm_map_acc_qs: null argument");
+    CallTrace call_trace;
+    MapSink sink;
+    sink.acc = acc;
+    sink.q_base = q_base;
+    sink.part_id = part_id;
+    sink.t_base = t_base;
+    return mm_map_qs(ctx, idx, opt, qs, nullptr, d_name_hash, sink);
 }
 
 int hymet_paf_acc_create(hymet_ctx *ctx, hymet_paf_acc **out) {
@@ -1209,13 +1287,16 @@
 int hymet_mm_map_acc(hymet_ctx *ctx, const hymet_mm_index *idx, const hymet_mm_opt *opt, const uint32_t *d_2b,
                      const uint32_t *d_mask, const int64_t *h_starts, const int64_t *h_lens, const uint32_t *d_name_hash,
                      int32_t n_q, int32_t q_base, int32_t part_id, int32_t t_base, hymet_paf_acc *acc) {
-    HY_ARG(acc && d_name_hash, "hymet_mm_map_acc: null argument");
+    HY_ARG(acc && d_name_hash && idx, "hymet_mm_map_acc: null argument");
+    CallTrace call_trace;
     MapSink sink;
     sink.acc = acc;
     sink.q_base = q_base;
     sink.part_id = part_id;
     sink.t_base = t_base;
-    return mm_map_impl(ctx, idx, opt, d_2b, d_mask, h_starts, h_lens, nullptr, d_name_hash, n_q, sink);
+    hymet_mm_qsketch qs;
+    const int rc = qsketch_build(ctx, opt, idx->w, idx->k, d_2b, d_mask, h_starts, h_lens, n_q, qs);
+    return rc ? rc : mm_map_qs(ctx, idx, opt, &qs, nullptr, d_name_hash, sink);
 }
 
 int hymet_mm_result_size(const hymet_mm_result *res, int64_t *n_regs) {
diff --git a/hymet_amd/csrc/mm_sketch.hip b/hymet_amd/csrc/mm_sketch.hip
--- a/hymet_amd/csrc/mm_sketch.hip
+++ b/hymet_amd/csrc/mm_sketch.hip
@@ -118,6 +118,14 @@
         ox[o + j] = sx[s0 + j];
         oy[o + j] = sy[s0 + j];
     }
+}
+
+__global__ void seq_off_kernel(const int64_t *off, const int64_t *chunk_off, int n_seq, int64_t n_chunks, int64_t total,
+                               int64_t *out) {
+    const int s = blockIdx.x * blockDim.x + threadIdx.x;
+    if (s > n_seq) return;
+    const int64_t c = chunk_off[s];
+    out[s] = c < n_chunks ? off[c] : total;
 }
 
 __global__ void bucket_hist_kernel(const uint64_t *__restrict__ x, int64_t n, uint32_t *__restrict__ cnt,
@@ -243,16 +251,12 @@
         if (rc) return rc;
     }
     if (d_seq_off) {
-        std::vector<int64_t> so(n_seq + 1);
-        std::vector<int64_t> choff(n_chunks + 1);
-        if (n_chunks) HY_HIP(hipMemcpyAsync(choff.data(), d_off.p, 8 * (size_t)n_chunks, hipMemcpyDeviceToHost, ctx->stream));
-        HY_HIP(hipStreamSynchronize(ctx->stream));
-        choff[n_chunks] = total;
-        for (int i = 0; i <= n_seq; i++) so[i] = choff[coff[i]];
         HY_HIP(d_seq_off->alloc(8 * (size_t)(n_seq + 1), ctx->stream));
-        HY_HIP(hipMemcpyAsync(d_seq_off->p, so.data(), 8 * (size_t)(n_seq + 1), hipMemcpyHostToDevice, ctx->stream));
-        HY_HIP(hipStreamSynchronize(ctx->stream));
-    }
+        hipLaunchKernelGGL(seq_off_kernel, dim3((unsigned)cdiv(n_seq + 1, 256)), dim3(256), 0, ctx->stream,
+                           d_off.as<int64_t>(), d_coff.as<int64_t>(), n_seq, n_chunks, total, d_seq_off->as<int64_t>());
+        HY_CHECK_LAUNCH("seq_off_kernel");
+    }
+    if (n_chunks == 0) HY_HIP(hipStreamSynchronize(ctx->stream));
     *n_out = total;
     return HYMET_OK;
 }
diff --git a/hymet_amd/csrc/mm_stages.hpp b/hymet_amd/csrc/mm_stages.hpp
--- a/hymet_amd/csrc/mm_stages.hpp
+++ b/hymet_amd/csrc/mm_stages.hpp
@@ -95,3 +95,19 @@
 
 }
 }
+
+struct hymet_mm_qsketch {
+    hymet_ctx *ctx = nullptr;
+    int w = 0, k = 0;
+    int32_t mid_occ = 0;
+    float q_occ_frac = 0.f;
+    int32_t n_q = 0;
+    hymet::mm::DevBuf mx, my, qm_off;
+    int64_t M = 0;
+    hymet::mm::DevBuf qid;
+    hymet::mm::DevBuf d_qlen;
+    hymet::mm::DevBuf d_qbase;
+    std::vector<int64_t> qbase;
+    int64_t max_qlen = 1;
+    bool counted = false;
+};
diff --git a/hymet_amd/pipeline.py b/hymet_amd/pipeline.py
--- a/hymet_amd/pipeline.py
+++ b/hymet_amd/pipeline.py
@@ -99,6 +99,7 @@
         h = _c.c_void_p()
         check(gpu.lib.hymet_paf_acc_create(gpu.ctx, _c.byref(h)), "hymet_paf_acc_create")
         self.h = h
+        self.stage: Optional["PafAcc"] = None
 
     def reset(self):
         check(self.gpu.lib.hymet_paf_acc_reset(self.h), "hymet_paf_acc_reset")
@@ -118,6 +119,9 @@
         return q[:n], part[:n], t[:n]
 
     def close(self):
+        if getattr(self, "stage", None):
+            self.stage.close()
+            self.stage = None
         if getattr(self, "h", None):
             self.gpu.lib.hymet_paf_acc_destroy(self.h)
             self.h = None
@@ -143,42 +147,77 @@
     return ix
 
 
+class _BatchMapper:
+
+    def __init__(self, ix: IndexSet, sh: QueryShard):
+        self.ix, self.sh = ix, sh
+        self.batches = [(b0, b1) for b0, b1 in sh.batches if b1 > b0]
+        self.starts = np.ascontiguousarray(sh.starts, np.int64)
+        self.lens = np.ascontiguousarray(sh.lengths, np.int64)
+        self.hbase = sh.name_hash.data_ptr()
+        self.segs = [[None] * len(self.batches) for _ in ix.parts]
+
+    def map_batch(self, g, a: PafAcc, bi: int):
+        ix, sh = self.ix, self.sh
+        b0, b1 = self.batches[bi]
+        qs = _c.c_void_p()
+        g.call("hymet_mm_qsketch_create", _c.byref(ix.opt), ix.parts[0].w, ix.parts[0].k, ptr(sh.mm.w2b), ptr(sh.mm.wmask),
+               _c.c_void_p(self.starts.ctypes.data + 8 * b0), _c.c_void_p(self.lens.ctypes.data + 8 * b0), b1 - b0,
+               _c.byref(qs))
+        try:
+            for pi, part in enumerate(ix.parts):
+                before = a.n
+                g.call("hymet_mm_map_acc_qs", part.h, _c.byref(ix.opt), qs, _c.c_void_p(self.hbase + 4 * b0), b0, pi,
+                       ix.part_first[pi], a.h)
+                self.segs[pi][bi] = (a, before, a.n)
+        finally:
+            g.lib.hymet_mm_qsketch_destroy(qs)
+
+    def assemble(self, acc: PafAcc) -> int:
+        acc.reset()
+        for part_segs in self.segs:
+            for a, b, e in part_segs:
+                acc.gpu.call("hymet_paf_acc_append", acc.h, a.h, b, e)
+        return acc.n
+
+
 def map_shard(gpu, ix: IndexSet, sh: QueryShard, acc: PafAcc) -> int:
-    acc.reset()
-    starts = np.ascontiguousarray(sh.starts, np.int64)
-    lens = np.ascontiguousarray(sh.lengths, np.int64)
-    hbase = sh.name_hash.data_ptr()
-    for pi, part in enumerate(ix.parts):
-        for b0, b1 in sh.batches:
-            n = b1 - b0
-            if n <= 0:
-                continue
-            gpu.call("hymet_mm_map_acc", part.h, _c.byref(ix.opt), ptr(sh.mm.w2b), ptr(sh.mm.wmask),
-                     _c.c_void_p(starts.ctypes.data + 8 * b0), _c.c_void_p(lens.ctypes.data + 8 * b0),
-                     _c.c_void_p(hbase + 4 * b0), n, b0, pi, ix.part_first[pi], acc.h)
-    return acc.n
+    m = _BatchMapper(ix, sh)
+    if len(ix.parts) == 1:
+        acc.reset()
+        for bi in range(len(m.batches)):
+            m.map_batch(gpu, acc, bi)
+        return acc.n
+    if acc.stage is None:
+        acc.stage = PafAcc(gpu)
+    acc.stage.reset()
+    for bi in range(len(m.batches)):
+        m.map_batch(gpu, acc.stage, bi)
+    return m.assemble(acc)
 
 
 def map_shard_streams(gpus, accs, ix: IndexSet, sh: QueryShard, acc: PafAcc) -> int:
     import threading
-    tasks = [(pi, b0, b1) for pi in range(len(ix.parts)) for b0, b1 in sh.batches if b1 > b0]
-    segs = [None] * len(tasks)
+    m = _BatchMapper(ix, sh)
     errs = []
-    starts = np.ascontiguousarray(sh.starts, np.int64)
-    lens = np.ascontiguousarray(sh.lengths, np.int64)
-    hbase = sh.name_hash.data_ptr()
+    lock = threading.Lock()
+    nxt = [0]
+
+    def take():
+        with lock:
+            bi = nxt[0]
+            nxt[0] += 1
+        return bi if bi < len(m.batches) else None
 
     def work(w):
         g, a = gpus[w], accs[w]
         try:
             a.reset()
-            for ti in range(w, len(tasks), len(gpus)):
-                pi, b0, b1 = tasks[ti]
-                before = a.n
-                g.call("hymet_mm_map_acc", ix.parts[pi].h, _c.byref(ix.opt), ptr(sh.mm.w2b), ptr(sh.mm.wmask),
-                       _c.c_void_p(starts.ctypes.data + 8 * b0), _c.c_void_p(lens.ctypes.data + 8 * b0),
-                       _c.c_void_p(hbase + 4 * b0), b1 - b0, b0, pi, ix.part_first[pi], a.h)
-                segs[ti] = (w, before, a.n)
+            while not errs:
+                bi = take()
+                if bi is None:
+                    break
+                m.map_batch(g, a, bi)
         except Exception as e:
             errs.append(e)
 
@@ -189,11 +228,7 @@
         t.join()
     if errs:
         raise errs[0]
-    acc.reset()
-    g0 = acc.gpu
-    for w, b, e in segs:
-        g0.call("hymet_paf_acc_append", acc.h, accs[w].h, b, e)
-    return acc.n
+    return m.assemble(acc)
 
 
 def _dev_buf(gpu, bufs, key, nbytes):
diff --git a/include/hymet_gpu.h b/include/hymet_gpu.h
--- a/include/hymet_gpu.h
+++ b/include/hymet_gpu.h
@@ -162,6 +162,15 @@
 int hymet_mm_map_acc(hymet_ctx *ctx, const hymet_mm_index *idx, const hymet_mm_opt *opt, const uint32_t *d_2b,
                      const uint32_t *d_mask, const int64_t *h_starts, const int64_t *h_lens, const uint32_t *d_name_hash,
                      int32_t n_q, int32_t q_base, int32_t part_id, int32_t t_base, hymet_paf_acc *acc);
+typedef struct hymet_mm_qsketch hymet_mm_qsketch;
+int hymet_mm_qsketch_create(hymet_ctx *ctx, const hymet_mm_opt *opt, int w, int k, const uint32_t *d_2b,
+                            const uint32_t *d_mask, const int64_t *h_starts, const int64_t *h_lens, int32_t n_q,
+                            hymet_mm_qsketch **out);
+int hymet_mm_qsketch_destroy(hymet_mm_qsketch *qs);
+int hymet_mm_map_acc_qs(hymet_ctx *ctx, const hymet_mm_index *idx, const hymet_mm_opt *opt, const hymet_mm_qsketch *qs,
+                        const uint32_t *d_name_hash, int32_t q_base, int32_t part_id, int32_t t_base, hymet_paf_acc *acc);
+int hymet_mm_qsketch_copy(const hymet_mm_qsketch *qs, int64_t *n_mz, uint64_t *h_mx, uint64_t *h_my, int64_t *h_qm_off);
+int hymet_mm_qsketch_live(const hymet_ctx *ctx, int64_t *n);
 int hymet_emit_paf(hymet_ctx *ctx, const hymet_paf_acc *acc, const uint8_t *d_qname, const int64_t *d_qname_off,
                    const int64_t *d_qlen, const uint8_t *d_tname, const int64_t *d_tname_off, const int64_t *d_tlen,
                    char *d_out, int64_t cap, int64_t *n_bytes, int64_t *d_line_off);
```

Result: no change. 138,100, median of 6 (+1.3%).
